# Yukun-Huang/DreamWaltz-G

Hardware: AMD Instinct MI355X
Metric: SDS steps/sec @512^2, 100k Gaussians, SD1.5+ControlNet; raster Mpix/s vs HBM roofline (higher is better)
Workload: dtype f32x

## Files before the change

### dreamwaltz-g_amd/_lib.py

```python
import ctypes
import os

_HERE = os.path.dirname(os.path.abspath(__file__))
LIB_PATH = os.environ.get("DWG_LIB") or os.path.join(_HERE, "csrc", "libdwg_hip.so")
_lib = None

c_f32p = ctypes.c_void_p
c_i32p = ctypes.c_void_p


class RasterSettingsC(ctypes.Structure):
    _fields_ = [
        ("image_height", ctypes.c_int32), ("image_width", ctypes.c_int32),
        ("tanfovx", ctypes.c_float), ("tanfovy", ctypes.c_float), ("scale_modifier", ctypes.c_float),
        ("sh_degree", ctypes.c_int32), ("sh_coeffs", ctypes.c_int32),
        ("prefiltered", ctypes.c_int32), ("debug", ctypes.c_int32),
        ("bg", ctypes.c_void_p), ("viewmatrix", ctypes.c_void_p), ("projmatrix", ctypes.c_void_p),
        ("campos", ctypes.c_void_p), ("visit_order", ctypes.c_void_p), ("tanfov", ctypes.c_void_p),
    ]


class AdamGroupC(ctypes.Structure):
    _fields_ = [("param", ctypes.c_void_p), ("grad", ctypes.c_void_p), ("exp_avg", ctypes.c_void_p), ("exp_avg_sq", ctypes.c_void_p),
                ("n", ctypes.c_int64), ("beta1", ctypes.c_float), ("beta2", ctypes.c_float), ("eps", ctypes.c_float), ("hyper_row", ctypes.c_int32)]


class SegmentC(ctypes.Structure):
    _fields_ = [("dst", ctypes.c_void_p), ("src", ctypes.c_void_p), ("count", ctypes.c_int64)]


class RasterFramesC(ctypes.Structure):
    _fields_ = [("num_frames", ctypes.c_int32), ("gaussian_stride", ctypes.c_int64), ("camera_stride", ctypes.c_int64)]


class NerfFieldDescC(ctypes.Structure):
    _fields_ = [("embeddings", ctypes.c_void_p), ("offsets", ctypes.c_void_p), ("host_offsets", ctypes.c_void_p),
                ("num_levels", ctypes.c_uint32), ("log2_per_level_scale", ctypes.c_float), ("base_resolution", ctypes.c_uint32),
                ("gridtype", ctypes.c_uint32), ("align_corners", ctypes.c_uint32), ("interp", ctypes.c_uint32), ("bound", ctypes.c_float),
                ("num_layers", ctypes.c_uint32), ("hidden", ctypes.c_uint32), ("out_dim", ctypes.c_uint32),
                ("weight", ctypes.c_void_p * 4), ("bias", ctypes.c_void_p * 4),
                ("density_activation", ctypes.c_uint32), ("density_prior", ctypes.c_uint32), ("albedo_sigmoid", ctypes.c_uint32),
                ("raw", ctypes.c_uint32), ("sigma_scale", ctypes.c_void_p), ("precision", ctypes.c_uint32)]


class NerfFieldGradsC(ctypes.Structure):
    _fields_ = [("embeddings", ctypes.c_void_p), ("weight", ctypes.c_void_p * 4), ("bias", ctypes.c_void_p * 4),
                ("sigma_scale", ctypes.c_void_p), ("accumulate", ctypes.c_uint32)]


_vp, _i32, _i64, _f32, _sz = ctypes.c_void_p, ctypes.c_int32, ctypes.c_int64, ctypes.c_float, ctypes.c_size_t
_u32 = ctypes.c_uint32
SIGNATURES = {
    "dwg_raster_workspace_sizes": (ctypes.c_int, [_i32, _i32, _i32, _i64, ctypes.POINTER(_sz), ctypes.POINTER(_sz),
                                                  ctypes.POINTER(_sz)]),
    "dwg_raster_num_pairs_ptr": (_vp, [_vp]),
    "dwg_raster_camera_setup": (ctypes.c_int, [_vp, _vp, _vp, _vp, _vp]),
    "dwg_raster_camera_block": (ctypes.c_int, [_vp, _vp, _vp, _vp, _vp, _vp, _vp]),
    "dwg_raster_forward_bin": (ctypes.c_int, [ctypes.POINTER(RasterSettingsC), _i32] + [_vp] * 9 + [_vp]),
    "dwg_raster_forward_render": (ctypes.c_int, [ctypes.POINTER(RasterSettingsC), _i32, _vp, _vp, _i64, _vp, _vp, _vp,
                                                 _vp, _vp]),
    "dwg_raster_forward_bin_frames": (ctypes.c_int, [ctypes.POINTER(RasterSettingsC), ctypes.POINTER(RasterFramesC), _i32] + [_vp] * 9 + [_vp]),
    "dwg_raster_forward_render_frames": (ctypes.c_int, [ctypes.POINTER(RasterSettingsC), ctypes.POINTER(RasterFramesC), _i32, _vp, _vp, _i64, _vp,
                                                        _vp, _vp, _vp, _vp]),
    "dwg_raster_backward": (ctypes.c_int, [ctypes.POINTER(RasterSettingsC), _i32] + [_vp] * 7 + [_vp, _vp, _i64, _vp, _vp]
                            + [_vp] * 3 + [_vp] * 8 + [_vp]),
    "dwg_raster_backward_frames": (ctypes.c_int, [ctypes.POINTER(RasterSettingsC), ctypes.POINTER(RasterFramesC), _i32] + [_vp] * 7
                                   + [_vp, _vp, _i64, _vp, _vp] + [_vp] * 3 + [_vp] * 8 + [_vp]),
    "dwg_lbs_joint_chain": (ctypes.c_int, [_i32, _vp, _vp, _vp, _vp, _vp, _vp, _i32, _vp, _vp, _vp]),
    "dwg_lbs_blend_forward": (ctypes.c_int, [_i32, _i32, _i32] + [_vp] * 7 + [_vp]),
    "dwg_lbs_blend_backward": (ctypes.c_int, [_i32] + [_vp] * 7 + [_vp]),
    "dwg_lbs_vertex_transform": (ctypes.c_int, [_i32] * 4 + [_vp] * 8 + [_vp]),
    "dwg_lbs_vertex_transform_backward_shape": (ctypes.c_int, [_i32] * 3 + [_vp] * 9 + [_vp]),
    "dwg_lbs_vertex_transform_backward_shape_ws": (ctypes.c_int, [_i32] * 3 + [_vp] * 10 + [_vp]),
    "dwg_lbs_vertex_transform_backward_shape_workspace_floats": (ctypes.c_size_t, [_i32]),
    "dwg_grid_encode_forward": (ctypes.c_int, [_vp, _vp, _vp, _vp, _u32, _u32, _u32, _u32, _f32, _u32, _vp, _u32, _u32, _u32,
                                               _u32, _vp]),
    "dwg_grid_encode_backward": (ctypes.c_int, [_vp, _vp, _vp, _vp, _vp, _u32, _u32, _u32, _u32, _f32, _u32, _vp, _vp, _u32,
                                                _u32, _u32, _u32, _vp, _vp]),
    "dwg_grid_backward_slabs_workspace_bytes": (_sz, [_u32, _u32, _u32]),
    "dwg_grid_encode_backward_slabs": (ctypes.c_int, [_vp, _vp, _vp, _vp, _vp, _u32, _u32, _u32, _u32, _f32, _u32, _vp, _vp, _u32, _u32,
                                                      _u32, _u32, _vp, _vp, _sz, _i32, _vp]),
    "dwg_nerf_field_forward": (ctypes.c_int, [ctypes.POINTER(NerfFieldDescC), _vp, ctypes.c_uint64, _vp, _vp, _vp]),
    "dwg_nerf_field_backward_workspace_bytes": (_sz, [ctypes.POINTER(NerfFieldDescC), ctypes.c_uint64]),
    "dwg_nerf_field_backward": (ctypes.c_int, [ctypes.POINTER(NerfFieldDescC), _vp, ctypes.c_uint64, _vp, _vp,
                                               ctypes.POINTER(NerfFieldGradsC), _vp, _sz, _vp]),
    "dwg_nerf_render_infer": (ctypes.c_int, [ctypes.POINTER(NerfFieldDescC), _vp, _vp, _vp, _vp, _u32, _vp, _f32, _u32, _f32, _u32, _u32, _u32, _f32,
                                             _u32, _vp, _vp, _vp, _vp, _u32, _vp]),
    "dwg_nerf_render_shaded": (ctypes.c_int, [ctypes.POINTER(NerfFieldDescC), _vp, _vp, _vp, _vp, _u32, _vp, _f32, _u32, _f32, _u32, _u32, _u32, _f32,
                                              _u32, _u32, _vp, _f32, _f32, _vp, _vp, _vp, _vp, _u32, _vp]),
    "dwg_pc_lattice_sigma": (ctypes.c_int, [ctypes.POINTER(NerfFieldDescC), _vp, _vp, _vp, _u32, _u32, _u32, _u32, _vp, _vp, _vp]),
    "dwg_pc_select_workspace_bytes": (_sz, [ctypes.c_uint64]),
    "dwg_pc_select_above": (ctypes.c_int, [ctypes.c_uint64, _vp, _f32, _vp, ctypes.c_uint64, _vp, _vp, _sz, _vp]),
    "dwg_pc_select_flags": (ctypes.c_int, [ctypes.c_uint64, _vp, _vp, ctypes.c_uint64, _vp, _vp, _sz, _vp]),
    "dwg_pc_lattice_points": (ctypes.c_int, [ctypes.c_uint64, _vp, _vp, _vp, _vp, _u32, _u32, _u32, _u32, _vp, _vp]),
    "dwg_pc_fd_points": (ctypes.c_int, [ctypes.c_uint64, _vp, _f32, _f32, _vp, _vp]),
    "dwg_pc_finish": (ctypes.c_int, [ctypes.c_uint64, _u32, _vp, _vp, _f32, _vp, _vp, _vp]),
    "dwg_pc_outside_boxes": (ctypes.c_int, [ctypes.c_uint64, _vp, _u32, _vp, _vp, _vp]),
    "dwg_occ_lattice_sigma": (ctypes.c_int, [ctypes.POINTER(NerfFieldDescC), _vp, _vp, _vp, _vp, _u32, _u32, _u32, _vp, _vp]),
    "dwg_occ_lattice_points": (ctypes.c_int, [_vp, _vp, _vp, _vp, _u32, _u32, _vp, _vp]),
    "dwg_occ_update_workspace_bytes": (_sz, [_u32, _u32]),
    "dwg_occ_update": (ctypes.c_int, [_vp, _vp, _u32, _u32, _f32, _f32, _vp, _vp, _vp, _sz, _vp]),
    "dwg_video_composite_forward": (ctypes.c_int, [_i32, _i32, _i32, _vp, _vp, _i64, _i64, _i64, _vp, _i32, _i32, _i32, _vp, _vp, _vp, _vp]),
    "dwg_video_composite_backward": (ctypes.c_int, [_i32, _i32, _i32, _vp, _i64, _i64, _i64, _vp, _i32, _i32, _i32, _vp, _vp, _vp]),
    "dwg_sigma_face_records": (ctypes.c_int, [_i32, _vp, _i32, _vp, _vp, _vp, _vp]),
    "dwg_sigma_area_cdf": (ctypes.c_int, [_i32, _vp, _vp, _vp]),
    "dwg_sigma_vertex_normals": (ctypes.c_int, [_i32, _vp, _vp, _vp, _vp, _vp, _vp]),
    "dwg_sigma_sample": (ctypes.c_int, [_i32, _vp, _i32, _vp, _i32, _vp, _vp, _vp, _f32, _vp, _vp, _vp, _vp, _vp]),
    "dwg_sigma_distance_workspace_bytes": (_sz, [_i32, _i32]),
    "dwg_sigma_point_mesh_distance": (ctypes.c_int, [_i32, _vp, _i32, _vp, _vp, _vp, _vp, _vp, _sz, _vp]),
    "dwg_sigma_keep_mask": (ctypes.c_int, [_i32, _vp, _vp, _f32, _i32, _vp, _vp, _vp, _vp]),
    "dwg_avinit_barycentric": (ctypes.c_int, [_i32, _vp, _vp, _i32, _vp, _i32, _vp, _vp, _vp, _vp, _vp]),
    "dwg_avinit_lbs_interp": (ctypes.c_int, [_i32, _i32, _i32, _vp, _vp, _vp, _vp, _vp]),
    "dwg_avinit_knn": (ctypes.c_int, [_i32, _vp, _i32, _vp, _i32, _vp, _vp, _vp]),
    "dwg_avinit_knn_weights": (ctypes.c_int, [_i32, _i32, _vp, _vp, _vp, _i32, _f32, _f32, _vp, _vp, _vp]),
    "dwg_avinit_smooth": (ctypes.c_int, [_i32, _i32, _i32, _vp, _vp, _vp, _vp, _vp, _vp, _i32, _vp]),
    "dwg_raymarch_near_far_from_aabb": (ctypes.c_int, [_vp, _vp, _vp, _u32, _f32, _vp, _vp, _vp]),
    "dwg_raymarch_sph_from_ray": (ctypes.c_int, [_vp, _vp, _f32, _u32, _vp, _vp]),
    "dwg_raymarch_morton3d": (ctypes.c_int, [_vp, _u32, _vp, _vp]),
    "dwg_raymarch_morton3d_invert": (ctypes.c_int, [_vp, _u32, _vp, _vp]),
    "dwg_raymarch_packbits": (ctypes.c_int, [_vp, _u32, _f32, _vp, _vp]),
    "dwg_raymarch_packbits_dev": (ctypes.c_int, [_vp, _u32, _vp, _vp, _vp]),
    "dwg_raymarch_flatten_rays": (ctypes.c_int, [_vp, _u32, _u32, _vp, _vp]),
    "dwg_raymarch_train_workspace_bytes": (_sz, [_u32]),
    "dwg_raymarch_march_rays_train": (ctypes.c_int, [_vp, _vp, _vp, _f32, _u32, _f32, _u32, _u32, _u32, _u32, _vp, _vp, _vp, _vp, _vp, _u32,
                                                     _vp, _vp, _vp, _vp, _sz, _vp]),
    "dwg_raymarch_composite_rays_train_forward": (ctypes.c_int, [_vp, _vp, _vp, _vp, _u32, _u32, _u32, _f32, _u32, _vp, _vp, _vp, _vp, _vp]),
    "dwg_raymarch_composite_rays_train_backward": (ctypes.c_int, [_vp] * 11 + [_u32, _u32, _u32, _f32, _u32, _vp, _vp, _vp]),
    "dwg_raymarch_march_rays": (ctypes.c_int, [_u32, _u32, _vp, _vp, _vp, _vp, _f32, _u32, _f32, _u32, _u32, _u32, _vp, _vp, _vp, _u32, _vp, _vp,
                                               _vp, _vp, _vp]),
    "dwg_raymarch_composite_rays": (ctypes.c_int, [_u32, _u32, _u32, _f32, _u32, _vp, _vp, _vp, _vp, _vp, _u32, _vp, _vp, _vp, _vp]),
    "dwg_gemm":(ctypes.c_int, [_vp, _vp]),
    "dwg_gemm_workspace_bytes": (_sz, [_vp]),
    "dwg_transpose_2byte": (ctypes.c_int, [_i32, _i32, _i32, _vp, _i64, _i64, _vp, _i64, _i64, _vp]),
    "dwg_transpose_dt": (ctypes.c_int, [_i32, _i32, _i32, _i32, _vp, _i64, _i64, _vp, _i64, _i64, _vp]),
    "dwg_xfmt_pack": (ctypes.c_int, [_i64, _vp, _vp, _vp]),
    "dwg_xfmt_unpack": (ctypes.c_int, [_i64, _vp, _vp, _vp]),
    "dwg_vae_image_pack": (ctypes.c_int, [_i32, _i32, _i32, _vp, _vp, _vp]),
    "dwg_vae_grad_prescale_pack": (ctypes.c_int, [_i32, _i32, _vp, ctypes.c_float, _vp, _vp, _vp]),
    "dwg_vae_dx_unpack": (ctypes.c_int, [_i32, _i32, _i32, _vp, _vp, _vp, _vp]),
    "dwg_xfmt_range_scan": (ctypes.c_int, [_i64, _vp, _vp, _vp]),
    "dwg_act_backward_colsum": (ctypes.c_int, [_i32, _i32, _i32, _vp, _vp, _vp, _vp, _vp]),
    "dwg_mlp_chain_forward": (ctypes.c_int, [_i32, _i32, _vp, _i32, _i32, _vp, _vp, _vp, _vp, _vp, _vp, _vp, _i32, _vp, _i32, _vp]),
    "dwg_mlp_chain_backward_workspace_floats": (ctypes.c_size_t, [_i32, _i32]),
    "dwg_mlp_chain_backward": (ctypes.c_int, [_i32, _i32, _vp, _i32, _i32, _vp, _vp, _vp, _vp, _vp, _vp, _i32, _vp, _i32, _vp, _i32, _vp, _vp, _vp,
                                              _vp, _vp, _i32, _vp, _vp]),
    "dwg_adam_step": (ctypes.c_int, [_i64, _vp, _vp, _vp, _vp, _f32, _f32, _f32, _f32, _i32, _f32, _vp]),
    "dwg_adam_step_dev": (ctypes.c_int, [_i64, _vp, _vp, _vp, _vp, _vp, _f32, _f32, _f32, _vp]),
    "dwg_adam_step_groups_dev": (ctypes.c_int, [_i32, _vp, _vp, _vp]),
    "dwg_groupnorm_forward": (ctypes.c_int, [_i32, _i32, _i32, _i32, _vp, _vp, _vp, _f32, _i32, _vp, _vp, _vp, _vp]),
    "dwg_groupnorm_backward": (ctypes.c_int, [_i32, _i32, _i32, _i32, _vp, _vp, _vp, _vp, _vp, _f32, _i32, _vp, _vp, _vp, _vp, _vp]),
    "dwg_groupnorm_workspace_floats": (_sz, [_i32, _i32]),
    "dwg_layernorm_forward": (ctypes.c_int, [_i32, _i32, _vp, _vp, _vp, _f32, _vp, _vp]),
    "dwg_geglu_forward": (ctypes.c_int, [_i64, _i32, _vp, _vp, _vp]),
    "dwg_attention_forward": (ctypes.c_int, [_i32, _i32, _i32, _i32, _i32, _vp, _i64, _i64, _vp, _i64, _i64, _vp, _i64, _i64,
                                             _vp, _i64, _i64, _f32, _vp]),
    "dwg_attention_forward_dt": (ctypes.c_int, [_i32, _i32, _i32, _i32, _i32, _i32, _vp, _i64, _i64, _vp, _i64, _i64, _vp, _i64, _i64,
                                                _vp, _i64, _i64, _f32, _vp]),
    "dwg_attention_split_workspace_bytes": (_sz, [_i32, _i32, _i32, _i32, _i32, _i32]),
    "dwg_attention_forward_ws": (ctypes.c_int, [_i32, _i32, _i32, _i32, _i32, _i32, _vp, _i64, _i64, _vp, _i64, _i64, _vp, _i64, _i64,
                                                _vp, _i64, _i64, _f32, _vp, _sz, _vp]),
    "dwg_attention_forward_pairs_dt": (ctypes.c_int, [_i32] * 7 + [_vp, _i64, _i64, _i64] * 4 + [_f32, _vp]),
    "dwg_attention_forward_pairs_ws": (ctypes.c_int, [_i32] * 7 + [_vp, _i64, _i64, _i64] * 4 + [_f32, _vp, _sz, _vp]),
    "dwg_softmax_rows_forward": (ctypes.c_int, [_i32, _i32, _f32, _vp, _i64, _vp, _i64, _vp]),
    "dwg_softmax_rows_backward": (ctypes.c_int, [_i32, _i32, _f32, _vp, _i64, _vp, _i64, _vp, _i64, _vp]),
    "dwg_groupnorm_forward_dt": (ctypes.c_int, [_i32, _i32, _i32, _i32, _i32, _vp, _vp, _vp, _f32, _i32, _vp, _vp, _vp, _vp]),
    "dwg_groupnorm_backward_dt": (ctypes.c_int, [_i32, _i32, _i32, _i32, _i32, _vp, _vp, _vp, _vp, _vp, _f32, _i32, _vp, _vp, _vp, _vp, _vp]),
    "dwg_layernorm_forward_dt": (ctypes.c_int, [_i32, _i32, _i32, _vp, _vp, _vp, _f32, _vp, _vp]),
    "dwg_geglu_forward_dt": (ctypes.c_int, [_i32, _i64, _i32, _vp, _vp, _vp]),
    "dwg_softmax_rows_forward_dt": (ctypes.c_int, [_i32, _i32, _i32, _f32, _vp, _i64, _vp, _i64, _vp]),
    "dwg_softmax_rows_backward_dt": (ctypes.c_int, [_i32, _i32, _i32, _f32, _vp, _i64, _vp, _i64, _vp, _i64, _vp]),
    "dwg_add_dt": (ctypes.c_int, [_i32, _i64, _vp, _vp, _vp, _vp]),
    "dwg_cast_f32_to_dt": (ctypes.c_int, [_i32, _i64, _vp, _vp, _vp]),
    "dwg_mlp_wgrad_workspace_floats": (_sz, [_i32]),
    "dwg_mlp_wgrad": (ctypes.c_int, [_i32, _i32, _i32, _vp, _i32, _vp, _i32, _vp, _i32, _vp, _vp]),
    "dwg_concat_channels": (ctypes.c_int, [_i64, _i32, _i32, _vp, _vp, _vp, _vp]),
    "dwg_concat_channels_bcast": (ctypes.c_int, [_i64, _i64, _i32, _i32, _vp, _vp, _vp, _vp]),
    "dwg_add_bf16": (ctypes.c_int, [_i64, _vp, _vp, _vp, _vp]),
    "dwg_interleave2x2": (ctypes.c_int, [_i32, _i32, _i32, _i32, _vp, _vp, _vp, _vp, _vp, _vp]),
    "dwg_cast_f32_to_bf16": (ctypes.c_int, [_i64, _vp, _vp, _vp]),
    "dwg_sds_posterior_sample": (ctypes.c_int, [_i32, ctypes.c_int64, _vp, _vp, ctypes.c_float, _vp, _vp]),
    "dwg_sds_posterior_sample_backward": (ctypes.c_int, [_i32, ctypes.c_int64, _vp, _vp, ctypes.c_float, _vp, _vp, _vp]),
    "dwg_sds_add_noise": (ctypes.c_int, [_i32, ctypes.c_int64, _vp, _vp, _vp, _i32, _vp, _vp, _vp]),
    "dwg_sds_gradient": (ctypes.c_int, [_i32, ctypes.c_int64, _vp, _vp, _vp, _i32, _vp, ctypes.c_float, _i32, _i32, _vp, _vp, _vp]),
    "dwg_gaussian_assemble_forward": (ctypes.c_int, [_i32, _i32, _vp, _vp, _f32, _vp, _vp, _f32, _vp, _vp, _vp, _vp, _vp, _vp, _vp, _vp]),
    "dwg_gaussian_assemble_forward_ld": (ctypes.c_int, [_i32, _i32, _vp, _vp, _f32, _vp, _vp, _i32, _f32, _vp, _vp, _vp, _vp, _vp, _vp, _vp, _vp]),
    "dwg_gaussian_assemble_backward_ld": (ctypes.c_int, [_i32, _i32, _f32, _vp, _f32, _vp, _vp, _vp, _vp, _vp, _vp, _vp, _vp, _vp, _vp, _vp, _i32, _i32,
                                                         _vp, _vp, _vp]),
    "dwg_copy_segments": (ctypes.c_int, [_i32, _vp, _f32, _f32, _vp]),
    "dwg_add_segments": (ctypes.c_int, [_i32, _vp, _vp]),
    "dwg_gaussian_assemble_backward": (ctypes.c_int, [_i32, _i32, _f32, _vp, _f32, _vp, _vp, _vp, _vp, _vp, _vp, _vp, _vp, _vp, _vp,
                                                       _vp, _vp, _vp, _vp]),
    "dwg_mesh_vertex_normals": (ctypes.c_int, [_i32, _i32, _vp, _vp, _vp, _vp, _vp, _vp, _vp]),
    "dwg_meshbind_forward": (ctypes.c_int, [_i32, _i32, _vp, _vp, _vp, _vp, _vp, _vp, _vp, _vp, _vp, _vp, _vp]),
    "dwg_meshbind_backward": (ctypes.c_int, [_i32, _i32, _vp, _vp, _vp, _vp, _vp, _vp, _vp, _vp, _vp, _vp, _vp, _vp, _vp]),
    "dwg_meshbind_backward_verts": (ctypes.c_int, [_i32, _i32] + [_vp] * 15 + [_vp]),
    "dwg_meshbind_backward_verts_gather": (ctypes.c_int, [_i32, _i32, _i32] + [_vp] * 18 + [_vp]),
    "dwg_mesh_vertex_normals_backward": (ctypes.c_int, [_i32, _i32] + [_vp] * 8 + [_vp]),
    "dwg_condition_keypoints": (ctypes.c_int, [_i32, _vp, _vp, _vp, _i32, _vp, _i32, _vp, _vp, ctypes.c_float, ctypes.c_float,
                                               ctypes.c_float, _i32, _vp, _vp]),
    "dwg_condition_workspace_bytes": (_sz, [_i32, _i32]),
    "dwg_condition_draw": (ctypes.c_int, [_i32, _i32, _vp, _i32, _vp, _vp, _vp, _vp]),
    "dwg_condition_keypoints_people": (ctypes.c_int, [_i32, _i32, _vp, _vp, _vp, _i32, _vp, _i32, _vp, _vp, ctypes.c_float, ctypes.c_float,
                                                      ctypes.c_float, _i32, _i32, _vp, _vp, _vp]),
    "dwg_condition_people_workspace_bytes": (_sz, [_i32, _i32, _i32]),
    "dwg_condition_draw_people": (ctypes.c_int, [_i32, _i32, _i32, _vp, _i32, _vp, _vp, _vp, _vp]),
    "dwg_depthmap_workspace_bytes": (_sz, [_i32, _i32, _i32]),
    "dwg_depthmap_cast": (ctypes.c_int, [_i32, _i32, _vp, _vp, _i32, _vp, _i32, _vp, _vp, _vp, _i32, _vp, _sz, _vp]),
    "dwg_depthmap_image": (ctypes.c_int, [_i32, _i32, _vp, _i32, _vp, _vp, _vp, _sz, _vp]),
    "dwg_pretrain_loss_workspace_bytes": (_sz, [_i64]),
    "dwg_pretrain_loss_forward": (ctypes.c_int, [_i32, _i64, _vp, _vp, _vp, _vp, _vp, _sz, _vp]),
    "dwg_pretrain_loss_backward": (ctypes.c_int, [_i32, _i64, _vp, _vp, _vp, _vp, _vp, _vp, _vp]),
    "dwg_image_loss_workspace_bytes": (_sz, [_i32, _i32, _i32, _i32]),
    "dwg_image_loss_forward": (ctypes.c_int, [_i32] * 5 + [_f32] + [_vp, _i64, _i64, _i64, _i64] * 2 + [_vp, _vp, _vp, _vp, _sz, _vp]),
    "dwg_image_loss_backward": (ctypes.c_int, [_i32] * 5 + [ctypes.c_double] * 2 + [_vp, _i64, _i64, _i64, _i64] * 2
                                + [_vp, _vp, _i32, _vp, _vp]),
    "dwg_graph_begin_capture": (ctypes.c_int, [_vp]),
    "dwg_graph_end_capture": (ctypes.c_int, [_vp, ctypes.POINTER(_vp)]),
    "dwg_graph_launch": (ctypes.c_int, [_vp, _vp]),
    "dwg_graph_destroy": (ctypes.c_int, [_vp]),
    "dwg_stream_create": (ctypes.c_int, [ctypes.POINTER(_vp)]),
    "dwg_stream_destroy": (ctypes.c_int, [_vp]),
    "dwg_stream_fork": (ctypes.c_int, [_vp, _vp]),
    "dwg_prof_enable": (ctypes.c_int, [_i32]),
    "dwg_prof_query": (ctypes.c_int, [ctypes.c_char_p, ctypes.POINTER(_i64), ctypes.POINTER(ctypes.c_double)]),
    "dwg_prof_dump": (_i64, [ctypes.c_char_p, _i64]),
    "dwg_prof_dump_symbols": (_i64, [ctypes.c_char_p, _i64]),
}


def lib():
    global _lib
    if _lib is None:
        if not os.path.exists(LIB_PATH):
            raise RuntimeError(
                "libdwg_hip.so not found at %s -- run `python dreamwaltz-g_amd/build.py` "
                "(there is no CPU fallback for the product path)" % LIB_PATH)
        import torch
        l = ctypes.CDLL(LIB_PATH)
        for name, (res, args) in SIGNATURES.items():
            fn = getattr(l, name)
            fn.restype = res
            fn.argtypes = args
        _lib = l
    return _lib


def check(rc, what):
    if rc != 0:
        raise RuntimeError("%s failed with DWG error %d" % (what, rc))


def ptr(t):
    return None if t is None else ctypes.c_void_p(t.data_ptr())


def prof_enable(on=True):
    check(lib().dwg_prof_enable(int(bool(on))), "dwg_prof_enable")


def prof_table():
    L = lib()
    need = L.dwg_prof_dump(None, 0)
    buf = ctypes.create_string_buffer(int(need) + 16)
    L.dwg_prof_dump(buf, len(buf))
    out = {}
    for line in buf.value.decode().splitlines():
        n, c, ms = line.split()
        out[n] = (int(c), float(ms))
    return out


def prof_symbols():
    L = lib()
    need = L.dwg_prof_dump_symbols(None, 0)
    buf = ctypes.create_string_buffer(int(need) + 16)
    L.dwg_prof_dump_symbols(buf, len(buf))
    out = {}
    for line in buf.value.decode().splitlines():
        n, c, ms, w = line.split("\t")
        out[n] = (int(c), float(ms), float(w))
    return out
```

### dreamwaltz-g_amd/csrc/gemm.hip

```cpp
#include "dwg_common.h"
#include "dwg_prof_internal.h"
#include "../../include/dwg_gemm.h"
#include <cstdlib>
#include <type_traits>

#if defined(DWG_GEMM_X_TU)
#include "dwg_xfmt.h"
typedef _Float16 HT;
#define DWG_DTYPE_HALF DWG_DTYPE_F32X
#define DWG_MFMA16(a, b, c) __builtin_amdgcn_mfma_f32_32x32x16_f16(a, b, c, 0, 0, 0)
#define DWG_HALF_NAME "f32x"
#elif defined(DWG_GEMM_F16_TU)
typedef _Float16 HT;
#define DWG_DTYPE_HALF DWG_DTYPE_F16
#define DWG_MFMA16(a, b, c) __builtin_amdgcn_mfma_f32_32x32x16_f16(a, b, c, 0, 0, 0)
#define DWG_HALF_NAME "f16"
#else
typedef __bf16 HT;
#define DWG_DTYPE_HALF DWG_DTYPE_BF16
#define DWG_MFMA16(a, b, c) __builtin_amdgcn_mfma_f32_32x32x16_bf16(a, b, c, 0, 0, 0)
#define DWG_HALF_NAME "bf16"
#endif

namespace {

typedef __attribute__((ext_vector_type(8))) HT bf16x8;
typedef __attribute__((ext_vector_type(16))) float f32x16;

struct ConvP {
    int enabled, Cin, Hin, Win, Hout, Wout, KH, KW, stride, pad_t, pad_l, dil;
    int up;
    int cin1;
    const void* A2;
};

struct GemmP {
    const void* A; const void* B; void* C; const void* bias; const void* residual;
    int M, N, K;
    long long sam, sak, sbn, sbk, ldc, ldr;
    int nb2;
    long long bA1, bA2, bB1, bB2, bC1, bC2, bR1, bR2;
    int act; float alpha;
    int out_bf16, res_bf16, bias_per_row, splitk, accumulate;
    float* ws;
    int bias_row_div;
    long long bias_ld;
    ConvP conv;
};

__device__ __forceinline__ float bf2f(HT x) { return (float)x; }
__device__ __forceinline__ HT f2bf(float x) { return (HT)x; }

struct bf16x4_t { HT v[4]; };
#ifdef DWG_GEMM_X_TU
__device__ __forceinline__ float ld_half1(const void* base, long long i) { return dwg_x_get1(base, i); }
__device__ __forceinline__ void st_half1(void* base, long long i, float v) { dwg_x_put1(base, i, v); }
__device__ __forceinline__ void ld_half4(const void* base, long long i, float (&v)[4]) { dwg_x_get4(base, i, v); }
__device__ __forceinline__ void st_half4(void* base, long long i, const float (&v)[4]) { dwg_x_put4(base, i, v); }
#else
__device__ __forceinline__ float ld_half1(const void* base, long long i) { return bf2f(reinterpret_cast<const HT*>(base)[i]); }
__device__ __forceinline__ void st_half1(void* base, long long i, float v) { reinterpret_cast<HT*>(base)[i] = f2bf(v); }
__device__ __forceinline__ void ld_half4(const void* base, long long i, float (&v)[4]) {
    const bf16x4_t r = *reinterpret_cast<const bf16x4_t*>(reinterpret_cast<const HT*>(base) + i);
#pragma unroll
    for (int e = 0; e < 4; e++) v[e] = bf2f(r.v[e]);
}
__device__ __forceinline__ void st_half4(void* base, long long i, const float (&v)[4]) {
    bf16x4_t o;
#pragma unroll
    for (int e = 0; e < 4; e++) o.v[e] = f2bf(v[e]);
    *reinterpret_cast<bf16x4_t*>(reinterpret_cast<HT*>(base) + i) = o;
}
#endif

template <bool LIGHT = false>
__device__ __forceinline__ float apply_act(float v, int act) {
    if constexpr (LIGHT) return act == 3 ? v / (1.f + __expf(-v)) : v;
    switch (act) {
        case 1: return v > 0.f ? v : 0.f;
        case 2: return v > 0.f ? v : 0.01f * v;
        case 3: return v / (1.f + __expf(-v));
        case 4: return 0.5f * v * (1.f + erff(v * 0.70710678118654752f));
        case 5: return 1.f / (1.f + __expf(-v));
        default: return v;
    }
}

template <typename T> struct TT;
template <> struct TT<HT> { static constexpr int VEC = 8; static constexpr int BK = 64; static constexpr int PAD = 8; };
template <> struct TT<float> { static constexpr int VEC = 4; static constexpr int BK = 16; static constexpr int PAD = 4; };

enum { MODE_KVEC = 0, MODE_RVEC = 1, MODE_SCALAR = 2, MODE_CONV = 3 };

template <typename T, int VEC> struct Chunk { T v[VEC]; };

template <typename T, int VEC>
__device__ __forceinline__ Chunk<T, VEC> load_vec(const T* p) {
    Chunk<T, VEC> c;
    *reinterpret_cast<uint4*>(&c) = *reinterpret_cast<const uint4*>(p);
    return c;
}
template <typename T, int VEC>
__device__ __forceinline__ Chunk<T, VEC> zero_chunk() {
    Chunk<T, VEC> c;
    *reinterpret_cast<uint4*>(&c) = make_uint4(0u, 0u, 0u, 0u);
    return c;
}

template <typename T, int ROWS, int MODE>
struct TileLoader {
    static constexpr int VEC = TT<T>::VEC, BK = TT<T>::BK, LDT = BK + TT<T>::PAD;
    static constexpr int CPR = BK / VEC, RPI = 256 / CPR;
    static constexpr int CPK = ROWS / VEC, KPI = 256 / CPK;
    static constexpr int NCH = (MODE == MODE_SCALAR) ? (ROWS * BK / 256) : (MODE == MODE_RVEC ? BK / KPI : ROWS / RPI);
    Chunk<T, VEC> regs[(MODE == MODE_SCALAR) ? 1 : NCH];
    T sregs[(MODE == MODE_SCALAR) ? NCH : 1];
    const T* rowptr[(MODE == MODE_KVEC) ? NCH : 1];
    int iy0[(MODE == MODE_CONV) ? NCH : 1], ix0[(MODE == MODE_CONV) ? NCH : 1];
    long long pix0[(MODE == MODE_CONV) ? NCH : 1];
    bool rok[(MODE == MODE_CONV) ? NCH : 1];
    const T* base; long long srow, sk; int nrows, r0, kcur, kend;
    int ci, ky, kx;

    __device__ __forceinline__ void init(const T* base_, long long srow_, long long sk_, int nrows_, int r0_, int kbeg, int kend_,
                                         const ConvP& cv) {
        base = base_; srow = srow_; sk = sk_; nrows = nrows_; r0 = r0_; kend = kend_;
        const int tid = threadIdx.x;
        if (MODE == MODE_KVEC) {
            kcur = kbeg + (tid % CPR) * VEC;
#pragma unroll
            for (int i = 0; i < NCH; i++) {
                int r = r0 + tid / CPR + i * RPI;
                rowptr[i] = r < nrows ? base + (long long)r * srow : nullptr;
            }
        } else if (MODE == MODE_CONV) {
            kcur = kbeg + (tid % CPR) * VEC;
            const int hw = cv.Hout * cv.Wout;
#pragma unroll
            for (int i = 0; i < NCH; i++) {
                int r = r0 + tid / CPR + i * RPI;
                rok[i] = r < nrows;
                int rr = rok[i] ? r : 0;
                int img = rr / hw, rem = rr - img * hw;
                int oy = rem / cv.Wout, ox = rem - oy * cv.Wout;
                iy0[i] = oy * cv.stride - cv.pad_t; ix0[i] = ox * cv.stride - cv.pad_l;
                pix0[i] = (long long)img * cv.Hin * cv.Win;
            }
            int tap = kcur / cv.Cin;
            ci = kcur - tap * cv.Cin; ky = tap / cv.KW; kx = tap - ky * cv.KW;
        } else {
            kcur = kbeg;
        }
    }

    __device__ __forceinline__ void advance(const ConvP& cv) {
        kcur += BK;
        if (MODE == MODE_CONV) {
            ci += BK;
            while (ci >= cv.Cin) { ci -= cv.Cin; if (++kx == cv.KW) { kx = 0; ++ky; } }
        }
    }

    __device__ __forceinline__ void load(const ConvP& cv) {
        const int tid = threadIdx.x;
        if (MODE == MODE_KVEC) {
            const bool kok = kcur < kend;
#pragma unroll
            for (int i = 0; i < NCH; i++)
                regs[i] = (kok && rowptr[i]) ? load_vec<T, VEC>(rowptr[i] + kcur) : zero_chunk<T, VEC>();
        } else if (MODE == MODE_CONV) {
            const bool kok = kcur < kend;
            const T* src0 = ci < cv.cin1 ? base : reinterpret_cast<const T*>(cv.A2);
            const int cs = ci < cv.cin1 ? cv.cin1 : (cv.Cin - cv.cin1);
            const int co = ci < cv.cin1 ? ci : ci - cv.cin1;
#pragma unroll
            for (int i = 0; i < NCH; i++) {
                int iy = iy0[i] + ky, ix = ix0[i] + kx;
                bool ok = kok && rok[i] && iy >= 0 && ix >= 0;
                if (cv.dil > 1) { ok = ok && (iy % cv.dil == 0) && (ix % cv.dil == 0); iy /= cv.dil; ix /= cv.dil; }
                if (cv.up > 1) { iy >>= 1; ix >>= 1; }
                ok = ok && iy < cv.Hin && ix < cv.Win;
                regs[i] = ok ? load_vec<T, VEC>(src0 + (pix0[i] + (long long)iy * cv.Win + ix) * cs + co) : zero_chunk<T, VEC>();
            }
        } else if (MODE == MODE_RVEC) {
#pragma unroll
            for (int i = 0; i < NCH; i++) {
                int kk = tid / CPK + i * KPI, rc = tid % CPK;
                int r = r0 + rc * VEC, k = kcur + kk;
                regs[i] = (r < nrows && k < kend) ? load_vec<T, VEC>(base + (long long)k * sk + r) : zero_chunk<T, VEC>();
            }
        } else {
#pragma unroll
            for (int i = 0; i < NCH; i++) {
                int c = tid + i * 256, row = c / BK, kk = c - row * BK;
                int r = r0 + row, k = kcur + kk;
                sregs[i] = (r < nrows && k < kend) ? base[(long long)r * srow + (long long)k * sk] : (T)0.f;
            }
        }
    }

    __device__ __forceinline__ void store(T* lds) {
        const int tid = threadIdx.x;
        if (MODE == MODE_KVEC || MODE == MODE_CONV) {
#pragma unroll
            for (int i = 0; i < NCH; i++)
                *reinterpret_cast<uint4*>(lds + (tid / CPR + i * RPI) * LDT + (tid % CPR) * VEC) = *reinterpret_cast<uint4*>(&regs[i]);
        } else if (MODE == MODE_RVEC) {
#pragma unroll
            for (int i = 0; i < NCH; i++) {
                int kk = tid / CPK + i * KPI, rc = tid % CPK;
#pragma unroll
                for (int e = 0; e < VEC; e++) lds[(rc * VEC + e) * LDT + kk] = regs[i].v[e];
            }
        } else {
#pragma unroll
            for (int i = 0; i < NCH; i++) {
                int c = tid + i * 256, row = c / BK, kk = c - row * BK;
                lds[row * LDT + kk] = sregs[i];
            }
        }
    }
};

template <typename T>
__device__ __forceinline__ void mma_tile(const T* sa, const T* sb, int lane, f32x16& acc);

template <>
__device__ __forceinline__ void mma_tile<HT>(const HT* sa, const HT* sb, int lane, f32x16& acc) {
    constexpr int LDT = TT<HT>::BK + TT<HT>::PAD;
    const HT* pa = sa + (lane & 31) * LDT + (lane >> 5) * 8;
    const HT* pb = sb + (lane & 31) * LDT + (lane >> 5) * 8;
#pragma unroll
    for (int ks = 0; ks < TT<HT>::BK / 16; ks++) {
        bf16x8 a = *reinterpret_cast<const bf16x8*>(pa + ks * 16);
        bf16x8 b = *reinterpret_cast<const bf16x8*>(pb + ks * 16);
        acc = DWG_MFMA16(a, b, acc);
    }
}
template <>
__device__ __forceinline__ void mma_tile<float>(const float* sa, const float* sb, int lane, f32x16& acc) {
    constexpr int LDT = TT<float>::BK + TT<float>::PAD;
    const float* pa = sa + (lane & 31) * LDT + (lane >> 5);
    const float* pb = sb + (lane & 31) * LDT + (lane >> 5);
#pragma unroll
    for (int ks = 0; ks < TT<float>::BK / 2; ks++)
        acc = __builtin_amdgcn_mfma_f32_32x32x2f32(pa[ks * 2], pb[ks * 2], acc, 0, 0, 0);
}

template <bool LIGHT = false>
__device__ __forceinline__ void epilogue_store(const GemmP& p, float v, int row, int col, long long coff, long long roff) {
    const long long ci = coff + (long long)row * p.ldc + col;
    if (p.bias) v += reinterpret_cast<const float*>(p.bias)[p.bias_row_div > 0 ? (long long)(row / p.bias_row_div) * p.bias_ld + col
                                                                             : (p.bias_per_row ? row : col)];
    v = apply_act<LIGHT>(v, p.act);
    if (p.residual) {
        const long long ri = roff + (long long)row * p.ldr + col;
        v += p.res_bf16 ? ld_half1(p.residual, ri) : reinterpret_cast<const float*>(p.residual)[ri];
    }
    if (p.out_bf16) st_half1(p.C, ci, v);
    else if (p.accumulate) reinterpret_cast<float*>(p.C)[ci] += v;
    else reinterpret_cast<float*>(p.C)[ci] = v;
}

__device__ __forceinline__ bool epilogue_vec_ok(const GemmP& p, long long coff, long long roff) {
    bool ok = (p.N & 3) == 0 && (p.ldc & 3) == 0 && (coff & 3) == 0 && ((uintptr_t)p.C & 15) == 0;
    if (p.residual) ok = ok && (p.ldr & 3) == 0 && (roff & 3) == 0 && ((uintptr_t)p.residual & 15) == 0;
    return ok;
}

template <bool LIGHT = false>
__device__ __forceinline__ void epilogue_store4(const GemmP& p, float (&v)[4], int row, int col, long long coff, long long roff, bool vec_ok) {
    if (!vec_ok || col + 3 >= p.N) {
#pragma unroll
        for (int e = 0; e < 4; e++)
            if (col + e < p.N) epilogue_store<LIGHT>(p, v[e], row, col + e, coff, roff);
        return;
    }
    if (p.bias) {
        const float* b = reinterpret_cast<const float*>(p.bias);
        if (p.bias_row_div > 0) {
            b += (long long)(row / p.bias_row_div) * p.bias_ld + col;
            v[0] += b[0]; v[1] += b[1]; v[2] += b[2]; v[3] += b[3];
        } else if (p.bias_per_row) {
            const float br = b[row];
            v[0] += br; v[1] += br; v[2] += br; v[3] += br;
        } else {
            v[0] += b[col]; v[1] += b[col + 1]; v[2] += b[col + 2]; v[3] += b[col + 3];
        }
    }
#pragma unroll
    for (int e = 0; e < 4; e++) v[e] = apply_act<LIGHT>(v[e], p.act);
    if (p.residual) {
        const long long ri = roff + (long long)row * p.ldr + col;
        if (p.res_bf16) {
            float r[4];
            ld_half4(p.residual, ri, r);
#pragma unroll
            for (int e = 0; e < 4; e++) v[e] += r[e];
        } else {
            float4 r = *reinterpret_cast<const float4*>(reinterpret_cast<const float*>(p.residual) + ri);
            v[0] += r.x; v[1] += r.y; v[2] += r.z; v[3] += r.w;
        }
    }
    const long long ci = coff + (long long)row * p.ldc + col;
    if (p.out_bf16) {
        st_half4(p.C, ci, v);
    } else {
        float4* dst = reinterpret_cast<float4*>(reinterpret_cast<float*>(p.C) + ci);
        float4 o = make_float4(v[0], v[1], v[2], v[3]);
        if (p.accumulate) { float4 c = *dst; o.x += c.x; o.y += c.y; o.z += c.z; o.w += c.w; }
        *dst = o;
    }
}

template <int BN, int BM = 128> struct EpiLds {
    static constexpr int LDC = BN + 4;
    static constexpr int passes(size_t lds_bytes) {
        return lds_bytes >= (size_t)BM * LDC * 4 ? 1 : (lds_bytes >= (size_t)(BM / 2) * LDC * 4 ? 2 : 4);
    }
    static constexpr size_t bytes(int npass) { return (size_t)(BM / npass) * LDC * 4; }
};

template <int BN, int NPASS, int TM, int TN, bool LIGHT, int BM = 128, int NT = 256, typename RowFn>
__device__ __forceinline__ void tile_epilogue_lds(const GemmP& p, f32x16 (&acc)[TM][TN], float* sC, int n0, int wm, int wn, int lane, int tid,
                                                  int ks_id, long long coff, long long roff, RowFn row_of) {
    constexpr int LDC = EpiLds<BN, BM>::LDC, C4 = BN / 4, PR = BM / NPASS;
    constexpr int BPP = BM / 32 / NPASS;
    static_assert(NT % C4 == 0 && (C4 & (C4 - 1)) == 0, "a thread keeps one column group");
    const bool vec_ok = epilogue_vec_ok(p, coff, roff);
    const int lrow = lane & 31, lhalf = (lane >> 5) * 4;
    const bool geglu = p.act == 6;
    const float* bias = reinterpret_cast<const float*>(p.bias);
    const bool fast = vec_ok && !geglu && !p.accumulate && !p.bias_per_row && (p.splitk <= 1 || p.ws) &&
                      (!bias || p.bias_row_div > 0 || ((uintptr_t)bias & 15) == 0) &&
                      (!bias || p.bias_row_div <= 0 || (((uintptr_t)bias & 15) == 0 && (p.bias_ld & 3) == 0)) &&
                      (p.splitk <= 1 || ((uintptr_t)p.ws & 15) == 0);
#pragma unroll 1
    for (int q = 0; q < NPASS; q++) {
        __syncthreads();
#pragma unroll
        for (int i = 0; i < TM; i++) {
            const int rb = wm * TM + i;
            if (NPASS > 1 && rb / BPP != q) continue;
            float* dst = sC + ((NPASS > 1 ? rb % BPP : rb) * 32 + lrow) * LDC + wn * 64 + lhalf;
#pragma unroll
            for (int j = 0; j < TN; j++)
#pragma unroll
                for (int r4 = 0; r4 < 4; r4++)
                    *reinterpret_cast<float4*>(dst + j * 32 + 8 * r4) =
                        make_float4(acc[i][j][4 * r4], acc[i][j][4 * r4 + 1], acc[i][j][4 * r4 + 2], acc[i][j][4 * r4 + 3]);
        }
        __syncthreads();
        if (geglu) {
            constexpr int G = C4 / 2, RSTEP = NT / G;
            const int o4 = tid & (G - 1), rl0 = tid / G;
            const int b = o4 >> 3, w = (o4 & 7) * 4;
            const int colp = n0 + b * 64 + w;
            if (colp + 35 < p.N) {
                float bh[4] = {0.f, 0.f, 0.f, 0.f}, bg[4] = {0.f, 0.f, 0.f, 0.f};
                if (bias) {
#pragma unroll
                    for (int e = 0; e < 4; e++) { bh[e] = bias[colp + e]; bg[e] = bias[colp + 32 + e]; }
                }
                const bool vec_store = ((p.ldc | coff) & 3) == 0 && ((uintptr_t)p.C & 7) == 0;
#pragma unroll 2
                for (int rl = rl0; rl < PR; rl += RSTEP) {
                    const int row = row_of(q * PR + rl);
                    if (row < 0) continue;
                    const float4 h = *reinterpret_cast<const float4*>(sC + rl * LDC + b * 64 + w);
                    const float4 g = *reinterpret_cast<const float4*>(sC + rl * LDC + b * 64 + 32 + w);
                    const float hv[4] = {h.x, h.y, h.z, h.w}, gv[4] = {g.x, g.y, g.z, g.w};
                    float v[4];
#pragma unroll
                    for (int e = 0; e < 4; e++) {
                        const float a = fmaf(hv[e], p.alpha, bh[e]);
                        const float gg = fmaf(gv[e], p.alpha, bg[e]);
                        v[e] = a * 0.5f * gg * (1.f + dwg_erf_fast(gg * 0.70710678118654752f));
                    }
                    const long long ci = coff + (long long)row * p.ldc + (n0 + b * 64) / 2 + w;
                    if (p.out_bf16) {
                        if (vec_store) {
                            st_half4(p.C, ci, v);
                        } else {
#pragma unroll
                            for (int e = 0; e < 4; e++) st_half1(p.C, ci + e, v[e]);
                        }
                    } else {
#pragma unroll
                        for (int e = 0; e < 4; e++) reinterpret_cast<float*>(p.C)[ci + e] = v[e];
                    }
                }
            }
            continue;
        }
        if (fast) {
            constexpr int RSTEP = NT / C4;
            const int c4 = tid & (C4 - 1), rl0 = tid / C4;
            const int col = n0 + c4 * 4;
            if (col < p.N) {
                const bool col_bias = bias && p.bias_row_div <= 0;
                float4 bc = make_float4(0.f, 0.f, 0.f, 0.f);
                if (col_bias) bc = *reinterpret_cast<const float4*>(bias + col);
                const bool slab = p.splitk > 1;
#pragma unroll 2
                for (int rl = rl0; rl < PR; rl += RSTEP) {
                    const int row = row_of(q * PR + rl);
                    if (row < 0) continue;
                    const float4 a = *reinterpret_cast<const float4*>(sC + rl * LDC + c4 * 4);
                    float v[4] = {a.x * p.alpha, a.y * p.alpha, a.z * p.alpha, a.w * p.alpha};
                    if (slab) {
                        *reinterpret_cast<float4*>(p.ws + ((long long)ks_id * p.M + row) * p.N + col) = make_float4(v[0], v[1], v[2], v[3]);
                        continue;
                    }
                    if (col_bias) { v[0] += bc.x; v[1] += bc.y; v[2] += bc.z; v[3] += bc.w; }
                    else if (bias) {
                        const float4 b = *reinterpret_cast<const float4*>(bias + (long long)(row / p.bias_row_div) * p.bias_ld + col);
                        v[0] += b.x; v[1] += b.y; v[2] += b.z; v[3] += b.w;
                    }
                    if (p.act == 3) {
#pragma unroll
                        for (int e = 0; e < 4; e++) v[e] = v[e] / (1.f + __expf(-v[e]));
                    } else if (p.act != 0) {
#pragma unroll
                        for (int e = 0; e < 4; e++) v[e] = apply_act<LIGHT>(v[e], p.act);
                    }
                    if (p.residual) {
                        const long long ri = roff + (long long)row * p.ldr + col;
                        if (p.res_bf16) {
                            float r[4];
                            ld_half4(p.residual, ri, r);
#pragma unroll
                            for (int e = 0; e < 4; e++) v[e] += r[e];
                        } else {
                            const float4 r = *reinterpret_cast<const float4*>(reinterpret_cast<const float*>(p.residual) + ri);
                            v[0] += r.x; v[1] += r.y; v[2] += r.z; v[3] += r.w;
                        }
                    }
                    const long long ci = coff + (long long)row * p.ldc + col;
                    if (p.out_bf16) {
                        st_half4(p.C, ci, v);
                    } else {
                        *reinterpret_cast<float4*>(reinterpret_cast<float*>(p.C) + ci) = make_float4(v[0], v[1], v[2], v[3]);
                    }
                }
            }
            continue;
        }
#pragma unroll 1
        for (int idx = tid; idx < PR * C4; idx += NT) {
            const int rl = idx / C4, c4 = idx - rl * C4;
            const int row = row_of(q * PR + rl), col = n0 + c4 * 4;
            if (row < 0 || col >= p.N) continue;
            const float4 a = *reinterpret_cast<const float4*>(sC + rl * LDC + c4 * 4);
            float v[4] = {a.x * p.alpha, a.y * p.alpha, a.z * p.alpha, a.w * p.alpha};
            if (p.splitk > 1) {
                if (p.ws) {
                    float* dst = p.ws + ((long long)ks_id * p.M + row) * p.N + col;
                    if ((p.N & 3) == 0) *reinterpret_cast<float4*>(dst) = make_float4(v[0], v[1], v[2], v[3]);
                    else {
#pragma unroll
                        for (int e = 0; e < 4; e++) if (col + e < p.N) dst[e] = v[e];
                    }
                } else {
#pragma unroll
                    for (int e = 0; e < 4; e++)
                        if (col + e < p.N) atomicAdd(reinterpret_cast<float*>(p.C) + coff + (long long)row * p.ldc + col + e, v[e]);
                }
                continue;
            }
            epilogue_store4<LIGHT>(p, v, row, col, coff, roff, vec_ok);
        }
    }
}

__global__ __launch_bounds__(256) void k_splitk_epilogue(GemmP p) {
    const long long n = (long long)p.M * p.N;
    if ((p.N & 3) == 0) {
        const bool vec_ok = epilogue_vec_ok(p, 0, 0);
        const int N4 = p.N >> 2;
        const long long n4 = n >> 2;
        for (long long i = (long long)blockIdx.x * 256 + threadIdx.x; i < n4; i += (long long)gridDim.x * 256) {
            const unsigned iu = (unsigned)i;
            const int row = (int)(iu / (unsigned)N4), col = (int)(iu - (unsigned)row * (unsigned)N4) * 4;
            const float4* src = reinterpret_cast<const float4*>(p.ws) + i;
            float4 a = src[0];
            int sidx = 1;
            for (; sidx + 3 < p.splitk; sidx += 4) {
                const float4 u0 = src[(long long)sidx * n4], u1 = src[(long long)(sidx + 1) * n4], u2 = src[(long long)(sidx + 2) * n4],
                             u3 = src[(long long)(sidx + 3) * n4];
                a.x += u0.x; a.y += u0.y; a.z += u0.z; a.w += u0.w;
                a.x += u1.x; a.y += u1.y; a.z += u1.z; a.w += u1.w;
                a.x += u2.x; a.y += u2.y; a.z += u2.z; a.w += u2.w;
                a.x += u3.x; a.y += u3.y; a.z += u3.z; a.w += u3.w;
            }
            if (sidx + 1 < p.splitk) {
                const float4 u0 = src[(long long)sidx * n4], u1 = src[(long long)(sidx + 1) * n4];
                a.x += u0.x; a.y += u0.y; a.z += u0.z; a.w += u0.w;
                a.x += u1.x; a.y += u1.y; a.z += u1.z; a.w += u1.w;
                sidx += 2;
            }
            if (sidx < p.splitk) {
                const float4 u = src[(long long)sidx * n4];
                a.x += u.x; a.y += u.y; a.z += u.z; a.w += u.w;
            }
            float v[4] = {a.x, a.y, a.z, a.w};
            epilogue_store4(p, v, row, col, 0, 0, vec_ok);
        }
        return;
    }
    for (long long i = (long long)blockIdx.x * 256 + threadIdx.x; i < n; i += (long long)gridDim.x * 256) {
        float v = 0.f;
        for (int s = 0; s < p.splitk; s++) v += p.ws[(long long)s * n + i];
        int row = (int)(i / p.N), col = (int)(i - (long long)row * p.N);
        epilogue_store(p, v, row, col, 0, 0);
    }
}

static void launch_splitk_epilogue(const GemmP& p, hipStream_t stream) {
    if (!(p.splitk > 1 && p.ws)) return;
    long long n = (long long)p.M * p.N;
    if ((p.N & 3) == 0) n >>= 2;
    int blocks = (int)((n + 255) / 256); if (blocks > 2048) blocks = 2048;
    DWG_LAUNCH("splitk_epilogue", k_splitk_epilogue, dim3(blocks), dim3(256), 0, stream, p);
}
template <typename T, int BN, int AMODE, int BMODE>
__global__ __launch_bounds__(256, (sizeof(T) == 4 || BN == 64) ? 2 : 1) void k_gemm(GemmP p) {
    constexpr int BM = 128, BK = TT<T>::BK, LDT = BK + TT<T>::PAD;
    constexpr int WN = BN / 64;
    constexpr int WM = 4 / WN;
    constexpr int TM = BM / WM / 32;
    constexpr int TN = 2;
    extern __shared__ __attribute__((aligned(16))) unsigned char smem_raw[];
    T* sA = reinterpret_cast<T*>(smem_raw);
    T* sB = sA + 2 * BM * LDT;
    const int tid = threadIdx.x, lane = tid & 63, wave = tid >> 6;
    const int wm = wave / WN, wn = wave % WN;
    const int m0 = blockIdx.x * BM;
    const int ntn = (p.N + BN - 1) / BN;
    const int n0 = (blockIdx.y % ntn) * BN;
    const int ks_id = blockIdx.y / ntn;
    const int z = blockIdx.z, z1 = z / p.nb2, z2 = z - z1 * p.nb2;
    const T* A = reinterpret_cast<const T*>(p.A) + z1 * p.bA1 + z2 * p.bA2;
    const T* B = reinterpret_cast<const T*>(p.B) + z1 * p.bB1 + z2 * p.bB2;
    int kbeg = 0, kend = p.K;
    if (p.splitk > 1) {
        int per = ((p.K + p.splitk - 1) / p.splitk + BK - 1) / BK * BK;
        kbeg = ks_id * per; kend = min(p.K, kbeg + per);
    }
    f32x16 acc[TM][TN];
#pragma unroll
    for (int i = 0; i < TM; i++)
#pragma unroll
        for (int j = 0; j < TN; j++)
#pragma unroll
            for (int r = 0; r < 16; r++) acc[i][j][r] = 0.f;

    TileLoader<T, BM, AMODE> la;
    TileLoader<T, BN, BMODE> lb;
    la.init(A, p.sam, p.sak, p.M, m0, kbeg, kend, p.conv);
    lb.init(B, p.sbn, p.sbk, p.N, n0, kbeg, kend, p.conv);
    const int nk = kend > kbeg ? (kend - kbeg + BK - 1) / BK : 0;
    if (nk > 0) {
        la.load(p.conv); lb.load(p.conv);
        la.store(sA); lb.store(sB);
    }
    __syncthreads();
    for (int kt = 0; kt < nk; kt++) {
        const int cur = kt & 1;
        if (kt + 1 < nk) {
            la.advance(p.conv); lb.advance(p.conv);
            la.load(p.conv); lb.load(p.conv);
        }
        const T* a = sA + cur * BM * LDT + (wm * TM * 32) * LDT;
        const T* b = sB + cur * BN * LDT + (wn * 64) * LDT;
#pragma unroll
        for (int i = 0; i < TM; i++)
#pragma unroll
            for (int j = 0; j < TN; j++) mma_tile<T>(b + j * 32 * LDT, a + i * 32 * LDT, lane, acc[i][j]);
        if (kt + 1 < nk) { la.store(sA + (cur ^ 1) * BM * LDT); lb.store(sB + (cur ^ 1) * BN * LDT); }
        __syncthreads();
    }
    constexpr int NPASS = EpiLds<BN>::passes((size_t)2 * (BM + BN) * LDT * sizeof(T));
    static_assert((size_t)2 * (BM + BN) * LDT * sizeof(T) >= EpiLds<BN>::bytes(NPASS), "epilogue staging fits in the operand stages");
    tile_epilogue_lds<BN, NPASS, TM, TN, false>(p, acc, reinterpret_cast<float*>(smem_raw), n0, wm, wn, lane, tid, ks_id, z1 * p.bC1 + z2 * p.bC2,
                                         z1 * p.bR1 + z2 * p.bR2, [&](int rl) { const int r = m0 + rl; return r < p.M ? r : -1; });
}

__device__ __attribute__((aligned(16))) unsigned char g_zero16[16];

template <int ROWS, bool CONV, int NW = 4>
struct GldsLoader {
    static constexpr int NJ = ROWS / (8 * NW);
    const HT* rowptr[CONV ? 1 : NJ];
    int iy0[CONV ? NJ : 1], ix0[CONV ? NJ : 1];
    long long pix0[CONV ? NJ : 1];
    bool rok[CONV ? NJ : 1];
    const HT* base;
    int kc[2], kend, ci[2], ky[2], kx[2];

    __device__ __forceinline__ void init(const HT* base_, long long srow, int nrows, int r0, int kbeg, int kend_, const ConvP& cv) {
        static_assert(NJ % 2 == 0, "row-block parity must equal j parity");
        base = base_; kend = kend_;
        const int lane = threadIdx.x & 63, wave = threadIdx.x >> 6, sub = lane >> 3;
        const int lg0 = (lane & 7) ^ (sub >> 1);
        kc[0] = kbeg + lg0 * 8; kc[1] = kbeg + (lg0 ^ 4) * 8;
        if (!CONV) {
#pragma unroll
            for (int j = 0; j < NJ; j++) {
                int r = r0 + (wave * NJ + j) * 8 + sub;
                rowptr[j] = r < nrows ? base + (long long)r * srow : nullptr;
            }
        } else {
            const int hw = cv.Hout * cv.Wout;
#pragma unroll
            for (int j = 0; j < NJ; j++) {
                int r = r0 + (wave * NJ + j) * 8 + sub;
                rok[j] = r < nrows;
                int rr = rok[j] ? r : 0;
                int img = rr / hw, rem = rr - img * hw;
                int oy = rem / cv.Wout, ox = rem - oy * cv.Wout;
                iy0[j] = oy * cv.stride - cv.pad_t; ix0[j] = ox * cv.stride - cv.pad_l;
                pix0[j] = (long long)img * cv.Hin * cv.Win;
            }
#pragma unroll
            for (int q = 0; q < 2; q++) {
                int tap = kc[q] / cv.Cin;
                ci[q] = kc[q] - tap * cv.Cin; ky[q] = tap / cv.KW; kx[q] = tap - ky[q] * cv.KW;
            }
        }
    }
    __device__ __forceinline__ void advance(const ConvP& cv) {
        kc[0] += 64; kc[1] += 64;
        if (CONV) {
#pragma unroll
            for (int q = 0; q < 2; q++) {
                ci[q] += 64;
                while (ci[q] >= cv.Cin) { ci[q] -= cv.Cin; if (++kx[q] == cv.KW) { kx[q] = 0; ++ky[q]; } }
            }
        }
    }
    __device__ __forceinline__ void issue(unsigned char* lds_tile, const ConvP& cv) {
        const int wave = __builtin_amdgcn_readfirstlane(threadIdx.x >> 6);
        const HT* zero = reinterpret_cast<const HT*>(g_zero16);
        const HT* src0[2] = {base, base}; int cs[2] = {0, 0}, co[2] = {0, 0};
        bool kok[2];
#pragma unroll
        for (int q = 0; q < 2; q++) {
            kok[q] = kc[q] < kend;
            if (CONV) {
                src0[q] = ci[q] < cv.cin1 ? base : reinterpret_cast<const HT*>(cv.A2);
                cs[q] = ci[q] < cv.cin1 ? cv.cin1 : (cv.Cin - cv.cin1);
                co[q] = ci[q] < cv.cin1 ? ci[q] : ci[q] - cv.cin1;
            }
        }
#pragma unroll
        for (int j = 0; j < NJ; j++) {
            const int q = j & 1;
            const HT* src;
            if (!CONV) {
                src = (kok[q] && rowptr[j]) ? rowptr[j] + kc[q] : zero;
            } else {
                int iy = iy0[j] + ky[q], ix = ix0[j] + kx[q];
                bool ok = kok[q] && rok[j] && iy >= 0 && ix >= 0;
                if (cv.dil > 1) { ok = ok && (iy % cv.dil == 0) && (ix % cv.dil == 0); iy /= cv.dil; ix /= cv.dil; }
                if (cv.up > 1) { iy >>= 1; ix >>= 1; }
                ok = ok && iy < cv.Hin && ix < cv.Win;
                src = ok ? src0[q] + (pix0[j] + (long long)iy * cv.Win + ix) * cs[q] + co[q] : zero;
            }
            unsigned char* dst = lds_tile + ((wave * NJ + j) * 8) * 128;
            __builtin_amdgcn_global_load_lds((const __attribute__((address_space(1))) void*)src,
                                             (__attribute__((address_space(3))) void*)dst, 16, 0, 0);
        }
    }
};

template <int ROWS, int NW = 4, bool CAT = false>
struct GldsConvFast {
    static constexpr int NJ = ROWS / (8 * NW);
    const unsigned char* pb[NJ];
    const unsigned char* pb2[CAT ? NJ : 1];
    unsigned int mask[NJ];
    int kcur, kend, tap, ci, ky, kx;

    __device__ __forceinline__ void init(const HT* base, long long, int nrows, int r0, int kbeg, int kend_, const ConvP& cv) {
        static_assert(NJ % 2 == 0, "row-block parity must equal j parity");
        const int lane = threadIdx.x & 63, wave = threadIdx.x >> 6, sub = lane >> 3;
        const int lg0 = (lane & 7) ^ (sub >> 1);
        kcur = kbeg; kend = kend_;
        tap = kbeg / cv.Cin; ci = kbeg - tap * cv.Cin; ky = tap / cv.KW; kx = tap - ky * cv.KW;
        const int hw = cv.Hout * cv.Wout;
        const int cs1 = CAT ? cv.cin1 : cv.Cin;
#pragma unroll
        for (int j = 0; j < NJ; j++) {
            const int r = r0 + (wave * NJ + j) * 8 + sub;
            const bool rok = r < nrows;
            const int rr = rok ? r : 0;
            const int img = rr / hw, rem = rr - img * hw;
            const int oy = rem / cv.Wout, ox = rem - oy * cv.Wout;
            const int iy0 = oy * cv.stride - cv.pad_t, ix0 = ox * cv.stride - cv.pad_l;
            unsigned int m = 0;
            for (int t = 0, y = 0; y < cv.KH; y++)
                for (int x = 0; x < cv.KW; x++, t++) {
                    const int iy = iy0 + y, ix = ix0 + x;
                    if (rok && iy >= 0 && iy < cv.Hin && ix >= 0 && ix < cv.Win) m |= 1u << t;
                }
            mask[j] = m;
            const long long pix = ((long long)img * cv.Hin + iy0) * cv.Win + ix0;
            pb[j] = reinterpret_cast<const unsigned char*>(base) + (pix * cs1 + (lg0 ^ ((j & 1) << 2)) * 8) * 2;
            if (CAT) pb2[j] = reinterpret_cast<const unsigned char*>(cv.A2) + (pix * (cv.Cin - cv.cin1) + (lg0 ^ ((j & 1) << 2)) * 8) * 2;
        }
    }
    __device__ __forceinline__ void advance(const ConvP& cv) {
        kcur += 64; ci += 64;
        const int w = ci >= cv.Cin ? 1 : 0;
        ci = w ? 0 : ci; tap += w; kx += w;
        const int w2 = kx == cv.KW ? 1 : 0;
        kx = w2 ? 0 : kx; ky += w2;
    }
    __device__ __forceinline__ void issue(unsigned char* lds_tile, const ConvP& cv) {
        const int wave = __builtin_amdgcn_readfirstlane(threadIdx.x >> 6);
        const unsigned char* zero = g_zero16;
        const bool second = CAT && ci >= cv.cin1;
        const int cs = CAT ? (second ? cv.Cin - cv.cin1 : cv.cin1) : cv.Cin;
        const long long uoff = (((long long)ky * cv.Win + kx) * cs + (second ? ci - cv.cin1 : ci)) * 2;
        const unsigned int bit = kcur < kend ? (1u << tap) : 0u;
#pragma unroll
        for (int j = 0; j < NJ; j++) {
            const unsigned char* src = (mask[j] & bit) ? ((CAT && second) ? pb2[j] : pb[j]) + uoff : zero;
            unsigned char* dst = lds_tile + ((wave * NJ + j) * 8) * 128;
            __builtin_amdgcn_global_load_lds((const __attribute__((address_space(1))) void*)src,
                                             (__attribute__((address_space(3))) void*)dst, 16, 0, 0);
        }
    }
};

template <int N>
__device__ __forceinline__ void wait_vmcnt() {
    __builtin_amdgcn_s_waitcnt((N & 15) | ((N >> 4) << 14) | (7 << 4) | (15 << 8));
}

template <int BM, int AKIND, int NW = 4> struct ALoaderOf { typedef GldsLoader<BM, false, NW> type; };
template <int BM, int NW> struct ALoaderOf<BM, 1, NW> { typedef GldsLoader<BM, true, NW> type; };
template <int BM, int NW> struct ALoaderOf<BM, 2, NW> { typedef GldsConvFast<BM, NW, false> type; };
template <int BM, int NW> struct ALoaderOf<BM, 3, NW> { typedef GldsConvFast<BM, NW, true> type; };

template <int BM, int BN> struct GldsGeom {
    static constexpr int WN = BN / 64, WM = (BM == 128 && BN == 64) ? 4 : BM / 64, NW = WM * WN, NT = NW * 64, TM = BM / WM / 32, TN = 2;
};

template <int BM, int BN, int AKIND, int S>
__device__ __forceinline__ void gemm_glds_body(const GemmP& p) {
    typedef GldsGeom<BM, BN> Geo;
    constexpr int WN = Geo::WN, WM = Geo::WM, NW = Geo::NW, NT = Geo::NT, TM = Geo::TM, TN = Geo::TN;
    constexpr int ABYTES = BM * 128, BBYTES = BN * 128, STAGE = ABYTES + BBYTES;
    extern __shared__ __attribute__((aligned(16))) unsigned char smem_raw[];
    const int tid = threadIdx.x, lane = tid & 63, wave = tid >> 6;
    const int wm = wave / WN, wn = wave % WN;
    const int gm = (p.M + BM - 1) / BM, ntn = (p.N + BN - 1) / BN;
    const int nwg = gridDim.x;
    int id = blockIdx.x;
    {
        const int q = nwg / 8, r = nwg % 8, xcd = id % 8, loc = id / 8;
        id = (xcd < r ? xcd * (q + 1) : r * (q + 1) + (xcd - r) * q) + loc;
    }
    const int tile = id % (gm * ntn), ks_id = id / (gm * ntn);
    const int m0 = (tile / ntn) * BM, n0 = (tile % ntn) * BN;
    const int z = blockIdx.z, z1 = z / p.nb2, z2 = z - z1 * p.nb2;
    const HT* A = reinterpret_cast<const HT*>(p.A) + z1 * p.bA1 + z2 * p.bA2;
    const HT* B = reinterpret_cast<const HT*>(p.B) + z1 * p.bB1 + z2 * p.bB2;
    int kbeg = 0, kend = p.K;
    if (p.splitk > 1) {
        int per = ((p.K + p.splitk - 1) / p.splitk + 63) / 64 * 64;
        kbeg = ks_id * per; kend = min(p.K, kbeg + per);
    }
    f32x16 acc[TM][TN];
#pragma unroll
    for (int i = 0; i < TM; i++)
#pragma unroll
        for (int j = 0; j < TN; j++)
#pragma unroll
            for (int r = 0; r < 16; r++) acc[i][j][r] = 0.f;
#ifdef DWG_GEMM_X_TU
    f32x16 acx[TM][TN];
#pragma unroll
    for (int i = 0; i < TM; i++)
#pragma unroll
        for (int j = 0; j < TN; j++)
#pragma unroll
            for (int r = 0; r < 16; r++) acx[i][j][r] = 0.f;
#endif
    typename ALoaderOf<BM, AKIND, NW>::type la;
    GldsLoader<BN, false, NW> lb;
    la.init(A, p.sam, p.M, m0, kbeg, kend, p.conv);
    lb.init(B, p.sbn, p.N, n0, kbeg, kend, p.conv);
    const int nk = kend > kbeg ? (kend - kbeg + 63) / 64 : 0;
    constexpr int LPT = (BM + BN) * 128 / (NT * 16);
#pragma unroll
    for (int s = 0; s < S - 1; s++) {
        la.issue(smem_raw + s * STAGE, p.conv); lb.issue(smem_raw + s * STAGE + ABYTES, p.conv);
        la.advance(p.conv); lb.advance(p.conv);
    }
    const int frow = lane & 31, fx = (lane >> 1) & 7, fh = lane >> 5;
#ifdef DWG_GEMM_X_TU
    constexpr int KS = 2;
    struct Frag { bf16x8 ah[TM], al[TM], bh[TN], bl[TN]; };
#else
    constexpr int KS = 4;
    struct Frag { bf16x8 af[TM], bf[TN]; };
#endif
    auto load_frags = [&](int stage, int ks, Frag& f) {
        const unsigned char* ta = smem_raw + stage * STAGE + (wm * TM * 32 + frow) * 128;
        const unsigned char* tb = smem_raw + stage * STAGE + ABYTES + (wn * 64 + frow) * 128;
#ifdef DWG_GEMM_X_TU
        const int offh = (((ks * 4 + fh * 2) ^ fx) << 4), offl = (((ks * 4 + fh * 2 + 1) ^ fx) << 4);
#pragma unroll
        for (int i = 0; i < TM; i++) {
            f.ah[i] = *reinterpret_cast<const bf16x8*>(ta + i * 32 * 128 + offh);
            f.al[i] = *reinterpret_cast<const bf16x8*>(ta + i * 32 * 128 + offl);
        }
#pragma unroll
        for (int j = 0; j < TN; j++) {
            f.bh[j] = *reinterpret_cast<const bf16x8*>(tb + j * 32 * 128 + offh);
            f.bl[j] = *reinterpret_cast<const bf16x8*>(tb + j * 32 * 128 + offl);
        }
#else
        const int off = (((ks * 2 + fh) ^ fx) << 4);
#pragma unroll
        for (int i = 0; i < TM; i++) f.af[i] = *reinterpret_cast<const bf16x8*>(ta + i * 32 * 128 + off);
#pragma unroll
        for (int j = 0; j < TN; j++) f.bf[j] = *reinterpret_cast<const bf16x8*>(tb + j * 32 * 128 + off);
#endif
    };
    auto mma = [&](const Frag& f) {
#ifdef DWG_GEMM_X_TU
#pragma unroll
        for (int i = 0; i < TM; i++)
#pragma unroll
            for (int j = 0; j < TN; j++) acc[i][j] = DWG_MFMA16(f.bh[j], f.ah[i], acc[i][j]);
#pragma unroll
        for (int i = 0; i < TM; i++)
#pragma unroll
            for (int j = 0; j < TN; j++) acx[i][j] = DWG_MFMA16(f.bl[j], f.ah[i], acx[i][j]);
#pragma unroll
        for (int i = 0; i < TM; i++)
#pragma unroll
            for (int j = 0; j < TN; j++) acx[i][j] = DWG_MFMA16(f.bh[j], f.al[i], acx[i][j]);
#else
#pragma unroll
        for (int i = 0; i < TM; i++)
#pragma unroll
            for (int j = 0; j < TN; j++) acc[i][j] = DWG_MFMA16(f.bf[j], f.af[i], acc[i][j]);
#endif
    };
    auto wait_tile_and_lds = [&]() {
        constexpr int N = (S - 2) * LPT;
        __builtin_amdgcn_s_waitcnt((N & 15) | ((N >> 4) << 14) | (7 << 4) | (0 << 8));
    };
    Frag F[2];
    int cur = 0, nxt = S - 1;
    if (nk > 0) {
        wait_vmcnt<(S - 2) * LPT>();
        __builtin_amdgcn_s_barrier();
        load_frags(0, 0, F[0]);
        __builtin_amdgcn_s_waitcnt(0xC07F);
    }
#ifdef DWG_GEMM_X_TU
    constexpr int MPS = 3 * TM * TN;
#else
    constexpr int MPS = TM * TN;
#endif
    for (int kt = 0; kt < nk; kt++) {
        const int cnext = cur + 1 == S ? 0 : cur + 1;
#pragma unroll
        for (int ks = 0; ks < KS; ks++) {
            if (ks + 1 < KS) {
                load_frags(cur, ks + 1, F[(ks + 1) & 1]);
            } else {
                wait_tile_and_lds();
                __builtin_amdgcn_s_barrier();
                load_frags(cnext, 0, F[0]);
            }
            __builtin_amdgcn_sched_barrier(0);
            if (ks == 0) {
                la.issue(smem_raw + nxt * STAGE, p.conv); lb.issue(smem_raw + nxt * STAGE + ABYTES, p.conv);
                la.advance(p.conv); lb.advance(p.conv);
            }
            mma(F[ks & 1]);
            if (ks == 0) {
#pragma unroll
                for (int m = 0; m < MPS; m++) {
                    __builtin_amdgcn_sched_group_barrier(0x008, 1, 0);
                    __builtin_amdgcn_sched_group_barrier(0x006, (LPT * 10 + MPS - 1) / MPS, 0);
                    __builtin_amdgcn_sched_group_barrier(0x020, (LPT + MPS - 1) / MPS, 0);
                }
            }
            __builtin_amdgcn_sched_barrier(0);
        }
        __builtin_amdgcn_s_waitcnt(0xC07F);
        cur = cnext; nxt = nxt + 1 == S ? 0 : nxt + 1;
    }
    wait_vmcnt<0>();
#ifdef DWG_GEMM_X_TU
#pragma unroll
    for (int i = 0; i < TM; i++)
#pragma unroll
        for (int j = 0; j < TN; j++)
#pragma unroll
            for (int r = 0; r < 16; r++) acc[i][j][r] = fmaf(acx[i][j][r], DWG_X_LO_INV, acc[i][j][r]);
#endif
    constexpr int NPASS = EpiLds<BN, BM>::passes((size_t)S * STAGE);
    static_assert((size_t)S * STAGE >= EpiLds<BN, BM>::bytes(NPASS), "epilogue staging fits in the operand stages");
    tile_epilogue_lds<BN, NPASS, TM, TN, false, BM, NT>(p, acc, reinterpret_cast<float*>(smem_raw), n0, wm, wn, lane, tid, ks_id, z1 * p.bC1 + z2 * p.bC2,
                                         z1 * p.bR1 + z2 * p.bR2, [&](int rl) { const int r = m0 + rl; return r < p.M ? r : -1; });
}

template <int BN, int AKIND, int S>
__global__ __launch_bounds__(256, 2) void k_gemm_glds(GemmP p) {
    gemm_glds_body<128, BN, AKIND, S>(p);
}

template <int BM, int BN, int AKIND, int S>
__global__ __launch_bounds__(512, 2) void k_gemm_glds8(GemmP p) {
    static_assert(GldsGeom<BM, BN>::NT == 512, "eight waves");
    gemm_glds_body<BM, BN, AKIND, S>(p);
}

static double gemm_flops(const GemmP& p, int batch) {
    double f = 2.0 * p.M * p.N * p.K * batch;
#ifdef DWG_GEMM_X_TU
    f *= 0.5;
#endif
    if (p.conv.enabled && p.conv.dil > 1) f /= (double)(p.conv.dil * p.conv.dil);
    return f;
}

template <int BN, int AKIND>
static void launch_glds(const GemmP& p, int batch, hipStream_t stream, const char* name) {
    constexpr int S = (BN == 64 && AKIND != 1) ? 3 : 2;
    size_t lds = (size_t)S * (128 + BN) * 128;
    static bool attr_set = false;
    if (!attr_set) {
        hipFuncSetAttribute(reinterpret_cast<const void*>(&k_gemm_glds<BN, AKIND, S>), hipFuncAttributeMaxDynamicSharedMemorySize, (int)lds);
        attr_set = true;
    }
    dim3 grid(((p.M + 127) / 128) * ((p.N + BN - 1) / BN) * (p.splitk > 1 ? p.splitk : 1), 1, batch);
    static const char* const sym[2][4] = {{"k_gemm_glds<64, 0, 3>", "k_gemm_glds<64, 1, 2>", "k_gemm_glds<64, 2, 3>", "k_gemm_glds<64, 3, 3>"},
                                          {"k_gemm_glds<128, 0, 2>", "k_gemm_glds<128, 1, 2>", "k_gemm_glds<128, 2, 2>", "k_gemm_glds<128, 3, 2>"}};
    DWG_LAUNCH_W(name, sym[BN == 128][AKIND], gemm_flops(p, batch), (k_gemm_glds<BN, AKIND, S>), grid, dim3(256), lds, stream, p);
    launch_splitk_epilogue(p, stream);
}

template <int BM, int BN, int AKIND>
static void launch_glds8(const GemmP& p, int batch, hipStream_t stream, const char* name) {
    constexpr int S = 3;
    const size_t lds = (size_t)S * (BM + BN) * 128;
    static bool attr_set = false;
    if (!attr_set) {
        hipFuncSetAttribute(reinterpret_cast<const void*>(&k_gemm_glds8<BM, BN, AKIND, S>), hipFuncAttributeMaxDynamicSharedMemorySize, (int)lds);
        attr_set = true;
    }
    dim3 grid(((p.M + BM - 1) / BM) * ((p.N + BN - 1) / BN) * (p.splitk > 1 ? p.splitk : 1), 1, batch);
    static const char* const sym[2][4] = {
        {"k_gemm_glds8<256, 128, 0, 3>", "k_gemm_glds8<256, 128, 1, 3>", "k_gemm_glds8<256, 128, 2, 3>", "k_gemm_glds8<256, 128, 3, 3>"},
        {"k_gemm_glds8<128, 256, 0, 3>", "k_gemm_glds8<128, 256, 1, 3>", "k_gemm_glds8<128, 256, 2, 3>", "k_gemm_glds8<128, 256, 3, 3>"}};
    DWG_LAUNCH_W(name, sym[BN == 256][AKIND], gemm_flops(p, batch), (k_gemm_glds8<BM, BN, AKIND, S>), grid, dim3(512), lds, stream, p);
    launch_splitk_epilogue(p, stream);
}

template <bool V> struct BoolC { static constexpr bool value = V; };
template <int BN, int NW> struct Patch2Geom {
    static constexpr int PH = NW == 8 ? 16 : 8, PW = 16, HP = PH + 2, WP = PW + 2, NPIX = HP * WP, BM = PH * PW;
    static constexpr int NPI = (NPIX + 7) / 8;
    static constexpr int PPW = (NPI + NW - 1) / NW;
    static constexpr int WN = BN / 64, WM = NW / WN, TM = BM / WM / 32, TN = 2, NT = NW * 64;
    static constexpr int NJW = BN / (8 * NW);
    static constexpr int PBYTES = NPI * 8 * 128, BBYTES = BN * 128;
};

template <int BN, bool SPLIT, int NW, int NBS>
__global__ __launch_bounds__(NW * 64, 2) void k_conv3x3_patch2(GemmP p) {
    typedef Patch2Geom<BN, NW> G;
    constexpr int PH = G::PH, PW = G::PW, WP = G::WP, NPIX = G::NPIX, NPI = G::NPI, PPW = G::PPW;
    constexpr int WN = G::WN, WM = G::WM, TM = G::TM, TN = G::TN, NT = G::NT, NJW = G::NJW, BM = G::BM;
    constexpr int PBYTES = G::PBYTES, BBYTES = G::BBYTES;
    static_assert(NJW >= 1 && (NJW % 2 == 0 || NJW == 1), "row-block parity");
    extern __shared__ __attribute__((aligned(16))) unsigned char smem_raw[];
    unsigned char* sP = smem_raw;
    unsigned char* sB = smem_raw + 2 * PBYTES;
    const ConvP& cv = p.conv;
    const int tid = threadIdx.x, lane = tid & 63, wave = tid >> 6;
    const int wv = __builtin_amdgcn_readfirstlane(wave);
    const int wm = wave / WN, wn = wave % WN;
    const int tiles_x = (cv.Wout + PW - 1) / PW, tiles_y = (cv.Hout + PH - 1) / PH;
    const int nimg = p.M / (cv.Hout * cv.Wout);
    const int gm = nimg * tiles_y * tiles_x, ntn = (p.N + BN - 1) / BN;
    int id = blockIdx.x;
    {
        const int nwg = gridDim.x, q = nwg / 8, r = nwg % 8, xcd = id % 8, loc = id / 8;
        id = (xcd < r ? xcd * (q + 1) : r * (q + 1) + (xcd - r) * q) + loc;
    }
    int ks_id = 0;
    if constexpr (SPLIT) { ks_id = id / (gm * ntn); id -= ks_id * gm * ntn; }
    const int mt = id / ntn, n0 = (id % ntn) * BN;
    const int img = mt / (tiles_y * tiles_x), trem = mt % (tiles_y * tiles_x);
    const int y0 = (trem / tiles_x) * PH, x0 = (trem % tiles_x) * PW;
    const HT* X = reinterpret_cast<const HT*>(p.A) + (long long)img * cv.Hin * cv.Win * cv.Cin;
    const HT* Wt = reinterpret_cast<const HT*>(p.B);
    const HT* zero = reinterpret_cast<const HT*>(g_zero16);
    const int sub = lane >> 3, lg0 = (lane & 7) ^ (sub >> 1);

    auto issue_patch = [&](int cc, bool valid, unsigned char* dst) {
#pragma unroll
        for (int q = 0; q < PPW; q++) {
            int inst = wv + q * NW;
            if (inst >= NPI) inst -= NW;
            const int pi = inst * 8 + sub;
            const int py = pi / WP, px = pi - py * WP;
            const int iy = y0 - 1 + py, ix = x0 - 1 + px;
            const bool ok = valid && pi < NPIX && iy >= 0 && iy < cv.Hin && ix >= 0 && ix < cv.Win;
            const HT* src = ok ? X + ((long long)iy * cv.Win + ix) * cv.Cin + (lg0 ^ ((inst & 1) << 2)) * 8 + cc * 64 : zero;
            __builtin_amdgcn_global_load_lds((const __attribute__((address_space(1))) void*)src,
                                             (__attribute__((address_space(3))) void*)(dst + inst * 8 * 128), 16, 0, 0);
        }
    };
    const HT* wrow[NJW];
#pragma unroll
    for (int j = 0; j < NJW; j++) {
        const int r = n0 + (wv * NJW + j) * 8 + sub;
        wrow[j] = r < p.N ? Wt + (long long)r * p.sbn + (lg0 ^ (((wv * NJW + j) & 1) << 2)) * 8 : nullptr;
    }
    auto issue_w = [&](int cc, int tap, bool valid, unsigned char* dst) {
        const long long kofs = (long long)tap * cv.Cin + cc * 64;
#pragma unroll
        for (int j = 0; j < NJW; j++) {
            const HT* src = (valid && wrow[j]) ? wrow[j] + kofs : zero;
            __builtin_amdgcn_global_load_lds((const __attribute__((address_space(1))) void*)src,
                                             (__attribute__((address_space(3))) void*)(dst + (wv * NJW + j) * 8 * 128), 16, 0, 0);
        }
    };
    f32x16 acc[TM][TN];
#pragma unroll
    for (int i = 0; i < TM; i++)
#pragma unroll
        for (int j = 0; j < TN; j++)
#pragma unroll
            for (int r = 0; r < 16; r++) acc[i][j][r] = 0.f;
#ifdef DWG_GEMM_X_TU
    f32x16 acx[TM][TN];
#pragma unroll
    for (int i = 0; i < TM; i++)
#pragma unroll
        for (int j = 0; j < TN; j++)
#pragma unroll
            for (int r = 0; r < 16; r++) acx[i][j][r] = 0.f;
    constexpr int KS = 2, MPS = 3 * TM * TN;
    struct Frag { bf16x8 ah[TM], al[TM], bh[TN], bl[TN]; };
#else
    constexpr int KS = 4, MPS = TM * TN;
    struct Frag { bf16x8 af[TM], bf[TN]; };
#endif
    int pbase[TM];
#pragma unroll
    for (int i = 0; i < TM; i++) {
        const int r = (wm * TM + i) * 32 + (lane & 31);
        pbase[i] = (r / PW) * WP + (r % PW);
    }
    int cc0 = 0, ncc = cv.Cin / 64;
    if constexpr (SPLIT) {
        const int per = (ncc + p.splitk - 1) / p.splitk;
        cc0 = ks_id * per; ncc = min(ncc, cc0 + per);
    }
    const int frow = lane & 31, fx = (lane >> 1) & 7, fh = lane >> 5;
    const int nsteps = max(0, ncc - cc0) * 9;
    auto load_frags = [&](const unsigned char* pa, int toff, const unsigned char* tbs, int ks, Frag& f) {
        const unsigned char* tb = tbs + (wn * 64 + frow) * 128;
#ifdef DWG_GEMM_X_TU
        const int cl = ks * 4 + fh * 2;
#pragma unroll
        for (int i = 0; i < TM; i++) {
            const int pi = pbase[i] + toff, sw = (pi >> 1) & 7;
            f.ah[i] = *reinterpret_cast<const bf16x8*>(pa + pi * 128 + ((cl ^ sw) << 4));
            f.al[i] = *reinterpret_cast<const bf16x8*>(pa + pi * 128 + (((cl + 1) ^ sw) << 4));
        }
#pragma unroll
        for (int j = 0; j < TN; j++) {
            f.bh[j] = *reinterpret_cast<const bf16x8*>(tb + j * 32 * 128 + ((cl ^ fx) << 4));
            f.bl[j] = *reinterpret_cast<const bf16x8*>(tb + j * 32 * 128 + (((cl + 1) ^ fx) << 4));
        }
#else
        const int cl = ks * 2 + fh;
#pragma unroll
        for (int i = 0; i < TM; i++) {
            const int pi = pbase[i] + toff;
            f.af[i] = *reinterpret_cast<const bf16x8*>(pa + pi * 128 + ((cl ^ ((pi >> 1) & 7)) << 4));
        }
#pragma unroll
        for (int j = 0; j < TN; j++) f.bf[j] = *reinterpret_cast<const bf16x8*>(tb + j * 32 * 128 + ((cl ^ fx) << 4));
#endif
    };
    auto mma = [&](const Frag& f) {
#ifdef DWG_GEMM_X_TU
#pragma unroll
        for (int i = 0; i < TM; i++)
#pragma unroll
            for (int j = 0; j < TN; j++) acc[i][j] = DWG_MFMA16(f.bh[j], f.ah[i], acc[i][j]);
#pragma unroll
        for (int i = 0; i < TM; i++)
#pragma unroll
            for (int j = 0; j < TN; j++) acx[i][j] = DWG_MFMA16(f.bl[j], f.ah[i], acx[i][j]);
#pragma unroll
        for (int i = 0; i < TM; i++)
#pragma unroll
            for (int j = 0; j < TN; j++) acx[i][j] = DWG_MFMA16(f.bh[j], f.al[i], acx[i][j]);
#else
#pragma unroll
        for (int i = 0; i < TM; i++)
#pragma unroll
            for (int j = 0; j < TN; j++) acc[i][j] = DWG_MFMA16(f.bf[j], f.af[i], acc[i][j]);
#endif
    };
    issue_patch(cc0, nsteps > 0, sP + (cc0 & 1) * PBYTES);
#pragma unroll
    for (int g = 0; g < NBS - 1; g++) issue_w(cc0 + g / 9, g % 9, g < nsteps, sB + g * BBYTES);
    Frag F[2];
    if (nsteps > 0) {
        wait_vmcnt<(NBS - 2) * NJW>();
        __builtin_amdgcn_s_barrier();
        load_frags(sP + (cc0 & 1) * PBYTES, 0, sB, 0, F[0]);
        __builtin_amdgcn_s_waitcnt(0xC07F);
    }
    int bst = 0;
    auto step = [&](auto is_tap0, int tap, int cc, const unsigned char* pa, const unsigned char* pan) {
        constexpr bool TAP0 = decltype(is_tap0)::value;
        const int ty = tap >= 6 ? 2 : (tap >= 3 ? 1 : 0);
        const int toff = ty * WP + (tap - 3 * ty);
        const int bnext = bst + 1 == NBS ? 0 : bst + 1;
        const int bfill = bst == 0 ? NBS - 1 : bst - 1;
        const unsigned char* tb = sB + bst * BBYTES;
#pragma unroll
        for (int ks = 0; ks < KS; ks++) {
            if (ks + 1 < KS) {
                load_frags(pa, toff, tb, ks + 1, F[(ks + 1) & 1]);
            } else {
                if (TAP0 || tap <= NBS - 2) {
                    constexpr int N = (NBS - 2) * NJW + PPW;
                    __builtin_amdgcn_s_waitcnt((N & 15) | ((N >> 4) << 14) | (7 << 4) | (0 << 8));
                } else {
                    constexpr int N = (NBS - 2) * NJW;
                    __builtin_amdgcn_s_waitcnt((N & 15) | ((N >> 4) << 14) | (7 << 4) | (0 << 8));
                }
                __builtin_amdgcn_s_barrier();
                const int ntap = tap == 8 ? 0 : tap + 1;
                const int nty = ntap >= 6 ? 2 : (ntap >= 3 ? 1 : 0);
                load_frags(tap == 8 ? pan : pa, nty * WP + (ntap - 3 * nty), sB + bnext * BBYTES, 0, F[0]);
            }
            __builtin_amdgcn_sched_barrier(0);
            if (ks == 0) {
                const int ft = tap + NBS - 1, fcc = cc + (ft >= 9 ? 1 : 0), ftap = ft >= 9 ? ft - 9 : ft;
                issue_w(fcc, ftap, fcc < ncc, sB + bfill * BBYTES);
                if (TAP0) issue_patch(cc + 1, cc + 1 < ncc, const_cast<unsigned char*>(pan));
            }
            mma(F[ks & 1]);
            if (ks == 0) {
                constexpr int NL = NJW + (TAP0 ? PPW : 0);
#pragma unroll
                for (int m = 0; m < MPS; m++) {
                    __builtin_amdgcn_sched_group_barrier(0x008, 1, 0);
                    __builtin_amdgcn_sched_group_barrier(0x006, (NL * 8 + MPS - 1) / MPS, 0);
                    __builtin_amdgcn_sched_group_barrier(0x020, (NL + MPS - 1) / MPS, 0);
                }
            }
            __builtin_amdgcn_sched_barrier(0);
        }
        __builtin_amdgcn_s_waitcnt(0xC07F);
        bst = bnext;
    };
    for (int cc = cc0; cc < ncc; cc++) {
        const unsigned char* pa = sP + (cc & 1) * PBYTES;
        const unsigned char* pan = sP + ((cc + 1) & 1) * PBYTES;
        step(BoolC<true>{}, 0, cc, pa, pan);
#pragma unroll 1
        for (int tap = 1; tap < 9; tap++) step(BoolC<false>{}, tap, cc, pa, pan);
    }
    wait_vmcnt<0>();
    __builtin_amdgcn_s_barrier();
#ifdef DWG_GEMM_X_TU
#pragma unroll
    for (int i = 0; i < TM; i++)
#pragma unroll
        for (int j = 0; j < TN; j++)
#pragma unroll
            for (int r = 0; r < 16; r++) acc[i][j][r] = fmaf(acx[i][j][r], DWG_X_LO_INV, acc[i][j][r]);
#endif
    constexpr int NPASS = EpiLds<BN, BM>::passes((size_t)2 * PBYTES + NBS * BBYTES);
    static_assert((size_t)2 * PBYTES + NBS * BBYTES >= EpiLds<BN, BM>::bytes(NPASS), "epilogue staging fits in the patch / weight buffers");
    tile_epilogue_lds<BN, NPASS, TM, TN, !SPLIT, BM, NT>(p, acc, reinterpret_cast<float*>(smem_raw), n0, wm, wn, lane, tid, ks_id, 0, 0, [&](int rr) {
        const int y = y0 + rr / PW, x = x0 + rr % PW;
        return (y < cv.Hout && x < cv.Wout) ? (img * cv.Hout + y) * cv.Wout + x : -1;
    });
}

template <int BN, int NW, int NBS>
static void launch_conv3x3_patch2(const GemmP& p, hipStream_t stream, const char* name) {
    typedef Patch2Geom<BN, NW> G;
    const size_t lds = (size_t)2 * G::PBYTES + (size_t)NBS * G::BBYTES;
    const ConvP& cv = p.conv;
    const int nimg = p.M / (cv.Hout * cv.Wout);
    const int gm = nimg * ((cv.Hout + G::PH - 1) / G::PH) * ((cv.Wout + G::PW - 1) / G::PW);
    dim3 grid(gm * ((p.N + BN - 1) / BN) * (p.splitk > 1 ? p.splitk : 1));
    static bool attr_set = false;
    if (!attr_set) {
        hipFuncSetAttribute(reinterpret_cast<const void*>(&k_conv3x3_patch2<BN, false, NW, NBS>), hipFuncAttributeMaxDynamicSharedMemorySize, (int)lds);
        hipFuncSetAttribute(reinterpret_cast<const void*>(&k_conv3x3_patch2<BN, true, NW, NBS>), hipFuncAttributeMaxDynamicSharedMemorySize, (int)lds);
        attr_set = true;
    }
    static_assert((NW == 8 && BN == 128 && NBS == 4) || (NW == 4 && BN == 64 && NBS == 4) || (NW == 4 && BN == 128 && NBS == 2), "symbol table below");
    const char* sym = NW == 8 ? (p.splitk > 1 && p.ws ? "k_conv3x3_patch2<128, true, 8, 4>" : "k_conv3x3_patch2<128, false, 8, 4>")
                              : (BN == 64 ? (p.splitk > 1 && p.ws ? "k_conv3x3_patch2<64, true, 4, 4>" : "k_conv3x3_patch2<64, false, 4, 4>")
                                          : (p.splitk > 1 && p.ws ? "k_conv3x3_patch2<128, true, 4, 2>" : "k_conv3x3_patch2<128, false, 4, 2>"));
    if (p.splitk > 1 && p.ws)
        DWG_LAUNCH_W(name, sym, gemm_flops(p, 1), (k_conv3x3_patch2<BN, true, NW, NBS>), grid, dim3(NW * 64), lds, stream, p);
    else
        DWG_LAUNCH_W(name, sym, gemm_flops(p, 1), (k_conv3x3_patch2<BN, false, NW, NBS>), grid, dim3(NW * 64), lds, stream, p);
    launch_splitk_epilogue(p, stream);
}

template <typename T, int BN, int AMODE, int BMODE>
static void launch(const GemmP& p, int batch, hipStream_t stream, const char* name) {
    constexpr int LDT = TT<T>::BK + TT<T>::PAD;
    size_t lds = (size_t)2 * (128 + BN) * LDT * sizeof(T);
    dim3 grid((p.M + 127) / 128, ((p.N + BN - 1) / BN) * (p.splitk > 1 ? p.splitk : 1), batch);
    static bool attr_set = false;
    if (!attr_set) {
        hipFuncSetAttribute(reinterpret_cast<const void*>(&k_gemm<T, BN, AMODE, BMODE>), hipFuncAttributeMaxDynamicSharedMemorySize,
                            (int)lds);
        attr_set = true;
    }
    DWG_LAUNCH_W(name, (sizeof(T) == 2 ? "k_gemm<" DWG_HALF_NAME ">" : "k_gemm<f32>"), gemm_flops(p, batch), (k_gemm<T, BN, AMODE, BMODE>), grid,
                 dim3(256), lds, stream, p);
    launch_splitk_epilogue(p, stream);
}

template <typename T, int BN, int AMODE>
static void dispatch_b(const GemmP& p, int bmode, int batch, hipStream_t s, const char* name) {
    if (bmode == MODE_KVEC) launch<T, BN, AMODE, MODE_KVEC>(p, batch, s, name);
    else if (bmode == MODE_RVEC) launch<T, BN, AMODE, MODE_RVEC>(p, batch, s, name);
    else launch<T, BN, AMODE, MODE_SCALAR>(p, batch, s, name);
}
template <typename T, int BN>
static void dispatch_a(const GemmP& p, int amode, int bmode, int batch, hipStream_t s, const char* name) {
    if (amode == MODE_KVEC) dispatch_b<T, BN, MODE_KVEC>(p, bmode, batch, s, name);
    else if (amode == MODE_RVEC) dispatch_b<T, BN, MODE_RVEC>(p, bmode, batch, s, name);
    else if (amode == MODE_CONV) dispatch_b<T, BN, MODE_CONV>(p, bmode, batch, s, name);
    else dispatch_b<T, BN, MODE_SCALAR>(p, bmode, batch, s, name);
}

static int batch_of(const dwg_gemm_desc* d) { return d->batch1 * d->batch2; }

static int tile_bn(const dwg_gemm_desc* d) {
    if (d->N <= 64) return 64;
    const long long blocks128 = (long long)((d->M + 127) / 128) * ((d->N + 127) / 128) * batch_of(d);
    return blocks128 < 256 ? 64 : 128;
}

constexpr int kCUs = 256, kMinWgs = 200;
static bool fills_cus(long long wgs) {
    const long long rounds = (wgs + kCUs - 1) / kCUs;
    return wgs >= kMinWgs && wgs * 100 >= rounds * kCUs * 80;
}

constexpr int kSplitkTarget = 256;
constexpr int kSplitkNoSplit = 384;
constexpr int kSplitkMinSteps = 12;
static int auto_splitk(int M, int N, int K, int bn, int bk) {
    long long blocks = (long long)((M + 127) / 128) * ((N + bn - 1) / bn);
    if (blocks >= kSplitkNoSplit || K < 2 * kSplitkMinSteps * bk) return 1;
    if (2.0 * M * N * K < 4.0e8) return 1;
    long long sk = kSplitkTarget / blocks;
    long long kmax = K / (kSplitkMinSteps * bk);
    if (sk > kmax) sk = kmax;
    if (sk > 16) sk = 16;
    return sk >= 2 ? (int)sk : 1;
}

constexpr int kBigMinK = 1280, kBigMaxTiles = 2048;
constexpr int kBigMinSteps = 8, kBigSkMax = 24;
static int big_tile(int M, int N, int K, int* splitk_out) {
    *splitk_out = 1;
    if (K < kBigMinK) return 0;
    int bm = 0;
    if (M >= 192) { if (N >= 128 && (N % 128 == 0 || N >= 640)) bm = 256; }
    else if (N >= 256) bm = 128;
    if (!bm) return 0;
    const int bn = bm == 256 ? 128 : 256;
    const long long tiles = (long long)((M + bm - 1) / bm) * ((N + bn - 1) / bn);
    if (tiles > kBigMaxTiles) return 0;
    long long sk = 1;
    if (tiles < kCUs) {
        sk = kCUs / tiles;
        const long long kmax = K / (kBigMinSteps * 64);
        if (sk > kmax) sk = kmax;
        if (sk > kBigSkMax) sk = kBigSkMax;
        if (sk < 1) sk = 1;
    }
    if (!fills_cus(tiles * sk)) return 0;
    *splitk_out = (int)sk;
    return bm;
}

template <typename T>
static int pick_mode(const void* base, long long srow, long long sk, int nrows, int K, const long long* boffs, int nboffs) {
    constexpr int VEC = TT<T>::VEC;
    bool aligned = ((uintptr_t)base % 16) == 0;
    for (int i = 0; i < nboffs; i++) aligned = aligned && (boffs[i] % VEC == 0);
    if (sk == 1 && aligned && K % VEC == 0 && srow % VEC == 0) return MODE_KVEC;
    if (srow == 1 && aligned && nrows % VEC == 0 && sk % VEC == 0) return MODE_RVEC;
    return MODE_SCALAR;
}

static int splitk_of(const dwg_gemm_desc* d) {
    if (d->splitk > 1) return d->splitk;
    if (d->splitk != 0 || d->act == DWG_ACT_GEGLU_PAIR) return 1;
    return auto_splitk(d->M, d->N, d->K, tile_bn(d), d->dtype == DWG_DTYPE_HALF ? TT<HT>::BK : TT<float>::BK);
}
static bool slabs_possible(const dwg_gemm_desc* d) { return batch_of(d) == 1 && (long long)d->M * d->N < (1LL << 33); }
static long long fit_workspace(const dwg_gemm_desc* d, long long sk) {
    while (sk > 1 && (size_t)sk * d->M * d->N * sizeof(float) > d->workspace_bytes) sk--;
    return sk;
}

enum Family { FAM_GENERIC, FAM_GLDS, FAM_GLDS8, FAM_PATCH2 };
struct Plan {
    Family fam;
    int bm, bn, nw;
    int amode, bmode;
    int akind;
    int splitk;
    bool slabs;
};

constexpr int kPatchMinM = 8192;
constexpr int kPatch8MinSteps = 100;

static int make_plan(const dwg_gemm_desc* d, const GemmP& p, Plan& pl) {
    const bool half = d->dtype == DWG_DTYPE_HALF;
#if defined(DWG_GEMM_F16_TU) || defined(DWG_GEMM_X_TU)
    if (!half) return DWG_E_ARG;
#endif
    pl = Plan{FAM_GENERIC, 128, tile_bn(d), 4, MODE_KVEC, MODE_KVEC, 0, d->splitk > 1 ? d->splitk : 1, false};
    if (d->workspace && slabs_possible(d)) {
        pl.splitk = (int)fit_workspace(d, splitk_of(d));
        pl.slabs = pl.splitk > 1;
    }
    const long long ao[2] = {p.bA1, p.bA2}, bo[2] = {p.bB1, p.bB2};
    if (p.conv.enabled) {
        const int vec = half ? TT<HT>::VEC : TT<float>::VEC;
        if (d->conv_cin % vec != 0 || ((uintptr_t)d->A % 16) != 0) return DWG_E_ARG;
        if (d->A2 && (d->conv_cin1 % vec != 0 || d->conv_cin1 <= 0 || d->conv_cin1 >= d->conv_cin || ((uintptr_t)d->A2 % 16) != 0))
            return DWG_E_ARG;
        if (d->K != d->conv_kh * d->conv_kw * d->conv_cin) return DWG_E_ARG;
        pl.amode = MODE_CONV;
    } else {
        pl.amode = half ? pick_mode<HT>(p.A, p.sam, p.sak, p.M, p.K, ao, 2) : pick_mode<float>(p.A, p.sam, p.sak, p.M, p.K, ao, 2);
    }
    pl.bmode = half ? pick_mode<HT>(p.B, p.sbn, p.sbk, p.N, p.K, bo, 2) : pick_mode<float>(p.B, p.sbn, p.sbk, p.N, p.K, bo, 2);
    if (!half) return DWG_OK;
    if (pl.bmode != MODE_KVEC || (pl.amode != MODE_KVEC && pl.amode != MODE_CONV)) {
#ifdef DWG_GEMM_X_TU
        return DWG_E_ARG;
#else
        return DWG_OK;
#endif
    }
    const ConvP& cv = p.conv;
    const char* minm = getenv("DWG_CONV_PATCH_MINM");
    const int patch_min_m = minm ? atoi(minm) : kPatchMinM;
    const bool patch_geom = pl.amode == MODE_CONV && batch_of(d) == 1 && d->conv_kh == 3 && d->conv_kw == 3 && d->conv_stride == 1 &&
                            cv.dil == 1 && cv.up == 1 && d->conv_pad_t == 1 && d->conv_pad_l == 1 && !d->A2 && d->conv_cin % 64 == 0 &&
                            d->conv_hout == d->conv_hin && d->conv_wout == d->conv_win && d->conv_wout >= 16 && d->conv_hout >= 8;
    const int ncc = d->conv_cin / 64;
    if (patch_geom && d->splitk <= 1 && d->conv_hout % 16 == 0 && d->conv_wout % 16 == 0 && (d->N % 128 == 0 || d->N >= 512)) {
        const long long tiles8 = (long long)(d->M / 256) * ((d->N + 127) / 128);
        long long sk = 1;
        if (tiles8 < kMinWgs && d->workspace && d->splitk == 0 && slabs_possible(d)) {
            sk = kCUs / tiles8;
            if (sk > ncc / 2) sk = ncc / 2;
            sk = fit_workspace(d, sk);
            if (sk < 1) sk = 1;
            const long long per = (ncc + sk - 1) / sk;
            sk = (ncc + per - 1) / per;
        }
        const long long steps = (ncc + sk - 1) / sk * 9;
        const bool worth = sk > 1 || steps >= kPatch8MinSteps || d->M < patch_min_m;
        if (worth && fills_cus(tiles8 * sk) && (d->act == 0 || d->act == 3 || sk > 1)) {
            pl = Plan{FAM_PATCH2, 256, 128, 8, MODE_CONV, pl.bmode, 0, (int)sk, sk > 1};
            return DWG_OK;
        }
    }
    if (patch_geom && d->M >= patch_min_m && (d->act == 0 || d->act == 3 || pl.splitk > 1)) {
        if (pl.splitk > 1) {
            const int gm = (d->M / (d->conv_hout * d->conv_wout)) * ((d->conv_hout + 7) / 8) * ((d->conv_wout + 15) / 16);
            const int blocks = gm * ((d->N + pl.bn - 1) / pl.bn);
            int sk = blocks >= 256 ? 1 : (384 + blocks - 1) / blocks;
            if (sk > ncc / 2) sk = ncc / 2;
            if (sk > pl.splitk) sk = pl.splitk;
            if (sk < 2) sk = 1;
            pl.splitk = sk;
            pl.slabs = pl.slabs && sk > 1;
        }
        pl.fam = FAM_PATCH2;
        return DWG_OK;
    }
    const bool fast_geom = pl.amode == MODE_CONV && d->conv_cin % 64 == 0 && cv.dil == 1 && cv.up == 1 && d->conv_kh * d->conv_kw <= 32;
    const bool cat_fast = d->A2 && d->conv_cin1 % 64 == 0 && (d->conv_cin - d->conv_cin1) % 64 == 0;
    pl.akind = pl.amode != MODE_CONV ? 0 : (fast_geom && !d->A2 ? 2 : (fast_geom && cat_fast ? 3 : 1));
    int big_sk = 1;
    const int big_bm = d->splitk <= 1 ? big_tile(d->M, d->N, d->K, &big_sk) : 0;
    if (big_bm) {
        if (d->act == DWG_ACT_GEGLU_PAIR || !d->workspace || !slabs_possible(d) || d->splitk == 1) big_sk = 1;
        big_sk = (int)fit_workspace(d, big_sk);
        const int bbn = big_bm == 256 ? 128 : 256;
        const long long tiles = (long long)((d->M + big_bm - 1) / big_bm) * ((d->N + bbn - 1) / bbn) * batch_of(d);
        if (fills_cus(tiles * big_sk)) {
            pl = Plan{FAM_GLDS8, big_bm, bbn, 8, pl.amode, pl.bmode, pl.akind, big_sk, big_sk > 1};
            return DWG_OK;
        }
    }
    pl.fam = FAM_GLDS;
    return DWG_OK;
}

template <typename T>
static void launch_generic(const GemmP& p, const Plan& pl, int batch, hipStream_t s, const char* name) {
    if (pl.bn == 64) dispatch_a<T, 64>(p, pl.amode, pl.bmode, batch, s, name);
    else dispatch_a<T, 128>(p, pl.amode, pl.bmode, batch, s, name);
}
template <typename F>
static void with_akind(int akind, F f) {
    if (akind == 3) f(std::integral_constant<int, 3>{});
    else if (akind == 2) f(std::integral_constant<int, 2>{});
    else if (akind == 1) f(std::integral_constant<int, 1>{});
    else f(std::integral_constant<int, 0>{});
}

}

#ifdef DWG_GEMM_X_TU
static bool x_physical(const dwg_gemm_desc* d, dwg_gemm_desc* o) {
    if (!d) return false;
    *o = *d;
    if (d->dtype != DWG_DTYPE_F32X) return false;
    if (d->K % 8 || d->a_k_stride != 1 || d->b_k_stride != 1) return false;
    if ((d->a_row_stride | d->b_row_stride | d->a_batch1_stride | d->a_batch2_stride | d->b_batch1_stride | d->b_batch2_stride) % 8) return false;
    if (d->out_dtype == DWG_DTYPE_F32X && ((d->ldc | d->c_batch1_stride | d->c_batch2_stride) % 8 || ((uintptr_t)d->C % 16))) return false;
    if (d->residual && d->residual_dtype == DWG_DTYPE_F32X &&
        (((d->ldr ? d->ldr : d->ldc) | d->r_batch1_stride | d->r_batch2_stride) % 8 || ((uintptr_t)d->residual % 16))) return false;
    if (d->act == DWG_ACT_GEGLU_PAIR && d->out_dtype == DWG_DTYPE_F32X && d->N % 16) return false;
    if (d->conv_enabled && (d->conv_cin % 8 || (d->A2 && d->conv_cin1 % 8))) return false;
    o->K = 2 * d->K;
    o->a_row_stride = 2 * d->a_row_stride; o->b_row_stride = 2 * d->b_row_stride;
    o->a_batch1_stride = 2 * d->a_batch1_stride; o->a_batch2_stride = 2 * d->a_batch2_stride;
    o->b_batch1_stride = 2 * d->b_batch1_stride; o->b_batch2_stride = 2 * d->b_batch2_stride;
    o->conv_cin = 2 * d->conv_cin; o->conv_cin1 = 2 * d->conv_cin1;
    return true;
}
#endif

extern "C" {

#if defined(DWG_GEMM_X_TU)
#define DWG_GEMM_FN dwg_gemm_x
#define DWG_GEMM_WS_FN dwg_gemm_workspace_bytes_x
#elif defined(DWG_GEMM_F16_TU)
#define DWG_GEMM_FN dwg_gemm_f16
#define DWG_GEMM_WS_FN dwg_gemm_workspace_bytes_f16
#else
#define DWG_GEMM_FN dwg_gemm
#define DWG_GEMM_WS_FN dwg_gemm_workspace_bytes
size_t dwg_gemm_workspace_bytes_f16(const dwg_gemm_desc* d);
int dwg_gemm_f16(const dwg_gemm_desc* d, dwg_stream_t stream);
size_t dwg_gemm_workspace_bytes_x(const dwg_gemm_desc* d);
int dwg_gemm_x(const dwg_gemm_desc* d, dwg_stream_t stream);
#endif

size_t DWG_GEMM_WS_FN(const dwg_gemm_desc* d) {
#if !defined(DWG_GEMM_F16_TU) && !defined(DWG_GEMM_X_TU)
    if (d && d->dtype == DWG_DTYPE_F16) return dwg_gemm_workspace_bytes_f16(d);
    if (d && d->dtype == DWG_DTYPE_F32X) return dwg_gemm_workspace_bytes_x(d);
#endif
#ifdef DWG_GEMM_X_TU
    dwg_gemm_desc xd;
    if (!x_physical(d, &xd)) return 0;
    d = &xd;
#endif
    if (!d || d->M <= 0 || d->N <= 0 || !slabs_possible(d)) return 0;
    dwg_gemm_desc pd = *d;
    if (d->plan_m > d->M) pd.M = d->plan_m;
    d = &pd;
    int sk = splitk_of(d);
    if (d->dtype == DWG_DTYPE_HALF && d->splitk == 0 && d->act != DWG_ACT_GEGLU_PAIR) {
        int bsk = 1;
        if (big_tile(d->M, d->N, d->K, &bsk) && bsk > sk) sk = bsk;
    }
    return sk > 1 ? (size_t)sk * d->M * d->N * sizeof(float) : 0;
}

int DWG_GEMM_FN(const dwg_gemm_desc* d, dwg_stream_t stream_) {
#if !defined(DWG_GEMM_F16_TU) && !defined(DWG_GEMM_X_TU)
    if (d && d->dtype == DWG_DTYPE_F16) return dwg_gemm_f16(d, stream_);
    if (d && d->dtype == DWG_DTYPE_F32X) return dwg_gemm_x(d, stream_);
#endif
#ifdef DWG_GEMM_X_TU
    dwg_gemm_desc xd;
    if (!x_physical(d, &xd)) return DWG_E_ARG;
    d = &xd;
#endif
    if (!d || !d->A || !d->B || !d->C) return DWG_E_ARG;
    if (d->M < 0 || d->N < 0 || d->K < 0 || d->batch1 < 1 || d->batch2 < 1 || d->plan_m < 0) return DWG_E_ARG;
    if (d->M == 0 || d->N == 0) return DWG_OK;
    if (d->dtype != DWG_DTYPE_F32 && d->dtype != DWG_DTYPE_HALF) return DWG_E_ARG;
    if (d->splitk > 1 && !d->workspace && (d->out_dtype != DWG_DTYPE_F32 || d->bias || d->residual || d->act)) return DWG_E_ARG;
    if (d->accumulate && d->out_dtype != DWG_DTYPE_F32) return DWG_E_ARG;
    if (d->act == DWG_ACT_GEGLU_PAIR && (d->N % 64 != 0 || d->residual || d->splitk > 1 || d->bias_per_row || d->bias_row_div)) return DWG_E_ARG;
    if ((uintptr_t)d->workspace & 15) return DWG_E_ARG;
    GemmP p;
    p.A = d->A; p.B = d->B; p.C = d->C; p.bias = d->bias; p.residual = d->residual;
    p.M = d->M; p.N = d->N; p.K = d->K;
    p.sam = d->a_row_stride; p.sak = d->a_k_stride; p.sbn = d->b_row_stride; p.sbk = d->b_k_stride;
    p.ldc = d->ldc; p.ldr = d->ldr ? d->ldr : d->ldc;
    p.nb2 = d->batch2;
    p.bA1 = d->a_batch1_stride; p.bA2 = d->a_batch2_stride; p.bB1 = d->b_batch1_stride; p.bB2 = d->b_batch2_stride;
    p.bC1 = d->c_batch1_stride; p.bC2 = d->c_batch2_stride; p.bR1 = d->r_batch1_stride; p.bR2 = d->r_batch2_stride;
    p.act = d->act; p.alpha = d->alpha;
    p.out_bf16 = d->out_dtype == DWG_DTYPE_HALF; p.res_bf16 = d->residual_dtype == DWG_DTYPE_HALF;
    p.bias_per_row = d->bias_per_row; p.accumulate = d->accumulate;
    const bool plain1x1 = d->conv_enabled && d->conv_kh == 1 && d->conv_kw == 1 && d->conv_stride == 1 && d->conv_pad_t == 0 &&
                          d->conv_pad_l == 0 && d->conv_in_dilation <= 1 && d->conv_in_upsample <= 1 && !d->A2 && d->conv_hout == d->conv_hin &&
                          d->conv_wout == d->conv_win && d->K == d->conv_cin && batch_of(d) == 1;
    if (plain1x1) { p.sam = d->conv_cin; p.sak = 1; }
    p.conv.enabled = d->conv_enabled && !plain1x1;
    p.conv.Cin = d->conv_cin; p.conv.Hin = d->conv_hin; p.conv.Win = d->conv_win; p.conv.Hout = d->conv_hout;
    p.conv.Wout = d->conv_wout; p.conv.KH = d->conv_kh; p.conv.KW = d->conv_kw; p.conv.stride = d->conv_stride;
    p.conv.pad_t = d->conv_pad_t; p.conv.pad_l = d->conv_pad_l; p.conv.dil = d->conv_in_dilation > 1 ? d->conv_in_dilation : 1;
    p.conv.up = d->conv_in_upsample > 1 ? d->conv_in_upsample : 1;
    p.conv.A2 = d->A2; p.conv.cin1 = d->A2 ? d->conv_cin1 : d->conv_cin;
    p.bias_row_div = d->bias_row_div; p.bias_ld = d->bias_ld > 0 ? d->bias_ld : d->N;
    Plan pl;
    dwg_gemm_desc pd = *d;
    if (d->plan_m > d->M) pd.M = d->plan_m;
    const int rc = make_plan(&pd, p, pl);
    if (rc != DWG_OK) return rc;
    p.splitk = pl.splitk;
    p.ws = pl.slabs ? reinterpret_cast<float*>(d->workspace) : nullptr;
    const int batch = batch_of(d);
    hipStream_t stream = (hipStream_t)stream_;
    const char* name = d->name ? d->name : (d->conv_enabled ? "conv_igemm" : "gemm");
    switch (pl.fam) {
        case FAM_PATCH2:
            if (pl.nw == 8) launch_conv3x3_patch2<128, 8, 4>(p, stream, name);
            else if (pl.bn == 64) launch_conv3x3_patch2<64, 4, 4>(p, stream, name);
            else launch_conv3x3_patch2<128, 4, 2>(p, stream, name);
            break;
        case FAM_GLDS8:
            with_akind(pl.akind, [&](auto ak) {
                if (pl.bm == 256) launch_glds8<256, 128, decltype(ak)::value>(p, batch, stream, name);
                else launch_glds8<128, 256, decltype(ak)::value>(p, batch, stream, name);
            });
            break;
        case FAM_GLDS:
            with_akind(pl.akind, [&](auto ak) {
                if (pl.bn == 64) launch_glds<64, decltype(ak)::value>(p, batch, stream, name);
                else launch_glds<128, decltype(ak)::value>(p, batch, stream, name);
            });
            break;
        case FAM_GENERIC:
#if defined(DWG_GEMM_X_TU)
            return DWG_E_ARG;
#elif defined(DWG_GEMM_F16_TU)
            launch_generic<HT>(p, pl, batch, stream, name);
#else
            if (d->dtype == DWG_DTYPE_HALF) launch_generic<HT>(p, pl, batch, stream, name);
            else launch_generic<float>(p, pl, batch, stream, name);
#endif
            break;
    }
    DWG_RETURN_IF_LAUNCH_FAILED();
    return DWG_OK;
}

}
```

### dreamwaltz-g_amd/csrc/nn_norm.hip

```cpp
#include "dwg_common.h"
#include "dwg_prof_internal.h"
#include "../../include/dwg_nn.h"
#include "dwg_xfmt.h"

namespace {

template <typename T> using vec8 = T __attribute__((ext_vector_type(8)));

template <typename T> struct V8 {
    vec8<T> v;
    __device__ __forceinline__ static V8 load(const T* p) { V8 r; r.v = *reinterpret_cast<const vec8<T>*>(p); return r; }
    __device__ __forceinline__ void store(T* p) const { *reinterpret_cast<vec8<T>*>(p) = v; }
    __device__ __forceinline__ float get(int e) const { return (float)v[e]; }
    __device__ __forceinline__ void set(int e, float z) { v[e] = (T)z; }
};
template <> struct V8<dwg_xs> {
    dwg_x8 v;
    __device__ __forceinline__ static V8 load(const dwg_xs* p) { V8 r; r.v = dwg_x8::load(p); return r; }
    __device__ __forceinline__ void store(dwg_xs* p) const { v.store(p); }
    __device__ __forceinline__ float get(int e) const { return v.get(e); }
    __device__ __forceinline__ void set(int e, float z) { v.set(e, z); }
};
template <typename T> __device__ __forceinline__ float ld1(const T* row, long long j) { return (float)row[j]; }
template <typename T> __device__ __forceinline__ void st1(T* row, long long j, float v) { row[j] = (T)v; }
// ... 385 lines not shown
    float s = 0.f;
#pragma unroll
    for (int it = 0; it < 4; it++) {
        int cc = lane + it * 64;
        if (cc < C8) {
            V8<T> xv = V8<T>::load(x + (size_t)row * C + (size_t)cc * 8);
#pragma unroll
            for (int e = 0; e < 8; e++) { v[it][e] = xv.get(e); s += v[it][e]; }
        }
    }
    s = dwg_wave_sum_all(s);
    const float mean = s / C;
    float q = 0.f;
#pragma unroll
    for (int it = 0; it < 4; it++) {
        int cc = lane + it * 64;
        if (cc < C8) {
#pragma unroll
            for (int e = 0; e < 8; e++) { float d = v[it][e] - mean; q += d * d; }
        }
    }
    q = dwg_wave_sum_all(q);
    const float rstd = rsqrtf(q / C + eps);
#pragma unroll
    for (int it = 0; it < 4; it++) {
        int cc = lane + it * 64;
        if (cc < C8) {
            V8<T> o;
#pragma unroll
            for (int e = 0; e < 8; e++) { int ch = cc * 8 + e; o.set(e, (v[it][e] - mean) * rstd * gamma[ch] + beta[ch]); }
            o.store(y + (size_t)row * C + (size_t)cc * 8);
        }
    }
}

template <typename T>
__global__ __launch_bounds__(256) void k_geglu(long long M, int F, const T* __restrict__ x, T* __restrict__ out) {
    const int F8 = F / 8;
    const long long n = M * F8;
    for (long long i = (long long)blockIdx.x * 256 + threadIdx.x; i < n; i += (long long)gridDim.x * 256) {
        long long m = i / F8; int fc = (int)(i % F8);
        V8<T> a = V8<T>::load(x + m * 2 * F + (size_t)fc * 8);
        V8<T> g = V8<T>::load(x + m * 2 * F + F + (size_t)fc * 8);
        V8<T> o;
#pragma unroll
        for (int e = 0; e < 8; e++) {
            float gv = g.get(e);
            o.set(e, a.get(e) * 0.5f * gv * (1.f + dwg_erf_fast(gv * 0.70710678118654752f)));
        }
        o.store(out + m * F + (size_t)fc * 8);
    }
}

template <typename T>
__global__ __launch_bounds__(256) void k_softmax_rows(int rows, int n, float scale, const float* __restrict__ S, long long lds_,
                                                      T* __restrict__ P, long long ldp) {
    const int row = blockIdx.x * 4 + (threadIdx.x >> 6), lane = threadIdx.x & 63;
    if (row >= rows) return;
    const float* s = S + (size_t)row * lds_;
    float mx = -3.0e38f;
    for (int j = lane; j < n; j += 64) mx = fmaxf(mx, s[j] * scale);
    for (int o = 32; o > 0; o >>= 1) mx = fmaxf(mx, __shfl_xor(mx, o));
    float sum = 0.f;
    for (int j = lane; j < n; j += 64) sum += __expf(s[j] * scale - mx);
    sum = dwg_wave_sum_all(sum);
    const float inv = 1.f / sum;
    T* p = P + (size_t)row * ldp;
    for (int j = lane; j < n; j += 64) st1<T>(p, j, __expf(s[j] * scale - mx) * inv);
}

template <typename T>
__global__ __launch_bounds__(256) void k_softmax_rows_bwd(int rows, int n, float scale, const T* __restrict__ P, long long ldp,
                                                          const float* __restrict__ dP, long long lddp, T* __restrict__ dS,
                                                          long long ldds) {
    const int row = blockIdx.x * 4 + (threadIdx.x >> 6), lane = threadIdx.x & 63;
    if (row >= rows) return;
    const T* p = P + (size_t)row * ldp; const float* dp = dP + (size_t)row * lddp;
    float dot = 0.f;
    for (int j = lane; j < n; j += 64) dot += ld1<T>(p, j) * dp[j];
    dot = dwg_wave_sum_all(dot);
    T* ds = dS + (size_t)row * ldds;
    for (int j = lane; j < n; j += 64) st1<T>(ds, j, scale * ld1<T>(p, j) * (dp[j] - dot));
}

static int gn_geometry(int HW, int C, int G, int* pix_per_block, int* chunks, size_t* lds) {
    if (C % 8 || G <= 0 || G > 64 || C % G) return DWG_E_ARG;
    int ppb = HW / 256; if (ppb < 16) ppb = 16; if (ppb > 256) ppb = 256;
    *pix_per_block = ppb; *chunks = dwg_cdiv(HW, ppb);
    *lds = (size_t)256 * 8 * 2 * sizeof(float);
    return DWG_OK;
}
#define GN_MAX_CHUNKS 2048
#define GN_FOLD_MAX_CHUNKS 32
static void gn_reduce_geometry(int HW, int C, int* pix_per_block, int* chunks) {
    long long ppb = 16384 / C; if (ppb < 8) ppb = 8;
    int ch = (int)((HW + ppb - 1) / ppb);
    if (ch > GN_MAX_CHUNKS) { ch = GN_MAX_CHUNKS; ppb = (HW + ch - 1) / ch; ch = (int)((HW + ppb - 1) / ppb); }
    *pix_per_block = (int)ppb; *chunks = ch;
}
static bool gn_fold(int rchunks, int G) { return rchunks <= GN_FOLD_MAX_CHUNKS && 2 * G * 4 <= 256; }

}

#define DWG_DT_SWITCH(DT, ...)                                                           \
    switch (DT) {                                                                        \
        case DWG_DTYPE_BF16: { typedef __bf16 T; __VA_ARGS__; } break;                   \
        case DWG_DTYPE_F16: { typedef _Float16 T; __VA_ARGS__; } break;                  \
        case DWG_DTYPE_F32: { typedef float T; __VA_ARGS__; } break;                     \
        case DWG_DTYPE_F32X: { typedef dwg_xs T; __VA_ARGS__; } break;                   \
        default: return DWG_E_ARG;                                                       \
    }

extern "C" {

size_t dwg_groupnorm_workspace_floats(int32_t B, int32_t G) { return (size_t)(B > 0 ? B : 1) * GN_MAX_CHUNKS * (G > 0 ? G : 1) * 2; }

int dwg_groupnorm_forward_dt(int32_t dtype, int32_t B, int32_t HW, int32_t C, int32_t G, const void* x, const float* gamma, const float* beta,
                             float eps, int32_t fuse_silu, void* y, float* stats, float* workspace, dwg_stream_t stream_) {
    if (B <= 0 || HW <= 0 || !x || !gamma || !beta || !y || !stats || !workspace) return DWG_E_ARG;
    int ppb, chunks; size_t lds;
    int rc = gn_geometry(HW, C, G, &ppb, &chunks, &lds);
    if (rc) return rc;
    int rppb, rchunks;
    gn_reduce_geometry(HW, C, &rppb, &rchunks);
    hipStream_t stream = (hipStream_t)stream_;
    {
        const int cg = C / G;
        int gb = 0;
        for (int c = 1; c <= 8 && !gb; c *= 2) if ((c * cg) % 8 == 0 && G % c == 0) gb = c;
        const int small_max = 6144;
        const long long tensor_bytes = (long long)B * HW * C * (dtype == DWG_DTYPE_F32 || dtype == DWG_DTYPE_F32X ? 4 : 2);
        if (gb && B <= 4 && HW <= 1024 && (long long)HW * (gb * cg / 8) <= small_max && gb * cg / 8 <= 64 && tensor_bytes <= (8ll << 20)) {
            const int nb = gb * cg, tp = 256 / (nb / 8);
            const size_t sl = (size_t)(2 * tp * nb + 2 * nb) * sizeof(float);
            DWG_DT_SWITCH(dtype,
                DWG_LAUNCH("gn_small", (k_gn_small<T>), dim3(G / gb, B), dim3(256), sl, stream, HW, C, G, gb, (const T*)x, gamma, beta, fuse_silu,
                           eps, (T*)y, stats))
            DWG_RETURN_IF_LAUNCH_FAILED();
            return DWG_OK;
        }
    }
    const bool fold = gn_fold(rchunks, G);
    DWG_DT_SWITCH(dtype,
        DWG_LAUNCH("gn_stats", (k_gn_reduce<T, false>), dim3(rchunks, B), dim3(256), lds, stream, HW, C, G, rppb, (const T*)x,
                   (const T*)nullptr, (const float*)nullptr, gamma, beta, 0, eps, workspace);
        if (!fold) DWG_LAUNCH("gn_finalize", k_gn_finalize, dim3((2 * G + 3) / 4, B), dim3(256), 0, stream, rchunks, G, (const float*)workspace, stats);
        DWG_LAUNCH("gn_apply", (k_gn_apply<T, false>), dim3(chunks, B), dim3(256), 0, stream, HW, C, G, ppb, (const T*)x,
                   (const T*)nullptr, (const float*)stats, (const float*)nullptr, gamma, beta, fuse_silu, eps, (T*)y,
                   fold ? (const float*)workspace : (const float*)nullptr, rchunks, stats, (const T*)nullptr))
    DWG_RETURN_IF_LAUNCH_FAILED();
    return DWG_OK;
}

int dwg_groupnorm_forward(int32_t B, int32_t HW, int32_t C, int32_t G, const void* x, const float* gamma, const float* beta,
                          float eps, int32_t fuse_silu, void* y, float* stats, float* workspace, dwg_stream_t stream) {
    return dwg_groupnorm_forward_dt(DWG_DTYPE_BF16, B, HW, C, G, x, gamma, beta, eps, fuse_silu, y, stats, workspace, stream);
}

int dwg_groupnorm_backward_dt(int32_t dtype, int32_t B, int32_t HW, int32_t C, int32_t G, const void* x, const void* dy, const float* stats,
                              const float* gamma, const float* beta, float eps, int32_t fuse_silu, void* dx, float* scratch,
                              float* workspace, const void* residual, dwg_stream_t stream_) {
    if (B <= 0 || HW <= 0 || !x || !dy || !stats || !gamma || !beta || !dx || !scratch || !workspace) return DWG_E_ARG;
    int ppb, chunks; size_t lds;
    int rc = gn_geometry(HW, C, G, &ppb, &chunks, &lds);
    if (rc) return rc;
    int rppb, rchunks;
    gn_reduce_geometry(HW, C, &rppb, &rchunks);
    hipStream_t stream = (hipStream_t)stream_;
    const bool fold = gn_fold(rchunks, G);
    DWG_DT_SWITCH(dtype,
        DWG_LAUNCH("gn_bwd_stats", (k_gn_reduce<T, true>), dim3(rchunks, B), dim3(256), lds, stream, HW, C, G, rppb, (const T*)x,
                   (const T*)dy, stats, gamma, beta, fuse_silu, eps, workspace);
        if (!fold) DWG_LAUNCH("gn_finalize", k_gn_finalize, dim3((2 * G + 3) / 4, B), dim3(256), 0, stream, rchunks, G, (const float*)workspace, scratch);
        DWG_LAUNCH("gn_bwd_apply", (k_gn_apply<T, true>), dim3(chunks, B), dim3(256), 0, stream, HW, C, G, ppb, (const T*)x,
                   (const T*)dy, stats, (const float*)scratch, gamma, beta, fuse_silu, eps, (T*)dx,
                   fold ? (const float*)workspace : (const float*)nullptr, rchunks, scratch, (const T*)residual))
    DWG_RETURN_IF_LAUNCH_FAILED();
    return DWG_OK;
}

int dwg_groupnorm_backward(int32_t B, int32_t HW, int32_t C, int32_t G, const void* x, const void* dy, const float* stats,
                           const float* gamma, const float* beta, float eps, int32_t fuse_silu, void* dx, float* scratch,
                           float* workspace, const void* residual, dwg_stream_t stream) {
    return dwg_groupnorm_backward_dt(DWG_DTYPE_BF16, B, HW, C, G, x, dy, stats, gamma, beta, eps, fuse_silu, dx, scratch, workspace, residual,
                                     stream);
}

int dwg_layernorm_forward_dt(int32_t dtype, int32_t M, int32_t C, const void* x, const float* gamma, const float* beta, float eps, void* y,
                             dwg_stream_t stream) {
    if (M < 0 || C <= 0 || C % 8 || C > 2048 || !x || !gamma || !beta || !y) return DWG_E_ARG;
    if (M == 0) return DWG_OK;
    DWG_DT_SWITCH(dtype, DWG_LAUNCH("layernorm", k_layernorm<T>, dim3(dwg_cdiv(M, 4)), dim3(256), 0, (hipStream_t)stream, M, C, (const T*)x,
                                    gamma, beta, eps, (T*)y))
    DWG_RETURN_IF_LAUNCH_FAILED();
    return DWG_OK;
}

int dwg_layernorm_forward(int32_t M, int32_t C, const void* x, const float* gamma, const float* beta, float eps, void* y,
                          dwg_stream_t stream) {
    return dwg_layernorm_forward_dt(DWG_DTYPE_BF16, M, C, x, gamma, beta, eps, y, stream);
}

int dwg_geglu_forward_dt(int32_t dtype, int64_t M, int32_t F, const void* x, void* out, dwg_stream_t stream) {
    if (M < 0 || F <= 0 || F % 8 || !x || !out) return DWG_E_ARG;
    if (M == 0) return DWG_OK;
    long long n = M * (F / 8);
    int blocks = (int)((n + 255) / 256); if (blocks > 4096) blocks = 4096;
    DWG_DT_SWITCH(dtype, DWG_LAUNCH("geglu", k_geglu<T>, dim3(blocks), dim3(256), 0, (hipStream_t)stream, (long long)M, F, (const T*)x, (T*)out))
    DWG_RETURN_IF_LAUNCH_FAILED();
    return DWG_OK;
}

int dwg_geglu_forward(int64_t M, int32_t F, const void* x, void* out, dwg_stream_t stream) {
    return dwg_geglu_forward_dt(DWG_DTYPE_BF16, M, F, x, out, stream);
}

int dwg_softmax_rows_forward_dt(int32_t dtype, int32_t rows, int32_t n, float scale, const float* S, int64_t lds, void* P, int64_t ldp,
                                dwg_stream_t stream) {
    if (rows < 0 || n <= 0 || !S || !P) return DWG_E_ARG;
    if (rows == 0) return DWG_OK;
    DWG_DT_SWITCH(dtype, DWG_LAUNCH("softmax_rows", k_softmax_rows<T>, dim3(dwg_cdiv(rows, 4)), dim3(256), 0, (hipStream_t)stream, rows, n, scale,
                                    S, (long long)lds, (T*)P, (long long)ldp))
    DWG_RETURN_IF_LAUNCH_FAILED();
    return DWG_OK;
}

int dwg_softmax_rows_forward(int32_t rows, int32_t n, float scale, const float* S, int64_t lds, void* P, int64_t ldp,
                             dwg_stream_t stream) {
    return dwg_softmax_rows_forward_dt(DWG_DTYPE_BF16, rows, n, scale, S, lds, P, ldp, stream);
}

int dwg_softmax_rows_backward_dt(int32_t dtype, int32_t rows, int32_t n, float scale, const void* P, int64_t ldp, const float* dP, int64_t lddp,
                                 void* dS, int64_t ldds, dwg_stream_t stream) {
    if (rows < 0 || n <= 0 || !P || !dP || !dS) return DWG_E_ARG;
    if (rows == 0) return DWG_OK;
    DWG_DT_SWITCH(dtype, DWG_LAUNCH("softmax_rows_bwd", k_softmax_rows_bwd<T>, dim3(dwg_cdiv(rows, 4)), dim3(256), 0, (hipStream_t)stream, rows, n,
                                    scale, (const T*)P, (long long)ldp, dP, (long long)lddp, (T*)dS, (long long)ldds))
    DWG_RETURN_IF_LAUNCH_FAILED();
    return DWG_OK;
}

int dwg_softmax_rows_backward(int32_t rows, int32_t n, float scale, const void* P, int64_t ldp, const float* dP, int64_t lddp,
                              void* dS, int64_t ldds, dwg_stream_t stream) {
    return dwg_softmax_rows_backward_dt(DWG_DTYPE_BF16, rows, n, scale, P, ldp, dP, lddp, dS, ldds, stream);
}

}
```

### dreamwaltz-g_amd/gemm.py

```python
import ctypes

import torch

from . import _lib

F32, BF16, F16, F32X = 0, 1, 2, 3
ACT = {None: 0, "none": 0, "relu": 1, "leaky_relu": 2, "silu": 3, "gelu": 4, "sigmoid": 5, "geglu_pair": 6}


class GemmDesc(ctypes.Structure):
    _fields_ = [
        ("A", ctypes.c_void_p), ("B", ctypes.c_void_p), ("C", ctypes.c_void_p), ("bias", ctypes.c_void_p),
        ("residual", ctypes.c_void_p),
        ("M", ctypes.c_int32), ("N", ctypes.c_int32), ("K", ctypes.c_int32),
        ("a_row_stride", ctypes.c_int64), ("a_k_stride", ctypes.c_int64), ("b_row_stride", ctypes.c_int64),
        ("b_k_stride", ctypes.c_int64), ("ldc", ctypes.c_int64), ("ldr", ctypes.c_int64),
        ("batch1", ctypes.c_int32), ("batch2", ctypes.c_int32),
        ("a_batch1_stride", ctypes.c_int64), ("a_batch2_stride", ctypes.c_int64), ("b_batch1_stride", ctypes.c_int64),
        ("b_batch2_stride", ctypes.c_int64), ("c_batch1_stride", ctypes.c_int64), ("c_batch2_stride", ctypes.c_int64),
        ("r_batch1_stride", ctypes.c_int64), ("r_batch2_stride", ctypes.c_int64),
        ("dtype", ctypes.c_int32), ("out_dtype", ctypes.c_int32), ("residual_dtype", ctypes.c_int32),
        ("act", ctypes.c_int32), ("alpha", ctypes.c_float), ("bias_per_row", ctypes.c_int32),
        ("splitk", ctypes.c_int32), ("accumulate", ctypes.c_int32),
        ("conv_enabled", ctypes.c_int32), ("conv_cin", ctypes.c_int32), ("conv_hin", ctypes.c_int32),
        ("conv_win", ctypes.c_int32), ("conv_hout", ctypes.c_int32), ("conv_wout", ctypes.c_int32),
        ("conv_kh", ctypes.c_int32), ("conv_kw", ctypes.c_int32), ("conv_stride", ctypes.c_int32),
        ("conv_pad_t", ctypes.c_int32), ("conv_pad_l", ctypes.c_int32), ("conv_in_dilation", ctypes.c_int32),
        ("conv_in_upsample", ctypes.c_int32), ("A2", ctypes.c_void_p), ("conv_cin1", ctypes.c_int32),
        ("bias_row_div", ctypes.c_int32), ("bias_ld", ctypes.c_int64),
        ("workspace", ctypes.c_void_p), ("workspace_bytes", ctypes.c_size_t),
        ("name", ctypes.c_char_p), ("plan_m", ctypes.c_int32),
    ]


def _dt(t):
    if t.dtype == torch.float32:
        return F32
    if t.dtype == torch.bfloat16:
        return BF16
    if t.dtype == torch.float16:
        return F16
    if t.dtype == torch.int32:
        return F32X
    raise TypeError("dwg gemm supports float32, bfloat16, float16 and f32x (int32-typed, xfmt.py) tensors, got %s" % t.dtype)


def _stream(t):
    return ctypes.c_void_p(torch.cuda.current_stream(t.device).cuda_stream)


def gemm_raw(A, B, C, M, N, K, a_strides, b_strides, ldc, bias=None, residual=None, ldr=0, act=None, alpha=1.0,
             batch=(1, 1), a_batch=(0, 0), b_batch=(0, 0), c_batch=(0, 0), r_batch=(0, 0), bias_per_row=False, splitk=1,
             accumulate=False, conv=None, name=None, conv_upsample=1, A2=None, cin1=0, bias_row_div=0, bias_ld=0, plan_m=0, run=True):
    if not A.is_cuda:
        raise RuntimeError("dreamwaltz_g_amd GEMM runs on the GPU only (HIP kernels)")
    d = GemmDesc()
    d.A, d.B, d.C = A.data_ptr(), B.data_ptr(), C.data_ptr()
    d.bias = bias.data_ptr() if bias is not None else None
    d.residual = residual.data_ptr() if residual is not None else None
    d.M, d.N, d.K = M, N, K
    d.a_row_stride, d.a_k_stride = a_strides
    d.b_row_stride, d.b_k_stride = b_strides
    d.ldc, d.ldr = ldc, ldr
    d.batch1, d.batch2 = batch
    d.a_batch1_stride, d.a_batch2_stride = a_batch
    d.b_batch1_stride, d.b_batch2_stride = b_batch
    d.c_batch1_stride, d.c_batch2_stride = c_batch
    d.r_batch1_stride, d.r_batch2_stride = r_batch
    d.dtype = _dt(A)
    assert _dt(B) == d.dtype, "A and B must share a dtype"
    d.out_dtype = _dt(C)
    d.residual_dtype = _dt(residual) if residual is not None else F32
    d.act = ACT[act]
    d.alpha = alpha
    d.bias_per_row = int(bias_per_row)
    d.splitk = splitk
    d.accumulate = int(accumulate)
    if conv is not None:
        d.conv_enabled = 1
        (d.conv_cin, d.conv_hin, d.conv_win, d.conv_hout, d.conv_wout, d.conv_kh, d.conv_kw, d.conv_stride, d.conv_pad_t,
         d.conv_pad_l, d.conv_in_dilation) = conv
    d.conv_in_upsample = conv_upsample
    if A2 is not None:
        d.A2 = A2.data_ptr(); d.conv_cin1 = cin1
    d.bias_row_div = bias_row_div
    d.bias_ld = bias_ld
    d.name = name.encode() if name else None
    d.plan_m = plan_m
    if not run:
        return d
    _lib.check(_lib.lib().dwg_gemm(ctypes.byref(d), _stream(A)), "dwg_gemm")
    return C


def run_desc(d, stream):
    rc = _lib.lib().dwg_gemm(ctypes.byref(d), stream)
    if rc != 0:
        raise RuntimeError("dwg_gemm failed with DWG error %d" % rc)


def linear(x, w, bias=None, act=None, out_dtype=None, residual=None, out=None, name=None):
    K = x.shape[-1]
    x2 = x.reshape(-1, K)
    M, N = x2.shape[0], w.shape[0]
    out_dtype = out_dtype or x.dtype
    y = out if out is not None else torch.empty(M, N, device=x.device, dtype=out_dtype)
    r2 = None if residual is None else residual.reshape(M, N)
    gemm_raw(x2, w, y, M, N, K, (x2.stride(0), x2.stride(1)), (w.stride(0), w.stride(1)), y.stride(0), bias=bias, residual=r2,
             ldr=0 if r2 is None else r2.stride(0), act=act, name=name)
    return y.reshape(*x.shape[:-1], N)


def conv2d_nhwc(x, w, bias=None, stride=1, pad=(1, 1), act=None, residual=None, out_hw=None, in_dilation=1, out_dtype=None,
                name=None):
    Bn, H, W, Cin = x.shape
    Cout, KH, KW, _ = w.shape
    Hv, Wv = (H - 1) * in_dilation + 1, (W - 1) * in_dilation + 1
    if out_hw is None:
        Ho = (Hv + 2 * pad[0] - KH) // stride + 1
        Wo = (Wv + 2 * pad[1] - KW) // stride + 1
    else:
        Ho, Wo = out_hw
    y = torch.empty(Bn, Ho, Wo, Cout, device=x.device, dtype=out_dtype or x.dtype)
    M, N, K = Bn * Ho * Wo, Cout, KH * KW * Cin
    gemm_raw(x, w, y, M, N, K, (0, 1), (K, 1), Cout, bias=bias, residual=residual, ldr=Cout if residual is not None else 0,
             act=act, conv=(Cin, H, W, Ho, Wo, KH, KW, stride, pad[0], pad[1], in_dilation), name=name)
    return y
```

### dreamwaltz-g_amd/sd15.py

```python
import ctypes
import os
import math
from collections import OrderedDict
from dataclasses import dataclass
from typing import Dict, List, Optional, Tuple

import torch

from . import _lib, gemm, xfmt

BF16 = torch.bfloat16

TORCH_DTYPE = {"bf16": torch.bfloat16, "f32": torch.float32, "f16": torch.float16, "f32x": xfmt.DTYPE}
DT_CODE = {"f32": 0, "bf16": 1, "f16": 2, "f32x": 3}


def dtype_name(dtype) -> str:
    names = {"bf16": "bf16", "bfloat16": "bf16", torch.bfloat16: "bf16", "f32": "f32", "fp32": "f32", "float32": "f32", torch.float32: "f32",
             "f16": "f16", "fp16": "f16", "float16": "f16", "half": "f16", torch.float16: "f16", "f32x": "f32x", "fp32x": "f32x"}
    if dtype not in names:
        raise ValueError("plan dtype must be one of bf16 / f32 / f16 / f32x, got %r" % (dtype,))
    return names[dtype]


# ... 352 lines not shown
        _lib.prof_enable(False)
        self.run_eager()
        torch.cuda.synchronize(self.device)
        self._cap_stream = torch.cuda.Stream(device=self.device)
        s = ctypes.c_void_p(self._cap_stream.cuda_stream)
        _lib.check(self._lib.dwg_graph_begin_capture(s), "dwg_graph_begin_capture")
        try:
            self._issue(s)
        finally:
            h = ctypes.c_void_p()
            rc = self._lib.dwg_graph_end_capture(s, ctypes.byref(h))
        _lib.check(rc, "dwg_graph_end_capture")
        self.graph = h

    def run(self):
        if self.graph is not None and self.use_graph:
            cur = torch.cuda.current_stream(self.device).cuda_stream
            if cur == 0:
                self.run_eager()
                return
            _lib.check(self._lib.dwg_graph_launch(self.graph, ctypes.c_void_p(cur)), "dwg_graph_launch")
        else:
            self.run_eager()

    def run_debug(self):
        s = ctypes.c_void_p(torch.cuda.current_stream(self.device).cuda_stream)
        bufs = [t for t in self.keep if torch.is_tensor(t) and t.is_floating_point()]
        for i, op in enumerate(self.ops):
            rc = 0 if op[0] == "fork" else op[1](s)
            torch.cuda.synchronize()
            bad = [tuple(t.shape) for t in bufs if not torch.isfinite(t.float()).all()]
            if rc or bad:
                return i, rc, bad
        return None


class Weights:

    def __init__(self, sd: Dict[str, torch.Tensor], device, dtype="bf16"):
        self.device = device
        self.sd = sd
        self.cache = {}
        self.wdtype = TORCH_DTYPE[dtype_name(dtype)]
        self.is_x = dtype_name(dtype) == "f32x"

    def _to_dev(self, w):
        if self.is_x:
            a = w.abs()
            r = self.__dict__.setdefault("range", {"elements": 0, "saturated": 0, "subnormal": 0, "max_abs": 0.0})
            r["elements"] += a.numel(); r["saturated"] += int((a >= xfmt.X_MAX).sum()); r["subnormal"] += int(((a < 6.1035e-5) & (a > 0)).sum())
            r["max_abs"] = max(r["max_abs"], float(a.max()) if a.numel() else 0.0)
            return xfmt.pack(w.to(self.device)).contiguous()
        return w.to(self.device, self.wdtype).contiguous()

    def conv(self, name, flip_for_dgrad=False):
        key = (name, flip_for_dgrad)
        if key not in self.cache:
            w = self.sd[name + ".weight"].float()
            if flip_for_dgrad:
                w = w.flip(2, 3).permute(1, 0, 2, 3)
            cout, cin = w.shape[0], w.shape[1]
            wp = torch.zeros(_pad8(cout) if flip_for_dgrad else cout, w.shape[2], w.shape[3], _pad8(cin))
            wp[:cout, :, :, :cin] = w.permute(0, 2, 3, 1)
            self.cache[key] = self._to_dev(wp)
        return self.cache[key]

    def conv_dgrad_s2(self, name, py, px):
        key = ("dgrad_s2", name, py, px)
        if key not in self.cache:
            w = self.sd[name + ".weight"].float()
            kmap = {0: [2, 0], 1: [1]}
            kys, kxs = kmap[py], kmap[px]
            cy, cx = w.shape[0], w.shape[1]
            wp = torch.zeros(_pad8(cx), len(kys), len(kxs), _pad8(cy))
            for ty, ky in enumerate(kys):
                for tx, kx in enumerate(kxs):
                    wp[:cx, ty, tx, :cy] = w[:, :, ky, kx].t()
            self.cache[key] = self._to_dev(wp)
        return self.cache[key]

    def lin(self, *names):
        key = ("lin",) + names
        if key not in self.cache:
            self.cache[key] = self._to_dev(torch.cat([self.sd[n + ".weight"].float().reshape(self.sd[n + ".weight"].shape[0], -1)
                                                      for n in names], 0))
        return self.cache[key]

    def lin_t(self, name):
        key = ("lin_t", name)
        if key not in self.cache:
            w = self.sd[name + ".weight"].float()
            self.cache[key] = self._to_dev(w.reshape(w.shape[0], -1).t().contiguous())
        return self.cache[key]

    def lin_geglu(self, name):
        key = ("geglu", name)
        if key not in self.cache:
            w = self.sd[name + ".weight"].float(); b = self.sd[name + ".bias"].float()
            F = w.shape[0] // 2
            idx = torch.arange(F).view(-1, 32)
            perm = torch.cat([idx, idx + F], dim=1).reshape(-1)
            self.cache[key] = (self._to_dev(w[perm]), b[perm].to(self.device).contiguous())
        return self.cache[key]

    def f32(self, name):
        if name not in self.cache:
            self.cache[name] = self.sd[name].float().to(self.device).contiguous()
        return self.cache[name]

    def bias_cat(self, *names):
        key = ("bias",) + names
        if key not in self.cache:
            self.cache[key] = torch.cat([self.sd[n].float() for n in names], 0).to(self.device).contiguous()
        return self.cache[key]


class Builder:
    def __init__(self, plan: Plan, w: Weights, groups=32, prefix="net"):
        self.p, self.w, self.groups, self.prefix = plan, w, groups, prefix
        self.L = _lib.lib()
        self.full_batch = None

    def _plan_rows(self, b, m):
        return m * self.full_batch // b if self.full_batch and b < self.full_batch and self.full_batch % b == 0 else 0

    def _conv_tag(self, tag, KH, Ho, stride, dil, KW=None):
        if tag:
            return tag
        KW = KH if KW is None else KW
        base = "conv3x3" if KH == 3 else ("conv1x1" if KH * KW == 1 else "conv%dx%d" % (KH, KW))
        return "%s%s_%s_r%d" % (base, "s2" if stride == 2 else ("T" if dil > 1 else ""), self.prefix, Ho)

    def conv(self, x, name, stride=1, pad=1, act=None, residual=None, upsample=1, bias_img=None, out_dtype=None, out_hw=None,
             pad_tl=None, r_batch_bcast=False, weight=None, bias=True, in_dilation=1, tag=None):
        B, H, W, C = x.shape
        self.p.scope = name
        wt = self.w.conv(name) if weight is None else weight
        Cout, KH, KW, Cin = wt.shape
        assert Cin == C, (name, Cin, C)
        Hv, Wv = ((H - 1) * in_dilation + 1) * upsample, ((W - 1) * in_dilation + 1) * upsample
        pt, pl = (pad, pad) if pad_tl is None else pad_tl
        if out_hw is None:
            Ho, Wo = (Hv + 2 * pad - KH) // stride + 1, (Wv + 2 * pad - KW) // stride + 1
        else:
            Ho, Wo = out_hw
        y = self.p.buf(B, Ho, Wo, Cout, dtype=out_dtype)
        b = None
        if bias_img is None and bias:
            b = self.w.f32(name + ".bias")
            if b.numel() < Cout:
                b = None
        conv = (C, H, W, Ho, Wo, KH, KW, stride, pt, pl, in_dilation)
        K = KH * KW * C
        if r_batch_bcast and KH * KW == 1 and stride == 1 and pad == 0 and pad_tl is None and upsample == 1 and in_dilation == 1 and out_hw is None:
            Vr = int(residual.shape[0])
            assert B % Vr == 0 and bias_img is None, (B, Vr)
            Mr = Vr * H * W
            d = gemm.gemm_raw(x, wt, y, Mr, Cout, K, (C, 1), (K, 1), Cout, bias=b, residual=residual, ldr=Cout, act=act, batch=(B // Vr, 1),
                              a_batch=(Mr * C, 0), c_batch=(Mr * Cout, 0), r_batch=(0, 0), name=self._conv_tag(tag, KH, Ho, stride, in_dilation, KW),
                              run=False)
        elif r_batch_bcast:
            Vr = int(residual.shape[0])
            assert B % Vr == 0, (B, Vr)
            d = gemm.gemm_raw(x, wt, y, Ho * Wo, Cout, K, (0, 1), (K, 1), Cout, bias=b, residual=residual, ldr=Cout, act=act,
                              batch=(B // Vr, Vr), a_batch=(Vr * H * W * C, H * W * C), c_batch=(Vr * Ho * Wo * Cout, Ho * Wo * Cout),
                              r_batch=(0, Ho * Wo * Cout), conv=conv,
                              conv_upsample=upsample, name=self._conv_tag(tag, KH, Ho, stride, in_dilation, KW), run=False)
        else:
            kw = {}
            if bias_img is not None:
                kw = dict(bias=bias_img[0], bias_row_div=Ho * Wo, bias_ld=bias_img[1])
            else:
                kw = dict(bias=b)
            d = gemm.gemm_raw(x, wt, y, B * Ho * Wo, Cout, K, (0, 1), (K, 1), Cout, residual=residual,
                              ldr=Cout if residual is not None else 0, act=act, conv=conv, conv_upsample=upsample,
                              name=self._conv_tag(tag, KH, Ho, stride, in_dilation, KW), plan_m=self._plan_rows(B, B * Ho * Wo), run=False, **kw)
        self.p.add_gemm(d)
        return y

    def linear(self, x, wt, bias=None, act=None, residual=None, out_dtype=None, tag="linear"):
        K = x.shape[-1]
        M = x.numel() // K
        N = wt.shape[0]
        Nout = N // 2 if act == "geglu_pair" else N
        y = self.p.buf(*x.shape[:-1], Nout, dtype=out_dtype)
        if residual is not None and residual.numel() != M * Nout:
            R = (M * Nout) // residual.numel()
            Mr = M // R
            assert Mr * R == M and residual.numel() == Mr * Nout and x.is_contiguous(), (M, Nout, tuple(residual.shape))
            d = gemm.gemm_raw(x, wt, y, Mr, N, K, (K, 1), (wt.stride(0), 1), Nout, bias=bias, residual=residual, ldr=Nout, act=act, batch=(R, 1),
                              a_batch=(Mr * K, 0), c_batch=(Mr * Nout, 0), r_batch=(0, 0), name=tag, run=False)
            self.p.add_gemm(d)
            return y
        d = gemm.gemm_raw(x, wt, y, M, N, K, (K, 1), (wt.stride(0), 1), Nout, bias=bias, residual=residual,
                          ldr=Nout if residual is not None else 0, act=act, name=tag, plan_m=self._plan_rows(x.shape[0], M) if x.dim() > 2 else 0,
                          run=False)
        self.p.add_gemm(d)
        return y

    def _gn_ws(self, B):
        need = int(self.L.dwg_groupnorm_workspace_floats(B, self.groups))
        pool = self.p.__dict__.setdefault("_gn_workspace", {})
        ws = pool.get(self.p.branch)
        if ws is None or ws.numel() < need:
            ws = self.p.buf(need, dtype=torch.float32)
            pool[self.p.branch] = ws
        return ws

    def groupnorm(self, x, name, eps, silu, keep_stats=False):
        self.p.scope = name
        B, C = x.shape[0], x.shape[-1]
        HW = x.numel() // (B * C)
        y = self.p.buf(*x.shape)
        stats = self.p.buf(B, self.groups, 2, dtype=torch.float32)
        pp = lambda t: ctypes.c_void_p(t.data_ptr())
        self.p.add_call(self.L.dwg_groupnorm_forward_dt, self.p.dt, B, HW, C, self.groups, pp(x), pp(self.w.f32(name + ".weight")),
                        pp(self.w.f32(name + ".bias")), eps, int(silu), pp(y), pp(stats), pp(self._gn_ws(B)))
        return (y, stats) if keep_stats else y

    def groupnorm_bwd(self, x, dy, stats, name, eps, silu, residual=None):
        B, C = x.shape[0], x.shape[-1]
        HW = x.numel() // (B * C)
        dx = self.p.buf(*x.shape)
        scratch = self.p.buf(B, self.groups, 2, dtype=torch.float32)
        pp = lambda t: ctypes.c_void_p(t.data_ptr())
        self.p.add_call(self.L.dwg_groupnorm_backward_dt, self.p.dt, B, HW, C, self.groups, pp(x), pp(dy), pp(stats),
                        pp(self.w.f32(name + ".weight")), pp(self.w.f32(name + ".bias")), eps, int(silu), pp(dx), pp(scratch),
                        pp(self._gn_ws(B)), pp(residual) if residual is not None else None)
        return dx

    def layernorm(self, x, name):
        self.p.scope = name
        C = x.shape[-1]
        M = x.numel() // C
        y = self.p.buf(*x.shape)
        pp = lambda t: ctypes.c_void_p(t.data_ptr())
        self.p.add_call(self.L.dwg_layernorm_forward_dt, self.p.dt, M, C, pp(x), pp(self.w.f32(name + ".weight")), pp(self.w.f32(name + ".bias")),
                        1e-5, pp(y))
        return y

    def geglu(self, x):
        F2 = x.shape[-1]
        M = x.numel() // F2
        y = self.p.buf(*x.shape[:-1], F2 // 2)
        pp = lambda t: ctypes.c_void_p(t.data_ptr())
        self.p.add_call(self.L.dwg_geglu_forward_dt, self.p.dt, M, F2 // 2, pp(x), pp(y))
        return y

    def _pooled(self, tag, numel, dtype):
        pool = self.p.__dict__.setdefault("_scratch_pool", {})
        key = (tag, self.p.branch, dtype)
        t = pool.get(key)
        if t is None or t.numel() < numel:
            t = pool[key] = self.p.buf(numel, dtype=dtype)
        return t[:numel]

    def attention(self, q, k, v, heads):
        Bq, Nq, HD = q.shape
        B, Nk, d = k.shape[0], k.shape[1], HD // heads
        o = self.p.buf(B, Nq, HD)
        pp = lambda t: ctypes.c_void_p(t.data_ptr())
        if B != Bq:
            R = B // Bq
            assert R * Bq == B and v.shape[0] == B, (B, Bq)
            if self.p.dtype_name == "f32":
                raise NotImplementedError("the exact-f32 plans run attention on dwg_gemm, whose two batch levels are image x head")
            need = int(self.L.dwg_attention_split_workspace_bytes(self.p.dt, B, heads, Nq, Nk, d))
            ws = self.p.buf((need + 3) // 4, dtype=torch.float32) if need > 0 else None
            self.p.add_call(self.L.dwg_attention_forward_pairs_ws, self.p.dt, R, Bq, heads, Nq, Nk, d, pp(q), q.stride(1), q.stride(0), 0,
                            pp(k), k.stride(1), k.stride(0), Bq * k.stride(0), pp(v), v.stride(1), v.stride(0), Bq * v.stride(0),
                            pp(o), o.stride(1), o.stride(0), Bq * o.stride(0), float(d) ** -0.5, pp(ws) if ws is not None else None, need)
            return o
        if self.p.dtype_name == "f32":
            S = self._pooled("attn_S", B * heads * Nq * Nk, torch.float32)
            P = self._pooled("attn_P", B * heads * Nq * Nk, self.p.dtype)
            self.p.add_gemm(gemm.gemm_raw(q, k, S, Nq, Nk, d, (q.stride(1), 1), (k.stride(1), 1), Nk, batch=(B, heads),
                                          a_batch=(q.stride(0), d), b_batch=(k.stride(0), d), c_batch=(heads * Nq * Nk, Nq * Nk),
                                          name="attn_qk", run=False))
            self.p.add_call(self.L.dwg_softmax_rows_forward_dt, self.p.dt, B * heads * Nq, Nk, float(d) ** -0.5, pp(S), Nk, pp(P), Nk)
            self.p.add_gemm(gemm.gemm_raw(P, v, o, Nq, d, Nk, (Nk, 1), (1, v.stride(1)), HD, batch=(B, heads),
                                          a_batch=(heads * Nq * Nk, Nq * Nk), b_batch=(v.stride(0), d), c_batch=(o.stride(0), d),
                                          name="attn_pv", run=False))
            return o
        need = int(self.L.dwg_attention_split_workspace_bytes(self.p.dt, B, heads, Nq, Nk, d))
        if need > 0:
            ws = self.p.buf((need + 3) // 4, dtype=torch.float32)
            self.p.add_call(self.L.dwg_attention_forward_ws, self.p.dt, B, heads, Nq, Nk, d, pp(q), q.stride(1), q.stride(0), pp(k), k.stride(1),
                            k.stride(0), pp(v), v.stride(1), v.stride(0), pp(o), o.stride(1), o.stride(0), float(d) ** -0.5, pp(ws), need)
            return o
        self.p.add_call(self.L.dwg_attention_forward_dt, self.p.dt, B, heads, Nq, Nk, d, pp(q), q.stride(1), q.stride(0), pp(k), k.stride(1),
                        k.stride(0), pp(v), v.stride(1), v.stride(0), pp(o), o.stride(1), o.stride(0), float(d) ** -0.5)
        return o

    def cat(self, a, b):
        Ca, Cb = a.shape[-1], b.shape[-1]
        y = self.p.buf(*a.shape[:-1], Ca + Cb)
        pp = lambda t: ctypes.c_void_p(t.data_ptr())
        k2 = self.p.esize // 2
        if b.shape[0] != a.shape[0]:
            assert a.shape[0] % b.shape[0] == 0 and a.shape[1:-1] == b.shape[1:-1], (tuple(a.shape), tuple(b.shape))
            self.p.add_call(self.L.dwg_concat_channels_bcast, a.numel() // Ca, b.numel() // Cb, Ca * k2, Cb * k2, pp(a), pp(b), pp(y))
            return y
        self.p.add_call(self.L.dwg_concat_channels, a.numel() // Ca, Ca * k2, Cb * k2, pp(a), pp(b), pp(y))
        return y

    def add(self, a, b):
        y = self.p.buf(*a.shape)
        pp = lambda t: ctypes.c_void_p(t.data_ptr())
        self.p.add_call(self.L.dwg_add_dt, self.p.dt, a.numel(), pp(a), pp(b), pp(y))
        return y

    def conv_dgrad_s2(self, dy, name):
        B, Ho, Wo, _ = dy.shape
        subs = []
        for py in (0, 1):
            for px in (0, 1):
                wt = self.w.conv_dgrad_s2(name, py, px)
                subs.append(self.conv(dy, None, weight=wt, bias=False, stride=1, pad_tl=(wt.shape[1] - 1, wt.shape[2] - 1),
                                      out_hw=(Ho, Wo)))
        C = subs[0].shape[-1]
        out = self.p.buf(B, 2 * Ho, 2 * Wo, C)
        pp = lambda t: ctypes.c_void_p(t.data_ptr())
        self.p.add_call(self.L.dwg_interleave2x2, B, Ho, Wo, C * (self.p.esize // 2), pp(subs[0]), pp(subs[1]), pp(subs[2]), pp(subs[3]), pp(out))
        return out

    def transpose(self, x):
        B, R, C = x.shape
        y = self.p.buf(B, C, R)
        pp = lambda t: ctypes.c_void_p(t.data_ptr())
        self.p.add_call(self.L.dwg_transpose_dt, self.p.dt, B, R, C, pp(x), x.stride(1), x.stride(0), pp(y), R, C * R)
        return y

    def cast_bf16(self, x):
        if self.p.dtype_name == "f32":
            return x
        y = self.p.buf(*x.shape)
        pp = lambda t: ctypes.c_void_p(t.data_ptr())
        self.p.add_call(self.L.dwg_cast_f32_to_dt, self.p.dt, x.numel(), pp(x), pp(y))
        return y

    def resnet(self, x, pre, temb_bias, eps=1e-5):
        self.p.scope = pre
        C = x.shape[-1]
        n1 = self.groupnorm(x, pre + ".norm1", eps, True)
        h1 = self.conv(n1, pre + ".conv1", bias_img=temb_bias)
        n2 = self.groupnorm(h1, pre + ".norm2", eps, True)
        Cout = h1.shape[-1]
        sc = x if C == Cout else self.conv(x, pre + ".conv_shortcut", pad=0)
        return self.conv(n2, pre + ".conv2", residual=sc)

    def text_kv(self, text, t):
        batches = self.__dict__.setdefault("_text_kv", {})
        key = text.data_ptr()
        if key not in batches:
            suffix = ".attn2.to_k.weight"
            blocks = sorted(n[:-len(suffix)] for n in self.w.sd if n.endswith(suffix) and self.w.sd[n].shape[1] == text.shape[-1])
            names = []
            for b_ in blocks:
                names += [b_ + ".attn2.to_k", b_ + ".attn2.to_v"]
            out = self.linear(text, self.w.lin(*names), tag="attn_kv")
            offs, o = {}, 0
            for b_ in blocks:
                c = int(self.w.sd[b_ + suffix].shape[0])
                offs[b_] = (o, c); o += 2 * c
            batches[key] = (out, offs, text)
        ent = batches[key]
        if t not in ent[1]:
            return self.linear(text, self.w.lin(t + ".attn2.to_k", t + ".attn2.to_v"), tag="attn_kv")
# ... 398 lines not shown
```

### include/dwg_gemm.h

```cpp
#ifndef DWG_GEMM_H
#define DWG_GEMM_H
#include "dwg_types.h"
#ifdef __cplusplus
extern "C" {
#endif


#define DWG_ACT_NONE 0
#define DWG_ACT_RELU 1
#define DWG_ACT_LEAKY_RELU 2
#define DWG_ACT_SILU 3
#define DWG_ACT_GELU 4
#define DWG_ACT_SIGMOID 5
#define DWG_ACT_GEGLU_PAIR 6

typedef struct dwg_gemm_desc {
    const void* A; const void* B; void* C;
    const float* bias;
    const void* residual;
    int32_t M, N, K;
    int64_t a_row_stride, a_k_stride, b_row_stride, b_k_stride, ldc, ldr;
    int32_t batch1, batch2;
    int64_t a_batch1_stride, a_batch2_stride, b_batch1_stride, b_batch2_stride, c_batch1_stride, c_batch2_stride,
        r_batch1_stride, r_batch2_stride;
    int32_t dtype;
    int32_t out_dtype;
    int32_t residual_dtype;
    int32_t act;
    float alpha;
    int32_t bias_per_row;
    int32_t splitk;
    int32_t accumulate;
    int32_t conv_enabled, conv_cin, conv_hin, conv_win, conv_hout, conv_wout, conv_kh, conv_kw, conv_stride, conv_pad_t,
        conv_pad_l, conv_in_dilation;
    int32_t conv_in_upsample;
    const void* A2;
    int32_t conv_cin1;
    int32_t bias_row_div;
    int64_t bias_ld;
    void* workspace;
    size_t workspace_bytes;
    const char* name;
    int32_t plan_m;
} dwg_gemm_desc;

int dwg_gemm(const dwg_gemm_desc* desc, dwg_stream_t stream);

size_t dwg_gemm_workspace_bytes(const dwg_gemm_desc* desc);

#ifdef __cplusplus
}
#endif
#endif
```

### include/dwg_nn.h

```cpp
#ifndef DWG_NN_H
#define DWG_NN_H
#include "dwg_types.h"
#ifdef __cplusplus
extern "C" {
#endif

int dwg_groupnorm_forward(int32_t B, int32_t HW, int32_t C, int32_t G, const void* x, const float* gamma, const float* beta,
                          float eps, int32_t fuse_silu, void* y, float* stats, float* workspace, dwg_stream_t stream);
size_t dwg_groupnorm_workspace_floats(int32_t B, int32_t G);

int dwg_groupnorm_backward(int32_t B, int32_t HW, int32_t C, int32_t G, const void* x, const void* dy, const float* stats,
                           const float* gamma, const float* beta, float eps, int32_t fuse_silu, void* dx, float* scratch,
                           float* workspace, const void* residual, dwg_stream_t stream);

int dwg_layernorm_forward(int32_t M, int32_t C, const void* x, const float* gamma, const float* beta, float eps, void* y,
                          dwg_stream_t stream);

int dwg_geglu_forward(int64_t M, int32_t F, const void* x, void* out, dwg_stream_t stream);

int dwg_attention_forward(int32_t B, int32_t H, int32_t Nq, int32_t Nk, int32_t d, const void* Q, int64_t ldq, int64_t bq,
                          const void* K, int64_t ldk, int64_t bk, const void* V, int64_t ldv, int64_t bv, void* O, int64_t ldo,
                          int64_t bo, float scale, dwg_stream_t stream);

int dwg_softmax_rows_forward(int32_t rows, int32_t n, float scale, const float* S, int64_t lds, void* P, int64_t ldp,
                             dwg_stream_t stream);
int dwg_softmax_rows_backward(int32_t rows, int32_t n, float scale, const void* P, int64_t ldp, const float* dP, int64_t lddp,
                              void* dS, int64_t ldds, dwg_stream_t stream);

int dwg_groupnorm_forward_dt(int32_t dtype, int32_t B, int32_t HW, int32_t C, int32_t G, const void* x, const float* gamma,
                             const float* beta, float eps, int32_t fuse_silu, void* y, float* stats, float* workspace,
                             dwg_stream_t stream);
int dwg_groupnorm_backward_dt(int32_t dtype, int32_t B, int32_t HW, int32_t C, int32_t G, const void* x, const void* dy,
                              const float* stats, const float* gamma, const float* beta, float eps, int32_t fuse_silu, void* dx,
                              float* scratch, float* workspace, const void* residual, dwg_stream_t stream);
int dwg_layernorm_forward_dt(int32_t dtype, int32_t M, int32_t C, const void* x, const float* gamma, const float* beta, float eps,
                             void* y, dwg_stream_t stream);
int dwg_geglu_forward_dt(int32_t dtype, int64_t M, int32_t F, const void* x, void* out, dwg_stream_t stream);
int dwg_attention_forward_dt(int32_t dtype, int32_t B, int32_t H, int32_t Nq, int32_t Nk, int32_t d, const void* Q, int64_t ldq,
                             int64_t bq, const void* K, int64_t ldk, int64_t bk, const void* V, int64_t ldv, int64_t bv, void* O,
                             int64_t ldo, int64_t bo, float scale, dwg_stream_t stream);
size_t dwg_attention_split_workspace_bytes(int32_t dtype, int32_t B, int32_t H, int32_t Nq, int32_t Nk, int32_t d);
int dwg_attention_forward_ws(int32_t dtype, int32_t B, int32_t H, int32_t Nq, int32_t Nk, int32_t d, const void* Q, int64_t ldq,
                             int64_t bq, const void* K, int64_t ldk, int64_t bk, const void* V, int64_t ldv, int64_t bv, void* O,
                             int64_t ldo, int64_t bo, float scale, void* workspace, size_t workspace_bytes, dwg_stream_t stream);
int dwg_attention_forward_pairs_dt(int32_t dtype, int32_t R, int32_t Bq, int32_t H, int32_t Nq, int32_t Nk, int32_t d, const void* Q, int64_t ldq,
                                   int64_t bq, int64_t oq, const void* K, int64_t ldk, int64_t bk, int64_t ok, const void* V, int64_t ldv,
                                   int64_t bv, int64_t ov, void* O, int64_t ldo, int64_t bo, int64_t oo, float scale, dwg_stream_t stream);
int dwg_attention_forward_pairs_ws(int32_t dtype, int32_t R, int32_t Bq, int32_t H, int32_t Nq, int32_t Nk, int32_t d, const void* Q, int64_t ldq,
                                   int64_t bq, int64_t oq, const void* K, int64_t ldk, int64_t bk, int64_t ok, const void* V, int64_t ldv,
                                   int64_t bv, int64_t ov, void* O, int64_t ldo, int64_t bo, int64_t oo, float scale, void* workspace,
                                   size_t workspace_bytes, dwg_stream_t stream);
int dwg_softmax_rows_forward_dt(int32_t dtype, int32_t rows, int32_t n, float scale, const float* S, int64_t lds, void* P,
                                int64_t ldp, dwg_stream_t stream);
int dwg_softmax_rows_backward_dt(int32_t dtype, int32_t rows, int32_t n, float scale, const void* P, int64_t ldp, const float* dP,
                                 int64_t lddp, void* dS, int64_t ldds, dwg_stream_t stream);

#ifdef __cplusplus
}
#endif
#endif
```

Baseline: 40.54.

## Fuse GroupNorm statistics into GEMM/conv epilogue for f32x producers

Adds a STATS variant of the GEMM and conv3x3 epilogues that accumulates per-channel sum and sum-of-squares as tiles are stored. It reduces them in LDS and writes per-group, per-tile partials to a buffer. A GroupNorm that consumes a tensor produced by such a GEMM (f32x path, HW>1024) then skips its separate statistics pass over x and only finalizes and applies. This removes one full read of the activation per GroupNorm, at the cost of extra epilogue work, more LDS synchronization, and additional kernel instantiations.

```diff
diff --git a/dreamwaltz-g_amd/_lib.py b/dreamwaltz-g_amd/_lib.py
--- a/dreamwaltz-g_amd/_lib.py
+++ b/dreamwaltz-g_amd/_lib.py
@@ -131,6 +131,7 @@
     "dwg_raymarch_composite_rays": (ctypes.c_int, [_u32, _u32, _u32, _f32, _u32, _vp, _vp, _vp, _vp, _vp, _u32, _vp, _vp, _vp, _vp]),
     "dwg_gemm":(ctypes.c_int, [_vp, _vp]),
     "dwg_gemm_workspace_bytes": (_sz, [_vp]),
+    "dwg_gemm_gn_chunks": (_i32, [_vp]),
     "dwg_transpose_2byte": (ctypes.c_int, [_i32, _i32, _i32, _vp, _i64, _i64, _vp, _i64, _i64, _vp]),
     "dwg_transpose_dt": (ctypes.c_int, [_i32, _i32, _i32, _i32, _vp, _i64, _i64, _vp, _i64, _i64, _vp]),
     "dwg_xfmt_pack": (ctypes.c_int, [_i64, _vp, _vp, _vp]),
@@ -164,6 +165,7 @@
     "dwg_softmax_rows_forward": (ctypes.c_int, [_i32, _i32, _f32, _vp, _i64, _vp, _i64, _vp]),
     "dwg_softmax_rows_backward": (ctypes.c_int, [_i32, _i32, _f32, _vp, _i64, _vp, _i64, _vp, _i64, _vp]),
     "dwg_groupnorm_forward_dt": (ctypes.c_int, [_i32, _i32, _i32, _i32, _i32, _vp, _vp, _vp, _f32, _i32, _vp, _vp, _vp, _vp]),
+    "dwg_groupnorm_forward_partials": (ctypes.c_int, [_i32, _i32, _i32, _i32, _i32, _vp, _vp, _vp, _f32, _i32, _vp, _vp, _vp, _i32, _vp]),
     "dwg_groupnorm_backward_dt": (ctypes.c_int, [_i32, _i32, _i32, _i32, _i32, _vp, _vp, _vp, _vp, _vp, _f32, _i32, _vp, _vp, _vp, _vp, _vp]),
     "dwg_layernorm_forward_dt": (ctypes.c_int, [_i32, _i32, _i32, _vp, _vp, _vp, _f32, _vp, _vp]),
     "dwg_geglu_forward_dt": (ctypes.c_int, [_i32, _i64, _i32, _vp, _vp, _vp]),
diff --git a/dreamwaltz-g_amd/csrc/gemm.hip b/dreamwaltz-g_amd/csrc/gemm.hip
--- a/dreamwaltz-g_amd/csrc/gemm.hip
+++ b/dreamwaltz-g_amd/csrc/gemm.hip
@@ -10,6 +10,7 @@
 #define DWG_DTYPE_HALF DWG_DTYPE_F32X
 #define DWG_MFMA16(a, b, c) __builtin_amdgcn_mfma_f32_32x32x16_f16(a, b, c, 0, 0, 0)
 #define DWG_HALF_NAME "f32x"
+#define DWG_GEMM_GN 1
 #elif defined(DWG_GEMM_F16_TU)
 typedef _Float16 HT;
 #define DWG_DTYPE_HALF DWG_DTYPE_F16
@@ -46,6 +47,8 @@
     int bias_row_div;
     long long bias_ld;
     ConvP conv;
+    float* gn;
+    int gn_G, gn_cg, gn_hw, gn_chunks, gn_slots;
 };
 
 __device__ __forceinline__ float bf2f(HT x) { return (float)x; }
@@ -319,11 +322,33 @@
         return lds_bytes >= (size_t)BM * LDC * 4 ? 1 : (lds_bytes >= (size_t)(BM / 2) * LDC * 4 ? 2 : 4);
     }
     static constexpr size_t bytes(int npass) { return (size_t)(BM / npass) * LDC * 4; }
+    static constexpr size_t stats_bytes(int nt) { return ((size_t)nt * 8 + 2 * BN) * 4; }
 };
 
-template <int BN, int NPASS, int TM, int TN, bool LIGHT, int BM = 128, int NT = 256, typename RowFn>
+typedef float f32x2_t __attribute__((ext_vector_type(2)));
+__device__ __forceinline__ void st_half4_r(void* base, long long i, const float (&v)[4], float (&r)[4]) {
+#ifdef DWG_GEMM_X_TU
+    unsigned char* q = reinterpret_cast<unsigned char*>(base) + dwg_x_byte(i);
+    dwg_h4 h, l;
+#pragma unroll
+    for (int e = 0; e < 4; e++) {
+        _Float16 a, b;
+        dwg_x_split(v[e], a, b);
+        h[e] = a; l[e] = b;
+        r[e] = dwg_x_join(a, b);
+    }
+    *reinterpret_cast<dwg_h4*>(q) = h; *reinterpret_cast<dwg_h4*>(q + 16) = l;
+#else
+    bf16x4_t o;
+#pragma unroll
+    for (int e = 0; e < 4; e++) { o.v[e] = f2bf(v[e]); r[e] = bf2f(o.v[e]); }
+    *reinterpret_cast<bf16x4_t*>(reinterpret_cast<HT*>(base) + i) = o;
+#endif
+}
+
+template <int BN, int NPASS, int TM, int TN, bool LIGHT, int BM = 128, int NT = 256, bool STATS = false, typename RowFn>
 __device__ __forceinline__ void tile_epilogue_lds(const GemmP& p, f32x16 (&acc)[TM][TN], float* sC, int n0, int wm, int wn, int lane, int tid,
-                                                  int ks_id, long long coff, long long roff, RowFn row_of) {
+                                                  int ks_id, long long coff, long long roff, RowFn row_of, int gn_img = 0, int gn_tile = 0) {
     constexpr int LDC = EpiLds<BN, BM>::LDC, C4 = BN / 4, PR = BM / NPASS;
     constexpr int BPP = BM / 32 / NPASS;
     static_assert(NT % C4 == 0 && (C4 & (C4 - 1)) == 0, "a thread keeps one column group");
@@ -331,6 +356,7 @@
     const int lrow = lane & 31, lhalf = (lane >> 5) * 4;
     const bool geglu = p.act == 6;
     const float* bias = reinterpret_cast<const float*>(p.bias);
+    f32x2_t gs1a = {0.f, 0.f}, gs1b = {0.f, 0.f}, gs2a = {0.f, 0.f}, gs2b = {0.f, 0.f};
     const bool fast = vec_ok && !geglu && !p.accumulate && !p.bias_per_row && (p.splitk <= 1 || p.ws) &&
                       (!bias || p.bias_row_div > 0 || ((uintptr_t)bias & 15) == 0) &&
                       (!bias || p.bias_row_div <= 0 || (((uintptr_t)bias & 15) == 0 && (p.bias_ld & 3) == 0)) &&
@@ -437,7 +463,14 @@
                         }
                     }
                     const long long ci = coff + (long long)row * p.ldc + col;
-                    if (p.out_bf16) {
+                    if constexpr (STATS) {
+                        float s[4] = {v[0], v[1], v[2], v[3]};
+                        if (p.out_bf16) st_half4_r(p.C, ci, v, s);
+                        else *reinterpret_cast<float4*>(reinterpret_cast<float*>(p.C) + ci) = make_float4(v[0], v[1], v[2], v[3]);
+                        const f32x2_t s01 = {s[0], s[1]}, s23 = {s[2], s[3]};
+                        gs1a += s01; gs1b += s23;
+                        gs2a = __builtin_elementwise_fma(s01, s01, gs2a); gs2b = __builtin_elementwise_fma(s23, s23, gs2b);
+                    } else if (p.out_bf16) {
                         st_half4(p.C, ci, v);
                     } else {
                         *reinterpret_cast<float4*>(reinterpret_cast<float*>(p.C) + ci) = make_float4(v[0], v[1], v[2], v[3]);
@@ -469,6 +502,35 @@
                 continue;
             }
             epilogue_store4<LIGHT>(p, v, row, col, coff, roff, vec_ok);
+        }
+    }
+    if constexpr (STATS) {
+        constexpr int C4 = BN / 4, RT = NT / C4;
+        float* red = sC;
+        float* cs = sC + RT * 2 * BN;
+        const int c4 = tid & (C4 - 1), rl0 = tid / C4;
+        __syncthreads();
+        *reinterpret_cast<float4*>(red + (rl0 * 2 + 0) * BN + c4 * 4) = make_float4(gs1a[0], gs1a[1], gs1b[0], gs1b[1]);
+        *reinterpret_cast<float4*>(red + (rl0 * 2 + 1) * BN + c4 * 4) = make_float4(gs2a[0], gs2a[1], gs2b[0], gs2b[1]);
+        __syncthreads();
+        for (int i = tid; i < 2 * BN; i += NT) {
+            float a = 0.f;
+#pragma unroll 4
+            for (int r = 0; r < RT; r++) a += red[r * 2 * BN + i];
+            cs[i] = a;
+        }
+        __syncthreads();
+        const int cg = p.gn_cg, nend = min(n0 + BN, p.N);
+        const int g_lo = n0 / cg, ng = (nend - 1) / cg - g_lo + 1;
+        if (tid < 2 * ng) {
+            const int g = g_lo + (tid >> 1), st = tid & 1;
+            const int c_lo = max(g * cg, n0) - n0, c_hi = min((g + 1) * cg, nend) - n0;
+            float a = 0.f;
+            for (int c = c_lo; c < c_hi; c++) a += cs[st * BN + c];
+            const int first = (g * cg) / BN, slot = n0 / BN - first;
+            float* dst = p.gn + ((long long)gn_img * 2 * p.gn_G + 2 * g + st) * p.gn_chunks + gn_tile * p.gn_slots;
+            dst[slot] = a;
+            if (p.gn_slots == 2 && slot == 0 && ((g + 1) * cg - 1) / BN == first) dst[1] = 0.f;
         }
     }
 }
@@ -748,7 +810,7 @@
     static constexpr int WN = BN / 64, WM = (BM == 128 && BN == 64) ? 4 : BM / 64, NW = WM * WN, NT = NW * 64, TM = BM / WM / 32, TN = 2;
 };
 
-template <int BM, int BN, int AKIND, int S>
+template <int BM, int BN, int AKIND, int S, bool STATS = false>
 __device__ __forceinline__ void gemm_glds_body(const GemmP& p) {
     typedef GldsGeom<BM, BN> Geo;
     constexpr int WN = Geo::WN, WM = Geo::WM, NW = Geo::NW, NT = Geo::NT, TM = Geo::TM, TN = Geo::TN;
@@ -910,8 +972,10 @@
 #endif
     constexpr int NPASS = EpiLds<BN, BM>::passes((size_t)S * STAGE);
     static_assert((size_t)S * STAGE >= EpiLds<BN, BM>::bytes(NPASS), "epilogue staging fits in the operand stages");
-    tile_epilogue_lds<BN, NPASS, TM, TN, false, BM, NT>(p, acc, reinterpret_cast<float*>(smem_raw), n0, wm, wn, lane, tid, ks_id, z1 * p.bC1 + z2 * p.bC2,
-                                         z1 * p.bR1 + z2 * p.bR2, [&](int rl) { const int r = m0 + rl; return r < p.M ? r : -1; });
+    static_assert(!STATS || (size_t)S * STAGE >= EpiLds<BN, BM>::stats_bytes(NT), "the statistics' reduction fits in the operand stages");
+    tile_epilogue_lds<BN, NPASS, TM, TN, false, BM, NT, STATS>(p, acc, reinterpret_cast<float*>(smem_raw), n0, wm, wn, lane, tid, ks_id, z1 * p.bC1 + z2 * p.bC2,
+                                         z1 * p.bR1 + z2 * p.bR2, [&](int rl) { const int r = m0 + rl; return r < p.M ? r : -1; },
+                                         STATS ? m0 / p.gn_hw : 0, STATS ? (m0 % p.gn_hw) / BM : 0);
 }
 
 template <int BN, int AKIND, int S>
@@ -924,6 +988,17 @@
     static_assert(GldsGeom<BM, BN>::NT == 512, "eight waves");
     gemm_glds_body<BM, BN, AKIND, S>(p);
 }
+
+#ifdef DWG_GEMM_GN
+template <int BN, int AKIND, int S>
+__global__ __launch_bounds__(256, 2) void k_gemm_glds_gn(GemmP p) {
+    gemm_glds_body<128, BN, AKIND, S, true>(p);
+}
+template <int BM, int BN, int AKIND, int S>
+__global__ __launch_bounds__(512, 2) void k_gemm_glds8_gn(GemmP p) {
+    gemm_glds_body<BM, BN, AKIND, S, true>(p);
+}
+#endif
 
 static double gemm_flops(const GemmP& p, int batch) {
     double f = 2.0 * p.M * p.N * p.K * batch;
@@ -944,6 +1019,21 @@
         attr_set = true;
     }
     dim3 grid(((p.M + 127) / 128) * ((p.N + BN - 1) / BN) * (p.splitk > 1 ? p.splitk : 1), 1, batch);
+#ifdef DWG_GEMM_GN
+    if constexpr (AKIND != 3) {
+        if (p.gn) {
+            static bool gn_attr_set = false;
+            if (!gn_attr_set) {
+                hipFuncSetAttribute(reinterpret_cast<const void*>(&k_gemm_glds_gn<BN, AKIND, S>), hipFuncAttributeMaxDynamicSharedMemorySize, (int)lds);
+                gn_attr_set = true;
+            }
+            static const char* const gsym[2][3] = {{"k_gemm_glds_gn<64, 0, 3>", "k_gemm_glds_gn<64, 1, 2>", "k_gemm_glds_gn<64, 2, 3>"},
+                                                   {"k_gemm_glds_gn<128, 0, 2>", "k_gemm_glds_gn<128, 1, 2>", "k_gemm_glds_gn<128, 2, 2>"}};
+            DWG_LAUNCH_W(name, gsym[BN == 128][AKIND], gemm_flops(p, batch), (k_gemm_glds_gn<BN, AKIND, S>), grid, dim3(256), lds, stream, p);
+            return;
+        }
+    }
+#endif
     static const char* const sym[2][4] = {{"k_gemm_glds<64, 0, 3>", "k_gemm_glds<64, 1, 2>", "k_gemm_glds<64, 2, 3>", "k_gemm_glds<64, 3, 3>"},
                                           {"k_gemm_glds<128, 0, 2>", "k_gemm_glds<128, 1, 2>", "k_gemm_glds<128, 2, 2>", "k_gemm_glds<128, 3, 2>"}};
     DWG_LAUNCH_W(name, sym[BN == 128][AKIND], gemm_flops(p, batch), (k_gemm_glds<BN, AKIND, S>), grid, dim3(256), lds, stream, p);
@@ -960,6 +1050,21 @@
         attr_set = true;
     }
     dim3 grid(((p.M + BM - 1) / BM) * ((p.N + BN - 1) / BN) * (p.splitk > 1 ? p.splitk : 1), 1, batch);
+#ifdef DWG_GEMM_GN
+    if constexpr (AKIND != 3) {
+        if (p.gn) {
+            static bool gn_attr_set = false;
+            if (!gn_attr_set) {
+                hipFuncSetAttribute(reinterpret_cast<const void*>(&k_gemm_glds8_gn<BM, BN, AKIND, S>), hipFuncAttributeMaxDynamicSharedMemorySize, (int)lds);
+                gn_attr_set = true;
+            }
+            static const char* const gsym[2][3] = {{"k_gemm_glds8_gn<256, 128, 0, 3>", "k_gemm_glds8_gn<256, 128, 1, 3>", "k_gemm_glds8_gn<256, 128, 2, 3>"},
+                                                   {"k_gemm_glds8_gn<128, 256, 0, 3>", "k_gemm_glds8_gn<128, 256, 1, 3>", "k_gemm_glds8_gn<128, 256, 2, 3>"}};
+            DWG_LAUNCH_W(name, gsym[BN == 256][AKIND], gemm_flops(p, batch), (k_gemm_glds8_gn<BM, BN, AKIND, S>), grid, dim3(512), lds, stream, p);
+            return;
+        }
+    }
+#endif
     static const char* const sym[2][4] = {
         {"k_gemm_glds8<256, 128, 0, 3>", "k_gemm_glds8<256, 128, 1, 3>", "k_gemm_glds8<256, 128, 2, 3>", "k_gemm_glds8<256, 128, 3, 3>"},
         {"k_gemm_glds8<128, 256, 0, 3>", "k_gemm_glds8<128, 256, 1, 3>", "k_gemm_glds8<128, 256, 2, 3>", "k_gemm_glds8<128, 256, 3, 3>"}};
@@ -977,8 +1082,8 @@
     static constexpr int PBYTES = NPI * 8 * 128, BBYTES = BN * 128;
 };
 
-template <int BN, bool SPLIT, int NW, int NBS>
-__global__ __launch_bounds__(NW * 64, 2) void k_conv3x3_patch2(GemmP p) {
+template <int BN, bool SPLIT, int NW, int NBS, bool STATS = false>
+__device__ __forceinline__ void conv3x3_patch2_body(const GemmP& p) {
     typedef Patch2Geom<BN, NW> G;
     constexpr int PH = G::PH, PW = G::PW, WP = G::WP, NPIX = G::NPIX, NPI = G::NPI, PPW = G::PPW;
     constexpr int WN = G::WN, WM = G::WM, TM = G::TM, TN = G::TN, NT = G::NT, NJW = G::NJW, BM = G::BM;
@@ -1194,11 +1299,23 @@
 #endif
     constexpr int NPASS = EpiLds<BN, BM>::passes((size_t)2 * PBYTES + NBS * BBYTES);
     static_assert((size_t)2 * PBYTES + NBS * BBYTES >= EpiLds<BN, BM>::bytes(NPASS), "epilogue staging fits in the patch / weight buffers");
-    tile_epilogue_lds<BN, NPASS, TM, TN, !SPLIT, BM, NT>(p, acc, reinterpret_cast<float*>(smem_raw), n0, wm, wn, lane, tid, ks_id, 0, 0, [&](int rr) {
+    static_assert(!STATS || (!SPLIT && (size_t)2 * PBYTES + NBS * BBYTES >= EpiLds<BN, BM>::stats_bytes(NT)), "the statistics' reduction fits");
+    tile_epilogue_lds<BN, NPASS, TM, TN, !SPLIT, BM, NT, STATS>(p, acc, reinterpret_cast<float*>(smem_raw), n0, wm, wn, lane, tid, ks_id, 0, 0, [&](int rr) {
         const int y = y0 + rr / PW, x = x0 + rr % PW;
         return (y < cv.Hout && x < cv.Wout) ? (img * cv.Hout + y) * cv.Wout + x : -1;
-    });
-}
+    }, img, trem);
+}
+
+template <int BN, bool SPLIT, int NW, int NBS>
+__global__ __launch_bounds__(NW * 64, 2) void k_conv3x3_patch2(GemmP p) {
+    conv3x3_patch2_body<BN, SPLIT, NW, NBS>(p);
+}
+#ifdef DWG_GEMM_GN
+template <int BN, int NW, int NBS>
+__global__ __launch_bounds__(NW * 64, 2) void k_conv3x3_patch2_gn(GemmP p) {
+    conv3x3_patch2_body<BN, false, NW, NBS, true>(p);
+}
+#endif
 
 template <int BN, int NW, int NBS>
 static void launch_conv3x3_patch2(const GemmP& p, hipStream_t stream, const char* name) {
@@ -1218,6 +1335,18 @@
     const char* sym = NW == 8 ? (p.splitk > 1 && p.ws ? "k_conv3x3_patch2<128, true, 8, 4>" : "k_conv3x3_patch2<128, false, 8, 4>")
                               : (BN == 64 ? (p.splitk > 1 && p.ws ? "k_conv3x3_patch2<64, true, 4, 4>" : "k_conv3x3_patch2<64, false, 4, 4>")
                                           : (p.splitk > 1 && p.ws ? "k_conv3x3_patch2<128, true, 4, 2>" : "k_conv3x3_patch2<128, false, 4, 2>"));
+#ifdef DWG_GEMM_GN
+    if (p.gn) {
+        static bool gn_attr_set = false;
+        if (!gn_attr_set) {
+            hipFuncSetAttribute(reinterpret_cast<const void*>(&k_conv3x3_patch2_gn<BN, NW, NBS>), hipFuncAttributeMaxDynamicSharedMemorySize, (int)lds);
+            gn_attr_set = true;
+        }
+        const char* gsym = NW == 8 ? "k_conv3x3_patch2_gn<128, 8, 4>" : (BN == 64 ? "k_conv3x3_patch2_gn<64, 4, 4>" : "k_conv3x3_patch2_gn<128, 4, 2>");
+        DWG_LAUNCH_W(name, gsym, gemm_flops(p, 1), (k_conv3x3_patch2_gn<BN, NW, NBS>), grid, dim3(NW * 64), lds, stream, p);
+        return;
+    }
+#endif
     if (p.splitk > 1 && p.ws)
         DWG_LAUNCH_W(name, sym, gemm_flops(p, 1), (k_conv3x3_patch2<BN, true, NW, NBS>), grid, dim3(NW * 64), lds, stream, p);
     else
@@ -1443,87 +1572,16 @@
     else f(std::integral_constant<int, 0>{});
 }
 
-}
-
-#ifdef DWG_GEMM_X_TU
-static bool x_physical(const dwg_gemm_desc* d, dwg_gemm_desc* o) {
-    if (!d) return false;
-    *o = *d;
-    if (d->dtype != DWG_DTYPE_F32X) return false;
-    if (d->K % 8 || d->a_k_stride != 1 || d->b_k_stride != 1) return false;
-    if ((d->a_row_stride | d->b_row_stride | d->a_batch1_stride | d->a_batch2_stride | d->b_batch1_stride | d->b_batch2_stride) % 8) return false;
-    if (d->out_dtype == DWG_DTYPE_F32X && ((d->ldc | d->c_batch1_stride | d->c_batch2_stride) % 8 || ((uintptr_t)d->C % 16))) return false;
-    if (d->residual && d->residual_dtype == DWG_DTYPE_F32X &&
-        (((d->ldr ? d->ldr : d->ldc) | d->r_batch1_stride | d->r_batch2_stride) % 8 || ((uintptr_t)d->residual % 16))) return false;
-    if (d->act == DWG_ACT_GEGLU_PAIR && d->out_dtype == DWG_DTYPE_F32X && d->N % 16) return false;
-    if (d->conv_enabled && (d->conv_cin % 8 || (d->A2 && d->conv_cin1 % 8))) return false;
-    o->K = 2 * d->K;
-    o->a_row_stride = 2 * d->a_row_stride; o->b_row_stride = 2 * d->b_row_stride;
-    o->a_batch1_stride = 2 * d->a_batch1_stride; o->a_batch2_stride = 2 * d->a_batch2_stride;
-    o->b_batch1_stride = 2 * d->b_batch1_stride; o->b_batch2_stride = 2 * d->b_batch2_stride;
-    o->conv_cin = 2 * d->conv_cin; o->conv_cin1 = 2 * d->conv_cin1;
-    return true;
-}
-#endif
-
-extern "C" {
-
-#if defined(DWG_GEMM_X_TU)
-#define DWG_GEMM_FN dwg_gemm_x
-#define DWG_GEMM_WS_FN dwg_gemm_workspace_bytes_x
-#elif defined(DWG_GEMM_F16_TU)
-#define DWG_GEMM_FN dwg_gemm_f16
-#define DWG_GEMM_WS_FN dwg_gemm_workspace_bytes_f16
-#else
-#define DWG_GEMM_FN dwg_gemm
-#define DWG_GEMM_WS_FN dwg_gemm_workspace_bytes
-size_t dwg_gemm_workspace_bytes_f16(const dwg_gemm_desc* d);
-int dwg_gemm_f16(const dwg_gemm_desc* d, dwg_stream_t stream);
-size_t dwg_gemm_workspace_bytes_x(const dwg_gemm_desc* d);
-int dwg_gemm_x(const dwg_gemm_desc* d, dwg_stream_t stream);
-#endif
-
-size_t DWG_GEMM_WS_FN(const dwg_gemm_desc* d) {
-#if !defined(DWG_GEMM_F16_TU) && !defined(DWG_GEMM_X_TU)
-    if (d && d->dtype == DWG_DTYPE_F16) return dwg_gemm_workspace_bytes_f16(d);
-    if (d && d->dtype == DWG_DTYPE_F32X) return dwg_gemm_workspace_bytes_x(d);
-#endif
-#ifdef DWG_GEMM_X_TU
-    dwg_gemm_desc xd;
-    if (!x_physical(d, &xd)) return 0;
-    d = &xd;
-#endif
-    if (!d || d->M <= 0 || d->N <= 0 || !slabs_possible(d)) return 0;
-    dwg_gemm_desc pd = *d;
-    if (d->plan_m > d->M) pd.M = d->plan_m;
-    d = &pd;
-    int sk = splitk_of(d);
-    if (d->dtype == DWG_DTYPE_HALF && d->splitk == 0 && d->act != DWG_ACT_GEGLU_PAIR) {
-        int bsk = 1;
-        if (big_tile(d->M, d->N, d->K, &bsk) && bsk > sk) sk = bsk;
-    }
-    return sk > 1 ? (size_t)sk * d->M * d->N * sizeof(float) : 0;
-}
-
-int DWG_GEMM_FN(const dwg_gemm_desc* d, dwg_stream_t stream_) {
-#if !defined(DWG_GEMM_F16_TU) && !defined(DWG_GEMM_X_TU)
-    if (d && d->dtype == DWG_DTYPE_F16) return dwg_gemm_f16(d, stream_);
-    if (d && d->dtype == DWG_DTYPE_F32X) return dwg_gemm_x(d, stream_);
-#endif
-#ifdef DWG_GEMM_X_TU
-    dwg_gemm_desc xd;
-    if (!x_physical(d, &xd)) return DWG_E_ARG;
-    d = &xd;
-#endif
+static int prepare(const dwg_gemm_desc* d, GemmP& p, Plan& pl, bool* empty) {
+    *empty = false;
     if (!d || !d->A || !d->B || !d->C) return DWG_E_ARG;
     if (d->M < 0 || d->N < 0 || d->K < 0 || d->batch1 < 1 || d->batch2 < 1 || d->plan_m < 0) return DWG_E_ARG;
-    if (d->M == 0 || d->N == 0) return DWG_OK;
+    if (d->M == 0 || d->N == 0) { *empty = true; return DWG_OK; }
     if (d->dtype != DWG_DTYPE_F32 && d->dtype != DWG_DTYPE_HALF) return DWG_E_ARG;
     if (d->splitk > 1 && !d->workspace && (d->out_dtype != DWG_DTYPE_F32 || d->bias || d->residual || d->act)) return DWG_E_ARG;
     if (d->accumulate && d->out_dtype != DWG_DTYPE_F32) return DWG_E_ARG;
     if (d->act == DWG_ACT_GEGLU_PAIR && (d->N % 64 != 0 || d->residual || d->splitk > 1 || d->bias_per_row || d->bias_row_div)) return DWG_E_ARG;
     if ((uintptr_t)d->workspace & 15) return DWG_E_ARG;
-    GemmP p;
     p.A = d->A; p.B = d->B; p.C = d->C; p.bias = d->bias; p.residual = d->residual;
     p.M = d->M; p.N = d->N; p.K = d->K;
     p.sam = d->a_row_stride; p.sak = d->a_k_stride; p.sbn = d->b_row_stride; p.sbk = d->b_k_stride;
@@ -1545,11 +1603,144 @@
     p.conv.up = d->conv_in_upsample > 1 ? d->conv_in_upsample : 1;
     p.conv.A2 = d->A2; p.conv.cin1 = d->A2 ? d->conv_cin1 : d->conv_cin;
     p.bias_row_div = d->bias_row_div; p.bias_ld = d->bias_ld > 0 ? d->bias_ld : d->N;
-    Plan pl;
     dwg_gemm_desc pd = *d;
     if (d->plan_m > d->M) pd.M = d->plan_m;
-    const int rc = make_plan(&pd, p, pl);
+    p.gn = nullptr; p.gn_G = p.gn_cg = p.gn_hw = p.gn_chunks = p.gn_slots = 0;
+    return make_plan(&pd, p, pl);
+}
+
+static int gn_chunks_of(const dwg_gemm_desc* d, const Plan& pl, int* slots_out) {
+#ifndef DWG_GEMM_GN
+    return 0;
+#else
+    const int G = d->gn_groups, hw = d->gn_rows_per_image;
+    if (G <= 0 || G > 64 || hw <= 0 || d->N % G || d->M % hw || (d->plan_m > d->M && d->plan_m % hw)) return 0;
+    const int cg = d->N / G;
+    if (cg > 64) return 0;
+    if (pl.splitk > 1 || batch_of(d) != 1 || d->dtype != DWG_DTYPE_HALF) return 0;
+    if (pl.fam == FAM_GENERIC || (pl.fam != FAM_PATCH2 && pl.akind == 3)) return 0;
+    if (d->act == DWG_ACT_GEGLU_PAIR || d->accumulate || d->bias_per_row) return 0;
+    if ((d->N & 3) || (d->ldc & 3) || ((uintptr_t)d->C & 15)) return 0;
+    if (d->residual && (((d->ldr ? d->ldr : d->ldc) & 3) || ((uintptr_t)d->residual & 15))) return 0;
+    if (d->bias && (((uintptr_t)d->bias & 15) || (d->bias_row_div > 0 && ((d->bias_ld > 0 ? d->bias_ld : d->N) & 3)))) return 0;
+    long long tiles;
+    if (pl.fam == FAM_PATCH2) {
+        if (hw != d->conv_hout * d->conv_wout) return 0;
+        const int ph = pl.nw == 8 ? 16 : 8;
+        tiles = (long long)((d->conv_hout + ph - 1) / ph) * ((d->conv_wout + 15) / 16);
+    } else {
+        if (hw % pl.bm) return 0;
+        tiles = hw / pl.bm;
+    }
+    const int slots = pl.bn % cg == 0 ? 1 : 2;
+    if (tiles * slots > (1 << 20)) return 0;
+    *slots_out = slots;
+    return (int)(tiles * slots);
+#endif
+}
+
+}
+
+#ifdef DWG_GEMM_X_TU
+static bool x_physical(const dwg_gemm_desc* d, dwg_gemm_desc* o) {
+    if (!d) return false;
+    *o = *d;
+    if (d->dtype != DWG_DTYPE_F32X) return false;
+    if (d->K % 8 || d->a_k_stride != 1 || d->b_k_stride != 1) return false;
+    if ((d->a_row_stride | d->b_row_stride | d->a_batch1_stride | d->a_batch2_stride | d->b_batch1_stride | d->b_batch2_stride) % 8) return false;
+    if (d->out_dtype == DWG_DTYPE_F32X && ((d->ldc | d->c_batch1_stride | d->c_batch2_stride) % 8 || ((uintptr_t)d->C % 16))) return false;
+    if (d->residual && d->residual_dtype == DWG_DTYPE_F32X &&
+        (((d->ldr ? d->ldr : d->ldc) | d->r_batch1_stride | d->r_batch2_stride) % 8 || ((uintptr_t)d->residual % 16))) return false;
+    if (d->act == DWG_ACT_GEGLU_PAIR && d->out_dtype == DWG_DTYPE_F32X && d->N % 16) return false;
+    if (d->conv_enabled && (d->conv_cin % 8 || (d->A2 && d->conv_cin1 % 8))) return false;
+    o->K = 2 * d->K;
+    o->a_row_stride = 2 * d->a_row_stride; o->b_row_stride = 2 * d->b_row_stride;
+    o->a_batch1_stride = 2 * d->a_batch1_stride; o->a_batch2_stride = 2 * d->a_batch2_stride;
+    o->b_batch1_stride = 2 * d->b_batch1_stride; o->b_batch2_stride = 2 * d->b_batch2_stride;
+    o->conv_cin = 2 * d->conv_cin; o->conv_cin1 = 2 * d->conv_cin1;
+    return true;
+}
+#endif
+
+extern "C" {
+
+#if defined(DWG_GEMM_X_TU)
+#define DWG_GEMM_FN dwg_gemm_x
+#define DWG_GEMM_WS_FN dwg_gemm_workspace_bytes_x
+#elif defined(DWG_GEMM_F16_TU)
+#define DWG_GEMM_FN dwg_gemm_f16
+#define DWG_GEMM_WS_FN dwg_gemm_workspace_bytes_f16
+#else
+#define DWG_GEMM_FN dwg_gemm
+#define DWG_GEMM_WS_FN dwg_gemm_workspace_bytes
+size_t dwg_gemm_workspace_bytes_f16(const dwg_gemm_desc* d);
+int dwg_gemm_f16(const dwg_gemm_desc* d, dwg_stream_t stream);
+size_t dwg_gemm_workspace_bytes_x(const dwg_gemm_desc* d);
+int dwg_gemm_x(const dwg_gemm_desc* d, dwg_stream_t stream);
+#endif
+
+size_t DWG_GEMM_WS_FN(const dwg_gemm_desc* d) {
+#if !defined(DWG_GEMM_F16_TU) && !defined(DWG_GEMM_X_TU)
+    if (d && d->dtype == DWG_DTYPE_F16) return dwg_gemm_workspace_bytes_f16(d);
+    if (d && d->dtype == DWG_DTYPE_F32X) return dwg_gemm_workspace_bytes_x(d);
+#endif
+#ifdef DWG_GEMM_X_TU
+    dwg_gemm_desc xd;
+    if (!x_physical(d, &xd)) return 0;
+    d = &xd;
+#endif
+    if (!d || d->M <= 0 || d->N <= 0 || !slabs_possible(d)) return 0;
+    dwg_gemm_desc pd = *d;
+    if (d->plan_m > d->M) pd.M = d->plan_m;
+    d = &pd;
+    int sk = splitk_of(d);
+    if (d->dtype == DWG_DTYPE_HALF && d->splitk == 0 && d->act != DWG_ACT_GEGLU_PAIR) {
+        int bsk = 1;
+        if (big_tile(d->M, d->N, d->K, &bsk) && bsk > sk) sk = bsk;
+    }
+    return sk > 1 ? (size_t)sk * d->M * d->N * sizeof(float) : 0;
+}
+
+#if defined(DWG_GEMM_X_TU)
+int32_t dwg_gemm_gn_chunks_x(const dwg_gemm_desc* d) {
+    dwg_gemm_desc xd;
+    if (!x_physical(d, &xd)) return 0;
+    GemmP p;
+    Plan pl;
+    bool empty;
+    int slots = 1;
+    if (prepare(&xd, p, pl, &empty) != DWG_OK || empty) return 0;
+    return gn_chunks_of(&xd, pl, &slots);
+}
+#elif !defined(DWG_GEMM_F16_TU)
+int32_t dwg_gemm_gn_chunks_x(const dwg_gemm_desc* d);
+int32_t dwg_gemm_gn_chunks(const dwg_gemm_desc* d) { return d && d->dtype == DWG_DTYPE_F32X ? dwg_gemm_gn_chunks_x(d) : 0; }
+#endif
+
+int DWG_GEMM_FN(const dwg_gemm_desc* d, dwg_stream_t stream_) {
+#if !defined(DWG_GEMM_F16_TU) && !defined(DWG_GEMM_X_TU)
+    if (d && d->dtype == DWG_DTYPE_F16) return dwg_gemm_f16(d, stream_);
+    if (d && d->dtype == DWG_DTYPE_F32X) return dwg_gemm_x(d, stream_);
+#endif
+#ifdef DWG_GEMM_X_TU
+    dwg_gemm_desc xd;
+    if (!x_physical(d, &xd)) return DWG_E_ARG;
+    d = &xd;
+#endif
+    GemmP p;
+    Plan pl;
+    bool empty;
+    const int rc = prepare(d, p, pl, &empty);
     if (rc != DWG_OK) return rc;
+    if (empty) return DWG_OK;
+    if (d->gn_partials) {
+        int slots = 1;
+        const int chunks = gn_chunks_of(d, pl, &slots);
+        if (chunks <= 0 || ((uintptr_t)d->gn_partials & 3)) return DWG_E_ARG;
+        if ((size_t)(d->M / d->gn_rows_per_image) * 2 * d->gn_groups * chunks > d->gn_partials_floats) return DWG_E_ARG;
+        p.gn = d->gn_partials; p.gn_G = d->gn_groups; p.gn_cg = d->N / d->gn_groups; p.gn_hw = d->gn_rows_per_image;
+        p.gn_chunks = chunks; p.gn_slots = slots;
+    }
     p.splitk = pl.splitk;
     p.ws = pl.slabs ? reinterpret_cast<float*>(d->workspace) : nullptr;
     const int batch = batch_of(d);
diff --git a/dreamwaltz-g_amd/csrc/nn_norm.hip b/dreamwaltz-g_amd/csrc/nn_norm.hip
--- a/dreamwaltz-g_amd/csrc/nn_norm.hip
+++ b/dreamwaltz-g_amd/csrc/nn_norm.hip
@@ -561,6 +561,24 @@
     return DWG_OK;
 }
 
+int dwg_groupnorm_forward_partials(int32_t dtype, int32_t B, int32_t HW, int32_t C, int32_t G, const void* x, const float* gamma,
+                                   const float* beta, float eps, int32_t fuse_silu, void* y, float* stats, const float* partials,
+                                   int32_t chunks, dwg_stream_t stream_) {
+    if (B <= 0 || HW <= 0 || !x || !gamma || !beta || !y || !stats || !partials || chunks <= 0) return DWG_E_ARG;
+    int ppb, achunks; size_t lds;
+    int rc = gn_geometry(HW, C, G, &ppb, &achunks, &lds);
+    if (rc) return rc;
+    hipStream_t stream = (hipStream_t)stream_;
+    const bool fold = gn_fold(chunks, G);
+    DWG_DT_SWITCH(dtype,
+        if (!fold) DWG_LAUNCH("gn_finalize", k_gn_finalize, dim3((2 * G + 3) / 4, B), dim3(256), 0, stream, chunks, G, partials, stats);
+        DWG_LAUNCH("gn_apply", (k_gn_apply<T, false>), dim3(achunks, B), dim3(256), 0, stream, HW, C, G, ppb, (const T*)x,
+                   (const T*)nullptr, (const float*)stats, (const float*)nullptr, gamma, beta, fuse_silu, eps, (T*)y,
+                   fold ? partials : (const float*)nullptr, chunks, stats, (const T*)nullptr))
+    DWG_RETURN_IF_LAUNCH_FAILED();
+    return DWG_OK;
+}
+
 int dwg_groupnorm_forward(int32_t B, int32_t HW, int32_t C, int32_t G, const void* x, const float* gamma, const float* beta,
                           float eps, int32_t fuse_silu, void* y, float* stats, float* workspace, dwg_stream_t stream) {
     return dwg_groupnorm_forward_dt(DWG_DTYPE_BF16, B, HW, C, G, x, gamma, beta, eps, fuse_silu, y, stats, workspace, stream);
diff --git a/dreamwaltz-g_amd/gemm.py b/dreamwaltz-g_amd/gemm.py
--- a/dreamwaltz-g_amd/gemm.py
+++ b/dreamwaltz-g_amd/gemm.py
@@ -30,6 +30,8 @@
         ("bias_row_div", ctypes.c_int32), ("bias_ld", ctypes.c_int64),
         ("workspace", ctypes.c_void_p), ("workspace_bytes", ctypes.c_size_t),
         ("name", ctypes.c_char_p), ("plan_m", ctypes.c_int32),
+        ("gn_partials", ctypes.c_void_p), ("gn_partials_floats", ctypes.c_size_t),
+        ("gn_groups", ctypes.c_int32), ("gn_rows_per_image", ctypes.c_int32),
     ]
 
 
diff --git a/dreamwaltz-g_amd/sd15.py b/dreamwaltz-g_amd/sd15.py
--- a/dreamwaltz-g_amd/sd15.py
+++ b/dreamwaltz-g_amd/sd15.py
@@ -528,6 +528,7 @@
                 b = None
         conv = (C, H, W, Ho, Wo, KH, KW, stride, pt, pl, in_dilation)
         K = KH * KW * C
+        one_launch = False
         if r_batch_bcast and KH * KW == 1 and stride == 1 and pad == 0 and pad_tl is None and upsample == 1 and in_dilation == 1 and out_hw is None:
             Vr = int(residual.shape[0])
             assert B % Vr == 0 and bias_img is None, (B, Vr)
@@ -551,7 +552,10 @@
             d = gemm.gemm_raw(x, wt, y, B * Ho * Wo, Cout, K, (0, 1), (K, 1), Cout, residual=residual,
                               ldr=Cout if residual is not None else 0, act=act, conv=conv, conv_upsample=upsample,
                               name=self._conv_tag(tag, KH, Ho, stride, in_dilation, KW), plan_m=self._plan_rows(B, B * Ho * Wo), run=False, **kw)
+            one_launch = True
         self.p.add_gemm(d)
+        if one_launch:
+            self._produced(y, d, B, Ho * Wo)
         return y
 
     def linear(self, x, wt, bias=None, act=None, residual=None, out_dtype=None, tag="linear"):
@@ -572,7 +576,30 @@
                           ldr=Nout if residual is not None else 0, act=act, name=tag, plan_m=self._plan_rows(x.shape[0], M) if x.dim() > 2 else 0,
                           run=False)
         self.p.add_gemm(d)
+        if x.dim() > 2:
+            self._produced(y, d, x.shape[0], M // x.shape[0])
         return y
+
+    def _produced(self, y, d, images, rows):
+        self.__dict__.setdefault("_gn_producers", {})[y.data_ptr()] = [d, int(images), int(rows), None]
+
+    def gn_request(self, x):
+        src = self.__dict__.get("_gn_producers", {}).get(x.data_ptr())
+        if src is None or not self.p.is_x:
+            return None
+        B, C = x.shape[0], x.shape[-1]
+        HW = x.numel() // (B * C)
+        d = src[0]
+        if src[3] is None and (src[1], src[2], d.N, d.ldc) == (B, HW, C, C):
+            d.gn_groups, d.gn_rows_per_image = self.groups, HW
+            chunks = int(self.L.dwg_gemm_gn_chunks(ctypes.byref(d)))
+            if chunks <= 0:
+                d.gn_groups = d.gn_rows_per_image = 0
+                return None
+            part = self.p.buf(B, 2 * self.groups, chunks, dtype=torch.float32)
+            d.gn_partials, d.gn_partials_floats = part.data_ptr(), part.numel()
+            src[3] = (part, chunks)
+        return src[3]
 
     def _gn_ws(self, B):
         need = int(self.L.dwg_groupnorm_workspace_floats(B, self.groups))
@@ -590,6 +617,11 @@
         y = self.p.buf(*x.shape)
         stats = self.p.buf(B, self.groups, 2, dtype=torch.float32)
         pp = lambda t: ctypes.c_void_p(t.data_ptr())
+        part = self.gn_request(x) if HW > 1024 else None
+        if part is not None:
+            self.p.add_call(self.L.dwg_groupnorm_forward_partials, self.p.dt, B, HW, C, self.groups, pp(x), pp(self.w.f32(name + ".weight")),
+                            pp(self.w.f32(name + ".bias")), eps, int(silu), pp(y), pp(stats), pp(part[0]), part[1])
+            return (y, stats) if keep_stats else y
         self.p.add_call(self.L.dwg_groupnorm_forward_dt, self.p.dt, B, HW, C, self.groups, pp(x), pp(self.w.f32(name + ".weight")),
                         pp(self.w.f32(name + ".bias")), eps, int(silu), pp(y), pp(stats), pp(self._gn_ws(B)))
         return (y, stats) if keep_stats else y
diff --git a/include/dwg_gemm.h b/include/dwg_gemm.h
--- a/include/dwg_gemm.h
+++ b/include/dwg_gemm.h
@@ -42,9 +42,15 @@
     size_t workspace_bytes;
     const char* name;
     int32_t plan_m;
+    float* gn_partials;
+    size_t gn_partials_floats;
+    int32_t gn_groups;
+    int32_t gn_rows_per_image;
 } dwg_gemm_desc;
 
 int dwg_gemm(const dwg_gemm_desc* desc, dwg_stream_t stream);
+
+int32_t dwg_gemm_gn_chunks(const dwg_gemm_desc* desc);
 
 size_t dwg_gemm_workspace_bytes(const dwg_gemm_desc* desc);
 
diff --git a/include/dwg_nn.h b/include/dwg_nn.h
--- a/include/dwg_nn.h
+++ b/include/dwg_nn.h
@@ -30,6 +30,9 @@
 int dwg_groupnorm_forward_dt(int32_t dtype, int32_t B, int32_t HW, int32_t C, int32_t G, const void* x, const float* gamma,
                              const float* beta, float eps, int32_t fuse_silu, void* y, float* stats, float* workspace,
                              dwg_stream_t stream);
+int dwg_groupnorm_forward_partials(int32_t dtype, int32_t B, int32_t HW, int32_t C, int32_t G, const void* x, const float* gamma,
+                                   const float* beta, float eps, int32_t fuse_silu, void* y, float* stats, const float* partials,
+                                   int32_t chunks, dwg_stream_t stream);
 int dwg_groupnorm_backward_dt(int32_t dtype, int32_t B, int32_t HW, int32_t C, int32_t G, const void* x, const void* dy,
                               const float* stats, const float* gamma, const float* beta, float eps, int32_t fuse_silu, void* dx,
                               float* scratch, float* workspace, const void* residual, dwg_stream_t stream);
```

After: 40.86, median of 6. No clear change (+0.8%).
